# laboshinl/loam_velodyne

Measured on AMD Instinct MI355X. Metric: sweeps/sec (64-ring, 1M-pt map): feature extraction + odometry + scan-to-map registration, higher is better.
Workload: dtype f32

## Files before the change

include/loamx.h:

```cpp
#ifndef LOAMX_H
#define LOAMX_H

#include <stddef.h>
#include <stdint.h>

#ifdef __cplusplus
extern "C" {
#endif

#define LOAMX_OK 0
#define LOAMX_SKIPPED 1
#define LOAMX_E_INVALID (-1)
#define LOAMX_E_CAPACITY (-2)
#define LOAMX_E_HIP (-3)
#define LOAMX_E_NOGPU (-4)
#define LOAMX_E_UNSUPPORTED (-5)
#define LOAMX_E_INTERNAL (-6)

typedef struct loamx_cloud {
  void* data;
  uint32_t count;
  uint32_t stride;
  uint32_t intensity_offset;
  uint32_t reserved;
} loamx_cloud;

const char* loamx_last_error(void);
int loamx_device_count(void);
#define LOAMX_ABI_VERSION 6
int loamx_abi_version(void);
const char* loamx_build_info(void);
void* loamx_host_alloc(size_t bytes);
void loamx_host_free(void* p);

typedef struct loamx_scanreg loamx_scanreg;

typedef struct loamx_scanreg_config {
  float scan_period;
  int n_feature_regions;
  int curvature_region;
  int max_corner_sharp;
  int max_surface_flat;
  float less_flat_filter_size;
  float surface_curvature_threshold;
  int device;
  int max_corner_less_sharp;
  int imu_history_size;
} loamx_scanreg_config;


void loamx_scanreg_default_config(loamx_scanreg_config* cfg);
loamx_scanreg* loamx_scanreg_create(const loamx_scanreg_config* cfg);
void loamx_scanreg_destroy(loamx_scanreg* h);
int loamx_scanreg_configure(loamx_scanreg* h, const loamx_scanreg_config* cfg);
int loamx_scanreg_process(loamx_scanreg* h, const loamx_cloud* cloud, const uint32_t* ring_size, uint32_t n_rings,
                          loamx_cloud* sharp, loamx_cloud* less_sharp, loamx_cloud* flat, loamx_cloud* less_flat);

typedef struct loamx_multiscan_mapper {
  float lower_bound_deg;
  float upper_bound_deg;
  uint32_t n_scan_rings;
} loamx_multiscan_mapper;
int loamx_multiscan_mapper_preset(const char* sensor , loamx_multiscan_mapper* out);
int loamx_scanreg_process_raw(loamx_scanreg* h, const loamx_multiscan_mapper* mapper, const void* raw_xyz, uint32_t count,
                              uint32_t stride, loamx_cloud* full, uint32_t* ring_size, loamx_cloud* sharp, loamx_cloud* less_sharp,
                              loamx_cloud* flat, loamx_cloud* less_flat);

enum { LOAMX_RING_FROM_BOUNDS = 0, LOAMX_RING_FROM_TABLE = 1, LOAMX_RING_FROM_FIELD = 2 };
enum { LOAMX_TIME_FROM_AZIMUTH = 0, LOAMX_TIME_FROM_FIELD = 1 };
enum { LOAMX_FIELD_U8 = 1, LOAMX_FIELD_U16 = 2, LOAMX_FIELD_U32 = 3, LOAMX_FIELD_F32 = 4, LOAMX_FIELD_F64 = 5 };
typedef struct loamx_sensor_model {
  uint32_t n_scan_rings;
  uint32_t ring_source, time_source;
  float lower_bound_deg, upper_bound_deg;
  const float* ring_angles_deg;
  float max_angle_error_deg;
  uint32_t ring_offset, ring_type;
  uint32_t time_offset, time_type;
  double time_scale;
} loamx_sensor_model;
int loamx_sensor_model_from_mapper(const loamx_multiscan_mapper* m, loamx_sensor_model* out);
int loamx_sensor_model_check(const loamx_sensor_model* m, uint32_t stride);
int loamx_scanreg_process_sensor(loamx_scanreg* h, const loamx_sensor_model* m, const void* records, uint32_t count, uint32_t stride,
                                 loamx_cloud* full, uint32_t* ring_size, loamx_cloud* sharp, loamx_cloud* less_sharp,
                                 loamx_cloud* flat, loamx_cloud* less_flat);

int loamx_scanreg_update_imu(loamx_scanreg* h, double stamp_sec, float roll, float pitch, float yaw, const float acc_xyz[3]);
int loamx_scanreg_set_time(loamx_scanreg* h, double scan_time_sec);
int loamx_scanreg_get_imu_trans(loamx_scanreg* h, float imu_trans[12]);

typedef struct loamx_odom loamx_odom;

typedef struct loamx_odom_config {
  float scan_period;
  int max_iterations;
  float delta_t_abort;
  float delta_r_abort;
  int device;
} loamx_odom_config;

void loamx_odom_default_config(loamx_odom_config* cfg);
loamx_odom* loamx_odom_create(const loamx_odom_config* cfg);
void loamx_odom_destroy(loamx_odom* h);
int loamx_odom_update_imu(loamx_odom* h, const float imu_trans[12]);
int loamx_odom_process(loamx_odom* h, const loamx_cloud* sharp, const loamx_cloud* less_sharp, const loamx_cloud* flat,
                       const loamx_cloud* less_flat);
int loamx_odom_get_transform(loamx_odom* h, float transform[6]);
int loamx_odom_get_transform_sum(loamx_odom* h, float transform_sum[6]);
int loamx_odom_set_transform(loamx_odom* h, const float transform[6]);
int loamx_odom_set_transform_sum(loamx_odom* h, const float transform_sum[6]);
int loamx_odom_get_last_clouds(loamx_odom* h, loamx_cloud* last_corner, loamx_cloud* last_surf);
int loamx_odom_transform_to_end(loamx_odom* h, loamx_cloud* cloud);
int loamx_odom_get_stats(loamx_odom* h, int stats[4]);

int loamx_scanreg_process_linked(loamx_scanreg* h, const loamx_cloud* cloud, const uint32_t* ring_size, uint32_t n_rings);
int loamx_odom_process_linked(loamx_odom* h, loamx_scanreg* sr);
int loamx_odom_link_wait(loamx_odom* h);

typedef struct loamx_map loamx_map;

typedef struct loamx_map_config {
  float scan_period;
  int max_iterations;
  float delta_t_abort;
  float delta_r_abort;
  float corner_filter_size;
  float surf_filter_size;
  float map_filter_size;
  int device;
} loamx_map_config;

void loamx_map_default_config(loamx_map_config* cfg);
loamx_map* loamx_map_create(const loamx_map_config* cfg);
void loamx_map_destroy(loamx_map* h);
int loamx_map_update_odometry(loamx_map* h, const float transform_sum[6]);
int loamx_map_process(loamx_map* h, const loamx_cloud* corner_last, const loamx_cloud* surf_last, loamx_cloud* full_res);
int loamx_map_process_linked(loamx_map* h, loamx_odom* od, loamx_cloud* full_res_registered);
int loamx_map_get_speculation(loamx_map* h, uint64_t counts[2]);
int loamx_map_insert(loamx_map* h, const loamx_cloud* corner_last, const loamx_cloud* surf_last, const float pose6[6]);
int loamx_map_get_transform(loamx_map* h, int which, float transform[6]);
int loamx_map_set_transform(loamx_map* h, int which, const float transform[6]);
int loamx_map_update_imu(loamx_map* h, double stamp_sec, float roll, float pitch);
int loamx_map_set_time(loamx_map* h, double laser_odometry_time_sec);
int loamx_map_has_fresh_map(loamx_map* h);
int loamx_map_get_surround(loamx_map* h, loamx_cloud* out);
int loamx_map_load_cubes(loamx_map* h, const loamx_cloud* corner, const loamx_cloud* surf);
int loamx_map_get_cubes(loamx_map* h, int which, loamx_cloud* out);
int loamx_map_save_snapshot(loamx_map* h, const char* path);
int loamx_map_load_snapshot(loamx_map* h, const char* path);
int loamx_map_set_timing(loamx_map* h, int on);
int loamx_map_get_timing(loamx_map* h, float ms[4], uint64_t counts[4]);
int loamx_map_get_stats(loamx_map* h, int stats[8]);

typedef struct loamx_tm loamx_tm;
loamx_tm* loamx_tm_create(void);
void loamx_tm_destroy(loamx_tm* h);
int loamx_tm_update_odometry(loamx_tm* h, const float transform_sum[6]);
int loamx_tm_update_mapping_transform(loamx_tm* h, const float aft_mapped[6], const float bef_mapped[6]);
int loamx_tm_associate_to_map(loamx_tm* h);
int loamx_tm_get_mapped(loamx_tm* h, float transform_mapped[6]);
int loamx_wire_pose_to_quat(const float rot_xyz[3], double quat_xyzw[4]);
int loamx_wire_quat_to_pose(const double quat_xyzw[4], float rot_xyz[3]);

typedef struct loamx_batch loamx_batch;

loamx_batch* loamx_batch_create(const loamx_map_config* cfg, uint32_t max_sweeps);
void loamx_batch_destroy(loamx_batch* h);
int loamx_batch_set_frozen(loamx_batch* h, const loamx_cloud* corner_map, const loamx_cloud* surf_map);
int loamx_batch_set_frozen_device(loamx_batch* h, const void* d_corner_xyzi, uint32_t n_corner, const void* d_surf_xyzi,
                                  uint32_t n_surf);
int loamx_batch_stage_frozen_device(loamx_batch* h, const void* d_corner_xyzi, uint32_t n_corner, const void* d_surf_xyzi,
                                    uint32_t n_surf, void* wait_event );
int loamx_batch_stage_frozen(loamx_batch* h, const loamx_cloud* corner_map, const loamx_cloud* surf_map);
int loamx_batch_swap_frozen(loamx_batch* h);
int loamx_batch_upload(loamx_batch* h, uint32_t n_sweeps, const loamx_cloud* corner_last, const loamx_cloud* surf_last,
                       const loamx_cloud* full_res, const float* guess6);
int loamx_batch_run(loamx_batch* h);
int loamx_batch_run_async(loamx_batch* h);
int loamx_batch_sync(loamx_batch* h);
int loamx_batch_download(loamx_batch* h, float* poses6, int* stats4);
int loamx_batch_download_full_res(loamx_batch* h, uint32_t sweep, loamx_cloud* out);
int loamx_batch_set_timing(loamx_batch* h, int on);
int loamx_batch_get_timing(loamx_batch* h, float ms[4], uint64_t counts[4]);
void* loamx_batch_stream(loamx_batch* h);
int loamx_batch_knn_probe(loamx_batch* h, int which, const float* queries_xyz, uint32_t n, uint32_t* idx5, float* d2_5);
int loamx_batch_qr6_probe(loamx_batch* h, const float* ata, const float* atb, uint32_t n, float* x_coop, float* x_scalar);
int loamx_batch_xrec_stress(loamx_batch* h, uint32_t pairs, uint32_t rounds, uint64_t out4[4]);
int loamx_batch_download_ds(loamx_batch* h, uint32_t sweep, loamx_cloud* corner_ds, loamx_cloud* surf_ds);

int loamx_voxel_probe(const float* pts_xyzi, uint32_t n, const uint32_t* seg_off, const uint32_t* seg_ids, const uint8_t* valid, uint32_t nseg,
                      float leaf_even, float leaf_odd, float* out_xyzi, uint32_t* out_off);
#define LOAMX_SCAN_COUNT_ON_DEVICE 1u
#define LOAMX_SCAN_IN_PLACE 2u
#define LOAMX_SCAN_ZERO_IN 4u
int loamx_scan_probe(uint32_t* in, uint32_t n, uint32_t max_n, uint32_t flags, uint32_t* out, uint32_t* total, uint32_t* out2);
#define LOAMX_INDEX_SINGLE 1u
#define LOAMX_INDEX_PACK_RING 2u
#define LOAMX_INDEX_FOLD_BOUNDS 4u
typedef struct loamx_index_desc {
  float ox, oy, oz, inv_h;
  int32_t nx, ny, nz;
  uint32_t ncell;
  uint32_t cell_base;
  uint32_t pt_base;
} loamx_index_desc;
int loamx_index_probe(const float* pts_xyzw, uint32_t n, const uint32_t* off, uint32_t K, float cell_edge, uint32_t flags, loamx_index_desc* desc,
                      uint32_t* table, uint32_t table_cap, uint32_t* table_len, float* sorted_xyzw);
#define LOAMX_VOXBUCKET_SRC_POINTERS 1u
typedef struct loamx_voxbucket_seg {
  uint32_t bucket0, nbuckets, pos_bits, pad;
} loamx_voxbucket_seg;
typedef struct loamx_voxbucket_status {
  uint32_t gave_up;
  uint32_t why;
  uint32_t buckets;
  uint32_t pad;
} loamx_voxbucket_status;
int loamx_voxbucket_probe(const float* pts_xyzi, uint32_t n, const uint32_t* seg_off, uint32_t nseg, const float* poses12, float leaf_even,
                          float leaf_odd, uint32_t flags, float* stack_xyzi, float* out_xyzi, uint32_t* out_off,
                          loamx_voxbucket_status* status, loamx_voxbucket_seg* segs, uint64_t* lo, uint32_t* cnt, uint32_t bucket_cap);
#define LOAMX_REPROJECT_BATCH 0u
#define LOAMX_REPROJECT_FUSED 1u
#define LOAMX_REPROJECT_SINGLE 2u
#define LOAMX_REPROJECT_COPY 3u
#define LOAMX_REPROJECT_GATHER 4u
#define LOAMX_REPROJECT_TO_START 5u
#define LOAMX_REPROJECT_NO_RING_TABLE 8u
#define LOAMX_REPROJECT_NO_BOUNDS 16u
typedef struct loamx_reproject_params {
  float T[6];
  float sT[3], cT[3];
  float shift[3];
  float s_start[3], c_start[3];
  float s_end[3], c_end[3];
  float scan_period;
  int32_t enabled;
} loamx_reproject_params;
int loamx_reproject_probe(const float* pts_xyzw, uint32_t n, const uint32_t* off, uint32_t K, const loamx_reproject_params* params, uint32_t ns,
                          uint32_t epoch, uint32_t n_corner_all, uint32_t flags, float* out_xyzw, uint32_t* ring_first, uint32_t* bounds);

typedef struct loamx_pipeline loamx_pipeline;

loamx_pipeline* loamx_pipeline_create(const loamx_scanreg_config* fcfg, const loamx_odom_config* ocfg,
                                      const loamx_map_config* mcfg, uint32_t n_streams);
void loamx_pipeline_destroy(loamx_pipeline* h);
int loamx_pipeline_set_frozen(loamx_pipeline* h, const loamx_cloud* corner_map, const loamx_cloud* surf_map);
int loamx_pipeline_set_frozen_device(loamx_pipeline* h, const void* d_corner_xyzi, uint32_t n_corner, const void* d_surf_xyzi,
                                     uint32_t n_surf);
int loamx_pipeline_stage_frozen_device(loamx_pipeline* h, const void* d_corner_xyzi, uint32_t n_corner, const void* d_surf_xyzi,
                                       uint32_t n_surf, void* wait_event);
int loamx_pipeline_stage_frozen(loamx_pipeline* h, const loamx_cloud* corner_map, const loamx_cloud* surf_map);
int loamx_pipeline_swap_frozen(loamx_pipeline* h);
int loamx_pipeline_set_state(loamx_pipeline* h, uint32_t stream, const float* transform, const float* transform_sum,
                             const float* bef_mapped, const float* aft_mapped);
int loamx_pipeline_upload(loamx_pipeline* h, uint32_t n_steps, const loamx_cloud* clouds, const uint32_t* const* ring_size,
                          const uint32_t* n_rings);
int loamx_pipeline_stage_step(loamx_pipeline* h, uint32_t step, const loamx_cloud* clouds, const uint32_t* const* ring_size,
                              const uint32_t* n_rings);
int loamx_pipeline_stage_step_raw(loamx_pipeline* h, uint32_t step, const void* const* raw_xyz, const uint32_t* counts, uint32_t stride,
                                  const loamx_multiscan_mapper* mapper, const double* scan_time_sec);
int loamx_pipeline_stage_step_sensor(loamx_pipeline* h, uint32_t step, const void* const* records, const uint32_t* counts,
                                     uint32_t stride, const loamx_sensor_model* m, const double* scan_time_sec);
int loamx_pipeline_update_imu(loamx_pipeline* h, uint32_t stream, double stamp_sec, float roll, float pitch, float yaw, const float acc_xyz[3]);
int loamx_pipeline_enable_async_downloads(loamx_pipeline* h);
int loamx_pipeline_download_step_async(loamx_pipeline* h, loamx_cloud* out, uint32_t n_out);
int loamx_pipeline_wait_downloads(loamx_pipeline* h);
int loamx_pipeline_download_counts(loamx_pipeline* h, uint64_t counts[2]);
int loamx_pipeline_step(loamx_pipeline* h, uint32_t step);
int loamx_pipeline_get(loamx_pipeline* h, uint32_t stream, float* transform, float* transform_sum, float* aft_mapped,
                       int* stats8);
int loamx_pipeline_download_full_res(loamx_pipeline* h, uint32_t slot, loamx_cloud* out);
int loamx_pipeline_download_last_clouds(loamx_pipeline* h, uint32_t stream, loamx_cloud* last_corner, loamx_cloud* last_surf);
int loamx_pipeline_set_lookahead(loamx_pipeline* h, int on);
int loamx_pipeline_lookahead_depth(loamx_pipeline* h);
int loamx_pipeline_drain_lookahead(loamx_pipeline* h, int* last_odometry_step);
int loamx_pipeline_set_timing(loamx_pipeline* h, int on);
int loamx_pipeline_get_timing(loamx_pipeline* h, float stage_ms[4], float reg_ms[4], uint64_t counts[4]);
int loamx_pipeline_get_odom_launch_timing(loamx_pipeline* h, double ms4[4], uint64_t counts7[7]);
void* loamx_pipeline_stream(loamx_pipeline* h);

typedef struct loamx_dist loamx_dist;
#define LOAMX_DIST_ID_BYTES 128
int loamx_dist_get_unique_id(unsigned char id[LOAMX_DIST_ID_BYTES]);
loamx_dist* loamx_dist_create(const unsigned char id[LOAMX_DIST_ID_BYTES], int rank, int world_size, int device);
void loamx_dist_destroy(loamx_dist* h);
int loamx_dist_rank(const loamx_dist* h);
int loamx_dist_world_size(const loamx_dist* h);
int loamx_dist_shard(const loamx_dist* h, uint32_t batch, uint32_t* begin, uint32_t* end);
int loamx_dist_broadcast_map(loamx_dist* h, void* d_corner_xyzi, uint32_t n_corner, void* d_surf_xyzi, uint32_t n_surf, int root,
                             void* wait_event, void** done_event);
int loamx_dist_allgather_results(loamx_dist* h, const float* poses6, const int* iters_flags2, uint32_t n_local, float* poses6_all,
                                 int* iters_flags2_all, uint32_t* counts_all);
int loamx_dist_allgather_results_cap(loamx_dist* h, const float* poses6, const int* iters_flags2, uint32_t n_local, float* poses6_all,
                                     int* iters_flags2_all, uint32_t capacity_records, uint32_t* counts_all);
int loamx_dist_allgather_counts(loamx_dist* h, uint32_t n_local, uint32_t* counts_all);
int loamx_dist_comm_count(loamx_dist* h);
#define LOAMX_DIST_RECORD_FLOATS 8
int loamx_dist_shard_of(int rank, int world_size, uint32_t batch, uint32_t* begin, uint32_t* end);
int loamx_dist_pack_results(const float* poses6, const int* iters_flags2, uint32_t n_local, uint32_t n_pad, float* send8);
int loamx_dist_unpack_results(const float* recv8, const uint32_t* counts, int world_size, uint32_t n_pad, float* poses6_all,
                              int* iters_flags2_all);
int loamx_dist_pack_clouds(uint32_t n_streams, const loamx_cloud* corner, const loamx_cloud* surf, const float* poses6, uint32_t* words,
                           uint64_t capacity_words, uint64_t* n_words);
int loamx_dist_unpack_clouds_header(const uint32_t* words, uint64_t n_words, uint32_t* n_streams, uint32_t* n_corner, uint32_t* n_surf,
                                    uint32_t capacity_streams);
int loamx_dist_unpack_clouds_stream(const uint32_t* words, uint64_t n_words, uint32_t stream, float pose6[6], loamx_cloud* corner,
                                    loamx_cloud* surf);
int loamx_dist_gatherv(loamx_dist* h, const uint32_t* send_words, uint32_t n_words, int root, uint32_t* recv_words, uint64_t capacity_words,
                       uint32_t* counts_all);
int loamx_dist_barrier(loamx_dist* h);
void* loamx_dist_stream(loamx_dist* h);

typedef struct loamx_densemap loamx_densemap;
typedef struct loamx_densemap_config {
  float leaf;
  float min_range;
  float max_range;
  uint64_t max_voxels;
  uint32_t initial_slots;
  int device;
} loamx_densemap_config;

void loamx_densemap_default_config(loamx_densemap_config* cfg);
loamx_densemap* loamx_densemap_create(const loamx_densemap_config* cfg);
void loamx_densemap_destroy(loamx_densemap* h);
int loamx_densemap_reset(loamx_densemap* h);
int loamx_densemap_add(loamx_densemap* h, const loamx_cloud* points, const float origin[3]);
int loamx_densemap_add_from_map(loamx_densemap* h, loamx_map* m);
int loamx_densemap_add_from_pipeline(loamx_densemap* h, loamx_pipeline* p, uint32_t slot);
int loamx_densemap_get_stats(loamx_densemap* h, uint64_t stats[6]);
int loamx_densemap_download(loamx_densemap* h, loamx_cloud* out, int axes );
int loamx_densemap_save_pcd(loamx_densemap* h, const char* path, int axes);
int loamx_write_pcd(const char* path, const loamx_cloud* c, int axes);

typedef struct loamx_densemap_carve_config {
  float max_range;
  uint32_t ray_stride;
  uint32_t end_margin;
  uint32_t max_steps;
} loamx_densemap_carve_config;
typedef struct loamx_densemap_static_rule {
  uint32_t min_misses;
  uint32_t num, den;
} loamx_densemap_static_rule;
void loamx_densemap_carve_default_config(loamx_densemap_carve_config* cfg);
void loamx_densemap_static_rule_default(loamx_densemap_static_rule* rule);
int loamx_densemap_rule_is_dynamic(const loamx_densemap_static_rule* rule, uint64_t n, uint32_t miss);
int loamx_densemap_enable_carving(loamx_densemap* h, const loamx_densemap_carve_config* cfg );
int loamx_densemap_get_carve_stats(loamx_densemap* h, uint64_t stats[6]);
int loamx_densemap_download_misses(loamx_densemap* h, uint32_t* out, uint64_t capacity, uint64_t* n);
int loamx_densemap_download_static(loamx_densemap* h, loamx_cloud* out, int axes, const loamx_densemap_static_rule* rule);
int loamx_densemap_save_pcd_static(loamx_densemap* h, const char* path, int axes, const loamx_densemap_static_rule* rule);
int loamx_densemap_prune(loamx_densemap* h, const loamx_densemap_static_rule* rule, uint64_t* removed);

typedef struct loamx_surfel {
  float x, y, z, intensity, normal_x, normal_y, normal_z, curvature;
} loamx_surfel;
typedef struct loamx_densemap_surfel_config {
  uint32_t min_points;
  float min_planar_ratio;
} loamx_densemap_surfel_config;
void loamx_densemap_surfel_default_config(loamx_densemap_surfel_config* cfg);
int loamx_densemap_surfel_of(float leaf, const int32_t idx[3], const uint64_t vals[4], const uint64_t mom[9],
                             const loamx_densemap_surfel_config* cfg, int axes, loamx_surfel* out);
int loamx_densemap_enable_moments(loamx_densemap* h);
int loamx_densemap_download_moments(loamx_densemap* h, uint64_t* out, uint64_t capacity, uint64_t* n);
int loamx_densemap_download_surfels(loamx_densemap* h, loamx_surfel* out, uint64_t capacity, uint64_t* n, int axes,
                                    const loamx_densemap_surfel_config* cfg, const loamx_densemap_static_rule* rule);
int loamx_densemap_save_pcd_surfels(loamx_densemap* h, const char* path, int axes, const loamx_densemap_surfel_config* cfg,
                                    const loamx_densemap_static_rule* rule);

int loamx_densemap_freeze(loamx_densemap* h, const loamx_densemap_surfel_config* cfg, const loamx_densemap_static_rule* rule,
                          uint64_t* n_surfels);
int loamx_densemap_frozen_size(loamx_densemap* h, uint64_t* n_surfels);
int loamx_densemap_align_step(loamx_densemap* h, const loamx_cloud* points, const float rtc[15], uint32_t neighbourhood,
                              float max_residual, int64_t sums[28], uint64_t counts[5]);
typedef struct loamx_densemap_align_config {
  uint32_t max_iterations;
  uint32_t neighbourhood;
  float max_residual;
  uint32_t min_matched;
  float eps_rot, eps_trans;
  float degenerate_ratio;
} loamx_densemap_align_config;
typedef struct loamx_densemap_align_result {
  double pose[12];
  uint32_t iterations, degenerate_dims;
  int status;
  double rms;
  uint64_t counts[5];
} loamx_densemap_align_result;
void loamx_densemap_align_default_config(loamx_densemap_align_config* cfg);
int loamx_densemap_align_solve(const int64_t sums[28], float degenerate_ratio, double x[6], uint32_t* dropped);
int loamx_densemap_align(loamx_densemap* h, const loamx_cloud* points, const double pose_in[12], const float centre[3] ,
                         const loamx_densemap_align_config* cfg , loamx_densemap_align_result* out);
int loamx_densemap_align_from_map(loamx_densemap* h, loamx_map* m, const double pose_in[12] ,
                                  const loamx_densemap_align_config* cfg, loamx_densemap_align_result* out);
int loamx_densemap_align_from_pipeline(loamx_densemap* h, loamx_pipeline* p, uint32_t slot, const double pose_in[12],
                                       const loamx_densemap_align_config* cfg, loamx_densemap_align_result* out);

#define LOAMX_ALIGN_MAX_POSES 4096
int loamx_densemap_align_step_many(loamx_densemap* h, const loamx_cloud* points, const float* rtc , uint32_t n_poses,
                                   uint32_t neighbourhood, float max_residual, int64_t* sums , uint64_t* counts );
int loamx_densemap_align_many(loamx_densemap* h, const loamx_cloud* points, const double* poses_in , uint32_t n_poses,
                              const float centre[3] , const loamx_densemap_align_config* cfg,
                              loamx_densemap_align_result* out , uint32_t* best );
int loamx_densemap_align_many_from_map(loamx_densemap* h, loamx_map* m, const double* poses_in, uint32_t n_poses,
                                       const loamx_densemap_align_config* cfg, loamx_densemap_align_result* out, uint32_t* best);
int loamx_densemap_align_many_from_pipeline(loamx_densemap* h, loamx_pipeline* p, uint32_t slot, const double* poses_in, uint32_t n_poses,
                                            const loamx_densemap_align_config* cfg, loamx_densemap_align_result* out, uint32_t* best);
int loamx_densemap_align_best(const loamx_densemap_align_result* results, uint32_t n, uint32_t* best);
int loamx_densemap_get_align_stats(loamx_densemap* h, uint64_t stats[3]);

#define LOAMX_PYRAMID_MAX_LEVELS 6
typedef struct loamx_densemap_pyramid_config {
  uint32_t levels;
  float max_curvature;
} loamx_densemap_pyramid_config;
void loamx_densemap_pyramid_default_config(loamx_densemap_pyramid_config* cfg);
int loamx_densemap_coarsen(loamx_densemap* h, uint32_t level, const loamx_densemap_static_rule* rule ,
                           uint64_t* keys, uint64_t* vals , uint64_t* mom , uint64_t capacity,
                           uint64_t* n);
int loamx_densemap_freeze_pyramid(loamx_densemap* h, const loamx_densemap_surfel_config* cfg, const loamx_densemap_static_rule* rule,
                                  const loamx_densemap_pyramid_config* pyramid , uint64_t* n_surfels );
int loamx_densemap_frozen_levels(loamx_densemap* h, uint32_t* levels);
int loamx_densemap_align_select_level(loamx_densemap* h, uint32_t level);
int loamx_densemap_align_pyramid(loamx_densemap* h, const loamx_cloud* points, const double pose_in[12], const float centre[3] ,
                                 const loamx_densemap_align_config* cfg, uint32_t first_level,
                                 loamx_densemap_align_result* out );
int loamx_densemap_align_pyramid_from_map(loamx_densemap* h, loamx_map* m, const double pose_in[12] ,
                                          const loamx_densemap_align_config* cfg, uint32_t first_level, loamx_densemap_align_result* out);
int loamx_densemap_align_pyramid_from_pipeline(loamx_densemap* h, loamx_pipeline* p, uint32_t slot, const double pose_in[12],
                                               const loamx_densemap_align_config* cfg, uint32_t first_level,
                                               loamx_densemap_align_result* out);

struct loamx_densemap_file_info {
  uint32_t version, flags;
  float leaf;
  uint64_t voxels;
  uint64_t offered, dropped_range, dropped_key;
  uint64_t carve_stats[6];
  loamx_densemap_carve_config carve;
};
int loamx_densemap_save(loamx_densemap* h, const char* path);
int loamx_densemap_load(loamx_densemap* h, const char* path);
int loamx_densemap_merge(loamx_densemap* dst, loamx_densemap* src);
int loamx_densemap_merge_file(loamx_densemap* dst, const char* path);
int loamx_densemap_file_info(const char* path, struct loamx_densemap_file_info* info, int deep);

#define LOAMX_RAY_NOT_TRACED 0
#define LOAMX_RAY_MISS 1
#define LOAMX_RAY_HIT 2
#define LOAMX_RAY_HIT_END 3
typedef struct loamx_ray_hit {
  uint64_t key;
  float x, y, z;
  float range;
  uint32_t n;
  uint32_t miss;
  uint32_t steps;
  uint32_t status;
} loamx_ray_hit;
typedef struct loamx_densemap_raycast_config {
  uint32_t max_steps;
  uint32_t skip_steps;
  uint32_t min_points;
} loamx_densemap_raycast_config;
void loamx_densemap_raycast_default_config(loamx_densemap_raycast_config* cfg);
int loamx_densemap_raycast(loamx_densemap* h, const loamx_cloud* ends, const float origin[3],
                           const loamx_densemap_raycast_config* cfg ,
                           const loamx_densemap_static_rule* rule ,
                           loamx_ray_hit* out , uint64_t capacity, uint64_t counts[5]);
int loamx_densemap_raycast_from_map(loamx_densemap* h, loamx_map* m, const loamx_densemap_raycast_config* cfg,
                                    const loamx_densemap_static_rule* rule, loamx_ray_hit* out, uint64_t capacity, uint64_t counts[5]);
int loamx_densemap_raycast_from_pipeline(loamx_densemap* h, loamx_pipeline* p, uint32_t slot,
                                         const loamx_densemap_raycast_config* cfg, const loamx_densemap_static_rule* rule,
                                         loamx_ray_hit* out, uint64_t capacity, uint64_t counts[5]);

typedef struct loamx_densemap_history_config {
  uint64_t max_bytes;
  uint64_t initial_points;
} loamx_densemap_history_config;
void loamx_densemap_history_default_config(loamx_densemap_history_config* cfg);
int loamx_densemap_enable_history(loamx_densemap* h, const loamx_densemap_history_config* cfg );
int loamx_densemap_history_size(loamx_densemap* h, uint64_t* calls, uint64_t* points);
int loamx_densemap_history_download(loamx_densemap* h, uint64_t call, loamx_cloud* out , float origin[3]);
int loamx_densemap_correct(const double correction[12], const float* xyz_in, float* xyz_out, uint64_t n);
int loamx_densemap_rebuild(loamx_densemap* h, const double* corrections ,
                           uint64_t n_calls);
int loamx_densemap_get_rebuild_stats(loamx_densemap* h, uint64_t stats[4]);

#define LOAMX_GRID_UNKNOWN 0
#define LOAMX_GRID_FREE 1
#define LOAMX_GRID_OBSTACLE 2
#define LOAMX_GRID_STEP 3
typedef struct loamx_densemap_grid_config {
  uint32_t cell_leaves;
  int32_t  x0, z0;
  uint32_t nx, nz;
  uint32_t min_points;
  int32_t  y_min, y_max;
  uint32_t band_lo, band_hi;
  uint32_t min_obstacle_voxels;
  uint32_t max_step;
  uint32_t clear_max;
} loamx_densemap_grid_config;
typedef struct loamx_grid_cell {
  int32_t  ground;
  float    elevation;
  uint32_t obstacles;
  int32_t  overhead;
  uint32_t clear2;
  uint32_t cls;
} loamx_grid_cell;
void loamx_densemap_grid_default_config(loamx_densemap_grid_config* cfg);
int loamx_densemap_grid_check(const loamx_densemap_grid_config* cfg);
int loamx_densemap_grid_window(float leaf, float centre_x, float centre_z, float half_extent, loamx_densemap_grid_config* cfg);
int loamx_densemap_grid(loamx_densemap* h, const loamx_densemap_grid_config* cfg ,
                        const loamx_densemap_static_rule* rule ,
                        loamx_grid_cell* out );
int loamx_grid_occupancy(const loamx_grid_cell* cells, uint64_t n, int8_t* out);
int loamx_write_grid_pgm(const char* stem, const loamx_grid_cell* cells, const loamx_densemap_grid_config* cfg, float leaf);

#define LOAMX_ROUTE_UNREACHABLE 0xffffffffu
#define LOAMX_ROUTE_GOAL 8u
#define LOAMX_ROUTE_NONE 9u
typedef struct loamx_grid_route_config {
  uint32_t connectivity;
  uint32_t min_clear2;
  uint32_t soft_clear2;
  uint32_t soft_weight;
  uint32_t unknown_weight;
} loamx_grid_route_config;
typedef struct loamx_route_cell {
  uint32_t cost;
  uint32_t next;
} loamx_route_cell;
void loamx_grid_route_default_config(loamx_grid_route_config* cfg);
int loamx_grid_route_check(const loamx_grid_route_config* cfg);
int loamx_grid_route_weight(const loamx_grid_cell* cell, const loamx_grid_route_config* cfg);
int loamx_densemap_route(loamx_densemap* h, const loamx_densemap_grid_config* grid_cfg ,
                         const loamx_densemap_static_rule* rule ,
                         const loamx_grid_route_config* cfg , const uint32_t* goals_xz, uint32_t n_goals,
                         loamx_grid_cell* out_cells , loamx_route_cell* out_field ,
                         uint64_t stats[6] );
int loamx_densemap_route_cells(loamx_densemap* h, const loamx_grid_cell* cells, uint32_t nx, uint32_t nz,
                               const loamx_grid_route_config* cfg , const uint32_t* goals_xz, uint32_t n_goals,
                               loamx_route_cell* out_field , uint64_t stats[6] );
int loamx_densemap_route_trace(loamx_densemap* h, const uint32_t* starts_xz, uint32_t n_starts ,
                               uint32_t* out_xz , uint32_t capacity, uint32_t* lengths );
int loamx_grid_route_trace(const loamx_route_cell* field, uint32_t nx, uint32_t nz, uint32_t start_x, uint32_t start_z,
                           uint32_t* out_xz , uint32_t capacity, uint32_t* length);
int loamx_grid_route_points(const loamx_densemap_grid_config* grid_cfg, float leaf, const loamx_grid_cell* cells ,
                            const uint32_t* route_xz, uint32_t n, float* out_xyz );
int loamx_densemap_grid_cell_of(const loamx_densemap_grid_config* grid_cfg, float leaf, float x, float z, uint32_t* rx, uint32_t* rz,
                                int* inside);

#define LOAMX_FRONTIER_NONE 0xFFFFFFFFu
typedef struct loamx_grid_frontier_config {
  uint32_t connectivity;
  uint32_t min_unknown;
  uint32_t min_clear2;
  uint32_t min_cells;
} loamx_grid_frontier_config;
typedef struct loamx_frontier {
  uint32_t min_cell;
  uint32_t cells;
  uint32_t lo[2], hi[2];
  uint64_t sum_rx, sum_rz;
  uint64_t unknown_links;
  uint32_t reachable;
// ... 143 lines not shown
```

loam_velodyne_amd/csrc/hostlink.hpp:

```cpp
#pragma once
#include "common.h"
#include <hsa/hsa.h>
#include <hsa/hsa_ext_amd.h>

namespace loamx {

template <int SLOTS> class HostLinkT {
 public:
  ~HostLinkT() {
    for (int s = 0; s < SLOTS; s++) {
      if (!made_[s]) continue;
      try { wait(s); } catch (...) {}
      (void)hsa_signal_destroy(sig_[s]);
    }
  }
  bool can_copy(void* host_dst, const void* dev_src, size_t bytes) {
    if (!init_()) return false;
    hsa_agent_t g, c;
    return owner_(dev_src, bytes, HSA_DEVICE_TYPE_GPU, &g) && owner_(host_dst, bytes, HSA_DEVICE_TYPE_CPU, &c);
  }
  void begin(int slot, uint32_t n) {
    LX_REQUIRE(init_(), "ROCr is not available");
    wait(slot);
    if (!made_[slot]) {
      LX_REQUIRE(hsa_signal_create(0, 0, nullptr, &sig_[slot]) == HSA_STATUS_SUCCESS, "hsa_signal_create failed");
      made_[slot] = true;
    }
    hsa_signal_store_relaxed(sig_[slot], (hsa_signal_value_t)n);
    pending_[slot] = n > 0;
    unissued_[slot] = n;
  }
  void abandon(int slot) {
    if (!pending_[slot]) return;
    if (unissued_[slot]) hsa_signal_subtract_relaxed(sig_[slot], (hsa_signal_value_t)unissued_[slot]);
    unissued_[slot] = 0;
    try { wait(slot); } catch (...) { pending_[slot] = false; }
  }
  void copy_d2h(int slot, void* host_dst, const void* dev_src, size_t bytes) {
    hsa_agent_t g, c;
    LX_REQUIRE(owner_(dev_src, bytes, HSA_DEVICE_TYPE_GPU, &g) && owner_(host_dst, bytes, HSA_DEVICE_TYPE_CPU, &c), "not ROCr-allocated memory");
    hsa_status_t st = HSA_STATUS_ERROR;
    const uint32_t eng = engine_(c, g);
    if (eng) {
      st = hsa_amd_memory_async_copy_on_engine(host_dst, c, dev_src, g, bytes, 0, nullptr, sig_[slot], (hsa_amd_sdma_engine_id_t)eng, false);
      if (st != HSA_STATUS_SUCCESS) engine_mask_ = 0;
    }
    if (st != HSA_STATUS_SUCCESS) st = hsa_amd_memory_async_copy(host_dst, c, dev_src, g, bytes, 0, nullptr, sig_[slot]);
    if (st != HSA_STATUS_SUCCESS) {
      abandon(slot);
      throw Error(LOAMX_E_HIP, "hsa_amd_memory_async_copy failed (" + std::to_string((int)st) + ")");
    }
    if (unissued_[slot]) unissued_[slot]--;
  }
  bool can_copy_h2d(void* dev_dst, const void* host_src, size_t bytes) {
    if (!init_()) return false;
    hsa_agent_t g, c;
    return owner_(dev_dst, bytes, HSA_DEVICE_TYPE_GPU, &g) && owner_(host_src, bytes, HSA_DEVICE_TYPE_CPU, &c);
  }
  bool host_ok(const void* host, size_t bytes) {
    hsa_agent_t c;
    return init_() && owner_(host, bytes, HSA_DEVICE_TYPE_CPU, &c);
  }
  void copy_h2d(int slot, void* dev_dst, const void* host_src, size_t bytes) {
    hsa_agent_t g, c;
    LX_REQUIRE(owner_(dev_dst, bytes, HSA_DEVICE_TYPE_GPU, &g) && owner_(host_src, bytes, HSA_DEVICE_TYPE_CPU, &c), "not ROCr-allocated memory");
    const hsa_status_t st = hsa_amd_memory_async_copy(dev_dst, g, host_src, c, bytes, 0, nullptr, sig_[slot]);
    if (st != HSA_STATUS_SUCCESS) {
      abandon(slot);
      throw Error(LOAMX_E_HIP, "hsa_amd_memory_async_copy (host -> device) failed (" + std::to_string((int)st) + ")");
    }
    if (unissued_[slot]) unissued_[slot]--;
  }
  uint32_t engine() const { return engine_mask_ == ~0u ? 0u : engine_mask_; }
  bool pending(int slot) const { return pending_[slot]; }
  void wait(int slot) {
    if (!pending_[slot]) return;
    hsa_signal_value_t v;
    while ((v = hsa_signal_wait_scacquire(sig_[slot], HSA_SIGNAL_CONDITION_LT, 1, UINT64_MAX, HSA_WAIT_STATE_BLOCKED)) > 0) {}
    pending_[slot] = false;
    if (v < 0) throw Error(LOAMX_E_HIP, "a device -> host DMA reported an error");
  }

 private:
  static bool init_() {
    static const bool ok = hsa_init() == HSA_STATUS_SUCCESS;
    return ok;
  }
  static bool owner_(const void* p, size_t bytes, hsa_device_type_t want, hsa_agent_t* agent) {
    hsa_amd_pointer_info_t info;
    info.size = sizeof(info);
    if (hsa_amd_pointer_info(p, &info, nullptr, nullptr, nullptr) != HSA_STATUS_SUCCESS) return false;
    if (info.type != HSA_EXT_POINTER_TYPE_HSA) return false;
    const char* base = (const char*)(want == HSA_DEVICE_TYPE_CPU && info.hostBaseAddress ? info.hostBaseAddress : info.agentBaseAddress);
    if (!base || (const char*)p < base || (const char*)p + bytes > base + info.sizeInBytes) return false;
    hsa_device_type_t type;
    if (hsa_agent_get_info(info.agentOwner, HSA_AGENT_INFO_DEVICE, &type) != HSA_STATUS_SUCCESS || type != want) return false;
    *agent = info.agentOwner;
    return true;
  }
  uint32_t engine_(hsa_agent_t cpu, hsa_agent_t gpu) {
    if (engine_mask_ == ~0u) {
      if (const char* e = diag_env("LOAMX_D2H_ENGINE")) engine_mask_ = (uint32_t)strtoul(e, nullptr, 0);
      else {
        uint32_t rec = 0;
        if (hsa_amd_memory_get_preferred_copy_engine(cpu, gpu, &rec) != HSA_STATUS_SUCCESS) rec = 0;
        rec &= ~(uint32_t)HSA_AMD_SDMA_ENGINE_0;
        engine_mask_ = rec ? (rec & (~rec + 1u)) : (uint32_t)HSA_AMD_SDMA_ENGINE_1;
      }
    }
    return engine_mask_;
  }
  uint32_t engine_mask_ = ~0u;
  hsa_signal_t sig_[SLOTS] = {};
  bool made_[SLOTS] = {}, pending_[SLOTS] = {};
  uint32_t unissued_[SLOTS] = {};
};
using HostLinkDma = HostLinkT<2>;
using HostLinkUp = HostLinkT<8>;

}
```

loam_velodyne_amd/csrc/pipeline.hip:

```cpp
#include "pinned_copy.hpp"
#include "features.hpp"
#include "odometry.hpp"
#include "registration.hpp"
#include "hostlink.hpp"
#include "densemap.hpp"
#include "odom_lookahead.hpp"
#include <atomic>
#include <deque>
#include <chrono>
#include <mutex>
#include <memory>

namespace loamx {

struct OdomPub {
  HTwist transform, transform_sum;
  OdomStats stats = {0, 0, 0, 0};
  int rc = LOAMX_SKIPPED;
  const float4* last_corner = nullptr; uint32_t n_last_corner = 0;
  const float4* last_surf = nullptr; uint32_t n_last_surf = 0;
  ToEndParams to_end;
};

struct PipeStreamState {
  HTwist bef, aft, tobe, incre;
  OdomPub cur;
  SweepStats map_stats = {0, 0, 0, 0, 0, 0, 0, 0};
  bool mapped = false;
};

class Pipeline {
 public:
  Pipeline(const loamx_scanreg_config& fc, const loamx_odom_config& oc, const loamx_map_config& mc, uint32_t n_streams)
      : reg(mc.device, n_streams), fcfg(fc), n_streams_(n_streams), st(n_streams), imu(n_streams), map_imu(n_streams), map_imu_seq(n_streams, 0) {
    OdomParams op;
    op.scan_period = oc.scan_period;
    op.max_iterations = diag_env("LOAMX_ODOM_MAXIT") ? atoi(diag_env("LOAMX_ODOM_MAXIT")) : oc.max_iterations;
    if (op.max_iterations < 1 || op.max_iterations > 255) throw Error(LOAMX_E_INVALID, "odometry max_iterations must be in [1, 255]");
    op.delta_t_abort = oc.delta_t_abort;
    op.delta_r_abort = oc.delta_r_abort;
    {
      int g = (int)std::min<uint32_t>(n_streams, 2);
      if (const char* e = diag_env("LOAMX_ODOM_GROUPS")) g = atoi(e);
      n_groups = (uint32_t)std::max(1, std::min(g, (int)std::min<uint32_t>(n_streams, MAX_GROUPS)));
    }
    for (uint32_t g = 0; g < n_groups; g++) {
      chains.emplace_back(new OdomChain());
      OdomChain& c = *chains.back();
      c.s0 = (uint32_t)((uint64_t)g * n_streams / n_groups);
      c.s1 = (uint32_t)((uint64_t)(g + 1) * n_streams / n_groups);
      c.ob.reset(new OdometryBatch(mc.device, c.s1 - c.s0, nullptr));
    }
    for (auto& o : ores) o.resize(n_streams);
    for (auto& tr : imu) tr.history_size = std::max(200, fc.imu_history_size);
    reg.params.max_iterations = mc.max_iterations;
    reg.early_exit = true;
    reg.double_buffer_full = true;
    reg.params.delta_t_abort = mc.delta_t_abort;
    reg.params.delta_r_abort = mc.delta_r_abort;
    reg.params.corner_leaf = mc.corner_filter_size;
    reg.params.surf_leaf = mc.surf_filter_size;
    for (auto& c : chains) { c->ob->params = op; c->ob->set_keep(OR - 2); }
    device = mc.device;
    if (getenv("LOAMX_NO_LOOKAHEAD")) prefetch = false;
    const double spin_us = diag_env("LOAMX_SPIN_US") ? atof(diag_env("LOAMX_SPIN_US")) : 400.0;
    la.reset(new LookAhead(
        n_groups, [this](uint32_t g, int k) { run_chain_step(*chains[g], (uint32_t)k); }, [this] { (void)hipSetDevice(device); },
        std::chrono::duration_cast<std::chrono::steady_clock::duration>(std::chrono::duration<double, std::micro>(spin_us))));
  }
  Registrar reg;
  static constexpr int OR = 16;
  struct LazyTimer {
    hipEvent_t a = nullptr, b = nullptr;
    bool pending = false;
    float ms = 0.f;
    void start(hipStream_t s) {
      if (!a) { LX_HIP(hipEventCreate(&a)); LX_HIP(hipEventCreate(&b)); }
      pending = false;
      LX_HIP(hipEventRecord(a, s));
    }
    void stop(hipStream_t s) { LX_HIP(hipEventRecord(b, s)); pending = true; }
    bool resolve() {
      if (!pending || hipEventQuery(b) != hipSuccess) return false;
      LX_HIP(hipEventElapsedTime(&ms, a, b));
      pending = false;
      return true;
    }
    void destroy() { if (a) { (void)hipEventDestroy(a); (void)hipEventDestroy(b); a = b = nullptr; } }
  };
  struct OdomChain {
    uint32_t s0 = 0, s1 = 0;
    std::unique_ptr<OdometryBatch> ob;
    hipEvent_t ev_tail[OR] = {};
    LazyTimer tm[OR];
    std::atomic<float> ms{0.f};
    double tr[4] = {0, 0, 0, 0};
    std::atomic<float> last_us{0.f};
  };
  static constexpr uint32_t MAX_GROUPS = 16;
  uint32_t n_groups = 1;
  std::vector<std::unique_ptr<OdomChain>> chains;
  OdomChain& chain_of(uint32_t s) { uint32_t g = 0; while (g + 1 < n_groups && s >= chains[g]->s1) g++; return *chains[g]; }
  OdometryBatch& OB(uint32_t s) { return *chain_of(s).ob; }
  uint32_t LS(uint32_t s) { return s - chain_of(s).s0; }
  loamx_scanreg_config fcfg;
  uint32_t n_streams_;
  int device;
  std::vector<PipeStreamState> st;
  std::vector<std::unique_ptr<FeatureExtractor>> fx;
  static constexpr uint32_t RING = 8;
  bool streaming = false;
  std::atomic<uint32_t> staged_hi{0};
  hipStream_t cstream = nullptr, dstream = nullptr;
  hipEvent_t ev_stage[RING] = {};
  hipEvent_t ev_reg_done = nullptr, ev_d2h[2] = {nullptr, nullptr};
  bool d2h_pending[2] = {false, false};
  uint64_t downloads_direct = 0, downloads_hip = 0;
  HostLinkDma hostlink;
  HostLinkUp uplink;
  uint32_t up_runs[RING] = {};
  std::atomic<long> last_step{-1};
  std::vector<uint32_t> last_full_off;
  std::vector<uint32_t> last_who;
  struct RawSlot {
    bool raw = false, finalized = true;
    std::vector<uint32_t> count, off;
    DevBuf<char> d_bytes;
    DevBuf<float4> d_raw4, d_binned;
    DevBuf<uint32_t> d_ring_fld;
    DevBuf<double> d_time_fld;
    DevBuf<uint32_t> d_ring_cnt;
    PinBuf<uint32_t> h_ring_cnt;
    DevBuf<ImuLast> d_last;
    PinBuf<ImuLast> h_last;
    DevBuf<double> d_imu_d;
    DevBuf<float> d_imu_f;
    PinBuf<double> h_imu_d;
    PinBuf<float> h_imu_f;
    std::vector<uint32_t> imu_H;
    std::vector<float> imu_trans;
    std::vector<double> scan_time;
    std::vector<uint64_t> map_imu_upto;
    hipEvent_t ev_ingest = nullptr;
    uint32_t n_rings = 0;
  };
  RawSlot rawslot[RING];
  std::vector<ImuTracker> imu;
  struct MapImu { double stamp; float roll, pitch; uint64_t seq; };
  std::vector<std::deque<MapImu>> map_imu;
  std::vector<uint64_t> map_imu_seq;
  std::mutex map_imu_mu;
  void map_imu_push(uint32_t s, double stamp, float roll, float pitch) {
    std::lock_guard<std::mutex> lk(map_imu_mu);
    if (map_imu[s].size() >= 200) map_imu[s].pop_front();
    map_imu[s].push_back(MapImu{stamp, roll, pitch, map_imu_seq[s]++});
  }
  bool map_imu_blend(uint32_t s, uint64_t seq_limit, double odo_time, float scan_period, float* p6) {
    std::lock_guard<std::mutex> lk(map_imu_mu);
    const std::deque<MapImu>& Hq = map_imu[s];
    size_t n = 0;
    while (n < Hq.size() && Hq[n].seq < seq_limit) n++;
    if (!n) return false;
    size_t i = 0;
    while (i < n - 1 && (odo_time - Hq[i].stamp) + scan_period > 0) i++;
    float roll, pitch;
    if (i == 0 || (odo_time - Hq[i].stamp) + scan_period > 0) {
      roll = Hq[i].roll; pitch = Hq[i].pitch;
    } else {
      const float ratio = (float)(((Hq[i].stamp - odo_time) - scan_period) / (Hq[i].stamp - Hq[i - 1].stamp));
      const float inv = 1 - ratio;
      roll = Hq[i].roll * inv + Hq[i - 1].roll * ratio;
      pitch = Hq[i].pitch * inv + Hq[i - 1].pitch * ratio;
    }
    p6[0] = (float)(0.998 * p6[0] + 0.002 * pitch);
    p6[2] = (float)(0.998 * p6[2] + 0.002 * roll);
    return true;
  }
  RawBinner binner;
  FeatureExtractor& FX(uint32_t t) { return *fx[streaming ? t % RING : t]; }
  char& LA(uint32_t t) { return launched[streaming ? t % RING : t]; }
  uint32_t n_staged() const { return streaming ? staged_hi.load(std::memory_order_acquire) : (uint32_t)fx.size(); }
  hipStream_t fstream = nullptr;
  bool prefetch = true;
  std::vector<char> launched;
  PinBuf<uint32_t> h_off3[OR];
  hipEvent_t evF[OR][2] = {};
  LazyTimer tmM[2];
  float feat_ms[OR] = {};
  int f_hi = -1;
  int ahead_depth = std::max(1, std::min(diag_env("LOAMX_ODOM_AHEAD") ? atoi(diag_env("LOAMX_ODOM_AHEAD")) : 6, OR - 2));
  int depth() const { return !prefetch ? 0 : (streaming ? std::min(ahead_depth, (int)RING - 2) : ahead_depth); }
  float last_ms[4] = {0, 0, 0, 0};
  std::atomic<bool> timing{false};

  std::vector<OdomPub> ores[OR];
  std::unique_ptr<LookAhead> la;
  void run_chain_step(OdomChain& c, uint32_t k) {
    const auto tc0 = std::chrono::steady_clock::now();
    c.tr[0] = tr_us(); run_odometry(c, k); c.tr[3] = tr_us();
    c.last_us.store((float)std::chrono::duration<double, std::micro>(std::chrono::steady_clock::now() - tc0).count(), std::memory_order_relaxed);
  }
  int drain_lookahead() { return prefetch ? la->drain() : la->done_min(); }
  void park_odometry(int restart) {
    if (restart >= 0) pre_t = -1;
    la->park(restart);
  }

  ~Pipeline() {
    la.reset();
    for (auto& c : chains) {
      for (auto& e : c->ev_tail) if (e) (void)hipEventDestroy(e);
      for (auto& tm : c->tm) tm.destroy();
    }
    fx.clear();
    for (auto& a : evF) for (auto& e : a) if (e) (void)hipEventDestroy(e);
    for (auto& tm : tmM) tm.destroy();
    for (auto& e : ev_stage) if (e) (void)hipEventDestroy(e);
    for (auto& r : rawslot) if (r.ev_ingest) (void)hipEventDestroy(r.ev_ingest);
    for (auto& e : ev_d2h) if (e) (void)hipEventDestroy(e);
    if (ev_reg_done) (void)hipEventDestroy(ev_reg_done);
    if (cstream) { (void)hipStreamSynchronize(cstream); (void)hipStreamDestroy(cstream); }
    if (dstream) { (void)hipStreamSynchronize(dstream); (void)hipStreamDestroy(dstream); }
    if (fstream) (void)hipStreamDestroy(fstream);
  }

  void launch_features(uint32_t t) {
    TraceRange trace_range("loamx:features");
    finalize_raw(t);
    FeatureExtractor& F = FX(t);
    const uint32_t ns = n_streams_, nring = F.total_rings();
    if (streaming) {
      LX_HIP(hipStreamWaitEvent(fstream, ev_stage[t % RING], 0));
      if (up_runs[t % RING]) { uplink.wait((int)(t % RING)); up_runs[t % RING] = 0; }
    }
    PinBuf<uint32_t>& hb = h_off3[t % OR];
    hb.reserve(3 * (ns + 1) + nring + 2);
    for (auto& e : evF[t % OR]) if (!e) LX_HIP(hipEventCreate(&e));
    LX_HIP(hipEventRecord(evF[t % OR][0], fstream));
    F.run_async();
    LX_REQUIRE(F.n_offsets() == 3 * (ns + 1) + nring + 1, "internal: offset table layout");
    store_to_pinned_u32(hb.p, F.d_offsets(), F.n_offsets(), fstream);
    LX_HIP(hipEventRecord(evF[t % OR][1], fstream));
    LA(t) = 1;
  }

  std::unique_ptr<FeatureExtractor> new_extractor_() {
    auto f = std::make_unique<FeatureExtractor>(device, fstream);
    f->params = feat_params_from(fcfg);
    return f;
  }
  void feature_stream_() {
    if (!fstream) fstream = create_stream(env_priority("LOAMX_PRIO_FEAT", -1), diag_env("LOAMX_FEAT_CU_STRIDE") ? atoi(diag_env("LOAMX_FEAT_CU_STRIDE")) : 0, 1);
    LX_HIP(hipStreamSynchronize(fstream));
    fx.clear();
  }
  void restart_input_(uint32_t n_slots, bool ring) {
    streaming = ring;
    staged_hi = 0;
    last_step = -1;
    launched.assign(n_slots, 0);
    la->reset();
    f_hi = -1;
  }

  void upload(uint32_t n_steps, const loamx_cloud* clouds, const uint32_t* const* ring_size, const uint32_t* n_rings) {
    LX_REQUIRE(n_steps >= 1 && clouds && ring_size && n_rings, "invalid argument");
    LX_HIP(hipSetDevice(device));
    feature_stream_();
    restart_input_(n_steps, false);
    for (uint32_t t = 0; t < n_steps; t++) {
      auto f = new_extractor_();
      f->upload(n_streams_, clouds + (size_t)t * n_streams_, ring_size + (size_t)t * n_streams_, n_rings + (size_t)t * n_streams_);
      fx.push_back(std::move(f));
    }
  }

  void begin_staging_(uint32_t t, const char* entry) {
    LX_HIP(hipSetDevice(device));
    if (!streaming) {
      LX_REQUIRE(t == 0, "streaming input starts at step 0");
      feature_stream_();
      for (uint32_t k = 0; k < RING; k++) fx.push_back(new_extractor_());
      if (!cstream) cstream = create_stream(0);
      for (auto& e : ev_stage) if (!e) LX_HIP(hipEventCreateWithFlags(&e, hipEventDisableTiming));
      restart_input_(RING, true);
    }
    LX_REQUIRE(t == staged_hi.load(), "steps must be staged in order");
    LX_REQUIRE(t < RING || last_step.load() + (long)RING >= (long)t, std::string(entry) + "(t) needs step(t - 8) to have run: only eight steps can be in flight");
  }
  void publish_staged_(uint32_t t) {
    LA(t) = 0;
    staged_hi.store(t + 1, std::memory_order_release);
  }

  void stage_step(uint32_t t, const loamx_cloud* clouds, const uint32_t* const* ring_size, const uint32_t* n_rings) {
    LX_REQUIRE(clouds && ring_size && n_rings, "invalid argument");
    begin_staging_(t, "stage_step");
    TraceRange trace_range("loamx:pipeline:stage_step");
    if (t > 0) finalize_raw(t - 1);
    rawslot[t % RING].raw = false;
    rawslot[t % RING].finalized = true;
    static const bool direct = !(diag_env("LOAMX_H2D_DIRECT") && atoi(diag_env("LOAMX_H2D_DIRECT")) == 0);
    const int slot = (int)(t % RING);
    up_runs[slot] = 0;
    uint32_t n_blocks = 0;
    bool all_direct = direct;
    if (direct) {
      for (uint32_t s = 0; s < n_streams_ && all_direct;) {
        all_direct = clouds[s].stride == 16 && clouds[s].intensity_offset == 12;
        uint32_t e = s + 1;
        size_t cnt = clouds[s].count;
        while (all_direct && e < n_streams_ && (const char*)clouds[e].data == (const char*)clouds[s].data + sizeof(float4) * cnt) cnt += clouds[e++].count;
        if (cnt) { n_blocks++; all_direct = all_direct && uplink.host_ok(clouds[s].data, sizeof(float4) * cnt); }
        s = e;
      }
    }
    if (all_direct && n_blocks) {
      uplink.begin(slot, n_blocks);
      uint32_t issued = 0;
      try {
        fx[slot]->upload_async(n_streams_, clouds, ring_size, n_rings, cstream, ev_stage[slot], [&](void* dst, const void* src, size_t bytes) {
          if (!uplink.can_copy_h2d(dst, src, bytes)) throw Error(LOAMX_E_HIP, "internal: a staging block is not ROCr's memory after all");
          uplink.copy_h2d(slot, dst, src, bytes);
          issued++;
          return true;
        });
      } catch (...) {
        uplink.abandon(slot);
        throw;
      }
      up_runs[slot] = issued;
    } else {
      fx[slot]->upload_async(n_streams_, clouds, ring_size, n_rings, cstream, ev_stage[slot]);
    }
    publish_staged_(t);
  }

  void stage_step_raw(uint32_t t, const void* const* raw_xyz, const uint32_t* counts, uint32_t stride, const loamx_multiscan_mapper& mapper,
                      const double* scan_time) {
    LX_REQUIRE(raw_xyz && counts, "invalid argument");
    mapper_check(mapper.lower_bound_deg, mapper.upper_bound_deg, mapper.n_scan_rings, stride);
    stage_records_(t, raw_xyz, counts, stride, mapper_params(mapper.lower_bound_deg, mapper.upper_bound_deg, mapper.n_scan_rings), scan_time);
  }
  void stage_step_sensor(uint32_t t, const void* const* records, const uint32_t* counts, uint32_t stride, const loamx_sensor_model& model,
                         const double* scan_time) {
    LX_REQUIRE(records && counts, "invalid argument");
    sensor_model_check(model, stride);
    stage_records_(t, records, counts, stride, sensor_params(model), scan_time);
  }
  void stage_records_(uint32_t t, const void* const* raw_xyz, const uint32_t* counts, uint32_t stride, const SensorParams& model,
                      const double* scan_time) {
    begin_staging_(t, "stage_step_raw");
    TraceRange trace_range("loamx:pipeline:stage_step_raw");
    if (t > 0) finalize_raw(t - 1);
    const uint32_t ns = n_streams_, nr = model.M.n_rings;
    RawSlot& R = rawslot[t % RING];
    R.raw = true;
    R.finalized = false;
    R.n_rings = nr;
    R.count.assign(counts, counts + ns);
    R.off.assign(ns + 1, 0);
    for (uint32_t s = 0; s < ns; s++) {
      LX_REQUIRE(raw_xyz[s] || counts[s] == 0, "NULL raw cloud");
      R.off[s + 1] = R.off[s] + counts[s];
    }
    const uint32_t ntot = R.off[ns];
    R.d_bytes.reserve((size_t)ntot * stride + 16);
    R.d_raw4.reserve((size_t)ntot + 1);
    R.d_binned.reserve((size_t)ntot + 1);
    if (model.ring_src == RING_FIELD) R.d_ring_fld.reserve((size_t)ntot + 1);
    if (model.time_src == TIME_FIELD) R.d_time_fld.reserve((size_t)ntot + 1);
    R.d_ring_cnt.reserve((size_t)ns * nr + 1);
    R.h_ring_cnt.reserve((size_t)ns * nr + 1);
    R.d_last.reserve(ns);
    R.h_last.reserve(ns);
    R.imu_H.assign(ns, 0);
    R.imu_trans.assign((size_t)12 * ns, 0.f);
    if (scan_time) R.scan_time.assign(scan_time, scan_time + ns); else R.scan_time.clear();
    {
      std::lock_guard<std::mutex> lk(map_imu_mu);
      R.map_imu_upto = map_imu_seq;
    }
    if (!R.ev_ingest) LX_HIP(hipEventCreateWithFlags(&R.ev_ingest, hipEventDisableTiming));
    size_t Htot = 0;
    for (uint32_t s = 0; s < ns; s++) { R.imu_H[s] = imu[s].size(); Htot += R.imu_H[s]; }
    if (Htot) {
      R.h_imu_d.reserve(2 * Htot); R.h_imu_f.reserve(9 * Htot); R.d_imu_d.reserve(2 * Htot); R.d_imu_f.reserve(9 * Htot);
    }
    binner.init(cstream);
    LX_HIP(hipMemsetAsync(R.d_last.p, 0, sizeof(ImuLast) * ns, cstream));
    size_t hbase = 0;
    std::vector<ImuTable> tables(ns);
    for (uint32_t s = 0; s < ns; s++) {
      if (scan_time) imu[s].set_scan_time(scan_time[s]);
      const uint32_t H = R.imu_H[s];
      if (H) {
        imu[s].fill_table(R.h_imu_d.p + 2 * hbase, R.h_imu_f.p + 9 * hbase, tables[s]);
        tables[s].dt = R.d_imu_d.p + 2 * hbase;
        tables[s].dstamp = R.d_imu_d.p + 2 * hbase + H;
        tables[s].state = R.d_imu_f.p + 9 * hbase;
        hbase += H;
      }
    }
    if (Htot) {
      LX_HIP(hipMemcpyAsync(R.d_imu_d.p, R.h_imu_d.p, sizeof(double) * 2 * Htot, hipMemcpyHostToDevice, cstream));
      LX_HIP(hipMemcpyAsync(R.d_imu_f.p, R.h_imu_f.p, sizeof(float) * 9 * Htot, hipMemcpyHostToDevice, cstream));
    }
    for (uint32_t s = 0; s < ns; s++) {
      const uint32_t n = counts[s];
      if (n) LX_HIP(hipMemcpyAsync(R.d_bytes.p + (size_t)R.off[s] * stride, raw_xyz[s], (size_t)n * stride, hipMemcpyHostToDevice, cstream));
      SensorParams sp = model;
      sp.ring_fld = model.ring_src == RING_FIELD ? R.d_ring_fld.p + R.off[s] : nullptr;
      sp.time_fld = model.time_src == TIME_FIELD ? R.d_time_fld.p + R.off[s] : nullptr;
      unpack_records(R.d_bytes.p + (size_t)R.off[s] * stride, stride, n, sp, R.d_raw4.p + R.off[s], cstream);
      binner.run(R.d_raw4.p + R.off[s], n, sp, fcfg.scan_period, R.d_binned.p + R.off[s], R.d_ring_cnt.p + (size_t)s * nr,
                 R.imu_H[s] ? &tables[s] : nullptr, R.imu_H[s] ? R.d_last.p + s : nullptr);
    }
    LX_HIP(hipMemcpyAsync(R.h_ring_cnt.p, R.d_ring_cnt.p, sizeof(uint32_t) * ns * nr, hipMemcpyDeviceToHost, cstream));
    LX_HIP(hipMemcpyAsync(R.h_last.p, R.d_last.p, sizeof(ImuLast) * ns, hipMemcpyDeviceToHost, cstream));
    LX_HIP(hipEventRecord(R.ev_ingest, cstream));
    publish_staged_(t);
  }

  std::mutex raw_mu;
  void finalize_raw(uint32_t t) {
    if (!streaming) return;
    std::lock_guard<std::mutex> lk(raw_mu);
    RawSlot& R = rawslot[t % RING];
    if (!R.raw || R.finalized) return;
    LX_HIP(hipEventSynchronize(R.ev_ingest));
    const uint32_t ns = n_streams_, nr = R.n_rings;
    std::vector<const uint32_t*> rs(ns);
    std::vector<uint32_t> nrv(ns, nr);
    for (uint32_t s = 0; s < ns; s++) {
      if (R.imu_H[s] && R.h_last.p[s].valid) imu[s].apply_last(R.h_last.p[s]);
      imu[s].begin_sweep();
      memcpy(&R.imu_trans[12 * (size_t)s], imu[s].imu_trans(), sizeof(float) * 12);
      rs[s] = R.h_ring_cnt.p + (size_t)s * nr;
    }
    fx[t % RING]->upload_device(ns, R.d_binned.p, R.off.data(), rs.data(), nrv.data(), cstream, ev_stage[t % RING]);
    R.finalized = true;
  }

  void download_step_async(loamx_cloud* out, uint32_t n_out) {
    LX_REQUIRE(out, "NULL argument");
    LX_REQUIRE(reg.double_buffer_full, "call loamx_pipeline_enable_async_downloads() before the first step");
    LX_HIP(hipSetDevice(device));
    const uint32_t nw = last_full_off.empty() ? 0u : (uint32_t)last_full_off.size() - 1;
    LX_REQUIRE(n_out >= nw, "fewer output descriptors than registered streams");
    const int par = (int)((run_count + 1) & 1);
    int rc_cap = LOAMX_OK;
    for (uint32_t k = 0; k < nw; k++) {
      check_cloud(&out[k], false);
      LX_REQUIRE(out[k].stride == 16 && out[k].intensity_offset == 12, "asynchronous downloads need packed float4 records (stride 16, intensity at 12)");
    }
    struct Run { char* dst; const char* src; size_t bytes; };
    std::vector<Run> runs;
    for (uint32_t k = 0; k < nw;) {
      uint32_t e = k;
      size_t cnt = 0;
      char* base = (char*)out[k].data;
      do {
        const uint32_t n = last_full_off[e + 1] - last_full_off[e];
        const uint32_t m = std::min(n, out[e].count);
        if (n > out[e].count) rc_cap = LOAMX_E_CAPACITY;
        out[e].count = n;
        cnt += m;
        e++;
        if (m != n) break;
      } while (e < nw && (char*)out[e].data == base + sizeof(float4) * cnt);
      if (cnt) runs.push_back(Run{base, (const char*)(reg.d_full_res() + last_full_off[k]), sizeof(float4) * cnt});
      k = e;
    }
    static const bool via_hip = diag_env("LOAMX_D2H_HIP") != nullptr;
    bool direct = !via_hip && !runs.empty();
    for (const Run& r : runs) direct = direct && hostlink.can_copy(r.dst, r.src, r.bytes);
    wait_download(par);
    if (direct) {
      if (ev_reg_done) LX_HIP(hipEventSynchronize(ev_reg_done));
      try {
        hostlink.begin(par, (uint32_t)runs.size());
        for (const Run& r : runs) hostlink.copy_d2h(par, r.dst, r.src, r.bytes);
        downloads_direct++;
      } catch (const Error&) {
        direct = false;
      }
    }
    if (!direct && !runs.empty()) {
      if (!dstream) dstream = create_stream(0);
      if (!ev_d2h[par]) LX_HIP(hipEventCreateWithFlags(&ev_d2h[par], hipEventDisableTiming));
      LX_HIP(hipStreamWaitEvent(dstream, ev_reg_done, 0));
      for (const Run& r : runs) LX_HIP(hipMemcpyAsync(r.dst, r.src, r.bytes, hipMemcpyDeviceToHost, dstream));
      LX_HIP(hipEventRecord(ev_d2h[par], dstream));
      d2h_pending[par] = true;
      downloads_hip++;
    }
    if (rc_cap != LOAMX_OK) throw Error(LOAMX_E_CAPACITY, "an output cloud is smaller than the registered cloud (count fields hold the needed sizes)");
  }
  void wait_download(int par) {
    hostlink.wait(par);
    if (d2h_pending[par]) { LX_HIP(hipEventSynchronize(ev_d2h[par])); d2h_pending[par] = false; }
  }
  void wait_downloads() {
    for (int par = 0; par < 2; par++) wait_download(par);
  }
  uint64_t run_count = 0;

  void run_odometry(OdomChain& c, uint32_t t) {
    const uint32_t ns = n_streams_, ng = c.s1 - c.s0;
    FeatureExtractor& F = FX(t);
    LX_REQUIRE(LA(t), "internal: odometry of a step whose features were not launched");
    OdometryBatch& odom = *c.ob;
    uint32_t* hb = h_off3[t % OR].p;
    uint32_t* ho[3] = {hb, hb + (ns + 1), hb + 2 * (ns + 1)};
    uint32_t* hlf = hb + 3 * (ns + 1);
    wait_event(evF[t % OR][1]);
    F.check_finite_input();
    c.tr[1] = tr_us();
    const bool timed = timing.load(std::memory_order_relaxed);
    if (timed && c.s0 == 0) LX_HIP(hipEventElapsedTime(&feat_ms[t % OR], evF[t % OR][0], evF[t % OR][1]));
    std::vector<OdomInput> in(ng);
    std::vector<int> rc(ng, 0);
    for (uint32_t s = c.s0; s < c.s1; s++) {
      const uint32_t la = hlf[F.ring_base(s)], lb = hlf[F.ring_base(s + 1)];
      in[s - c.s0] = OdomInput{F.d_feat(0) + ho[0][s], ho[0][s + 1] - ho[0][s], F.d_feat(1) + ho[1][s], ho[1][s + 1] - ho[1][s],
                               F.d_feat(2) + ho[2][s], ho[2][s + 1] - ho[2][s], F.d_less_flat() + la, lb - la};
    }
    const int slot = (int)(t % OR);
    if (timed) c.tm[slot].start(odom.stream());
    if (streaming && rawslot[t % RING].raw)
      for (uint32_t s = c.s0; s < c.s1; s++) odom.update_imu(s - c.s0, &rawslot[t % RING].imu_trans[12 * (size_t)s]);
    odom.process(in.data(), rc.data(), true);
    c.tr[2] = tr_us();
    if (!c.ev_tail[slot]) LX_HIP(hipEventCreateWithFlags(&c.ev_tail[slot], hipEventDisableTiming));
    LX_HIP(hipEventRecord(c.ev_tail[slot], odom.stream()));
    if (timed) c.tm[slot].stop(odom.stream());
    for (auto& tm : c.tm)
      if (tm.resolve()) c.ms.store(tm.ms, std::memory_order_relaxed);
    for (uint32_t s = c.s0; s < c.s1; s++) {
      const uint32_t l = s - c.s0;
      OdomStream& O = odom.stream_state(l);
      OdomPub& N = ores[slot][s];
      N.transform = O.transform;
      N.transform_sum = O.transform_sum;
      N.stats = O.stats;
      N.rc = rc[l];
      N.last_corner = odom.d_last_corner(l); N.n_last_corner = O.n_last_corner;
      N.last_surf = odom.d_last_surf(l); N.n_last_surf = O.n_last_surf;
      N.to_end = odom.to_end_params(l, true);
    }
  }
  int pre_t = -1;
  void prestage_gather(int tn, int last_staged, hipStream_t s_) {
    static const bool off = !(diag_env("LOAMX_PRESTAGE") && atoi(diag_env("LOAMX_PRESTAGE")) != 0);
    if (off || !prefetch || pre_t == tn || tn > last_staged || tn < 1) return;
    const uint32_t ns = n_streams_;
    if (la->done_min() < tn) return;
    FeatureExtractor& F = FX((uint32_t)tn);
    std::vector<const float4*> fsrc;
    std::vector<uint32_t> nfr;
    std::vector<ToEndParams> tep;
    for (uint32_t s = 0; s < ns; s++) {
      const OdomPub& N = ores[tn % OR][s];
      if (N.rc != LOAMX_OK) continue;
      fsrc.push_back(F.d_cloud() + F.point_base(s));
      nfr.push_back(F.point_base(s + 1) - F.point_base(s));
      tep.push_back(N.to_end);
    }
    const uint32_t nw = (uint32_t)fsrc.size();
    if (!nw) return;
    const int par = (int)(run_count & 1);
    hostlink.wait(par);
    if (d2h_pending[par]) { LX_HIP(hipStreamWaitEvent(s_, ev_d2h[par], 0)); d2h_pending[par] = false; }
    float4* dst = reg.stage_full_next(nw, nfr.data());
    if (!dst) return;
    std::vector<uint32_t> foff(nw + 1, 0);
    for (uint32_t k = 0; k < nw; k++) foff[k + 1] = foff[k] + nfr[k];
    chains[0]->ob->to_end_gather(dst, foff.data(), fsrc.data(), tep.data(), nw, s_);
    pre_t = tn;
  }

  bool trace = getenv("LOAMX_PIPE_TRACE") != nullptr;
  std::chrono::steady_clock::time_point tr0, tr_exit = std::chrono::steady_clock::now();
  double tr_us() const { return std::chrono::duration<double, std::micro>(std::chrono::steady_clock::now() - tr0).count(); }

  struct Step {
    uint32_t t = 0;
    int ti = 0, last_staged = -1;
    LookaheadWindow w;
    bool late_pending = false;
    hipStream_t s_ = nullptr;
    std::vector<uint32_t> who;
    std::vector<const float4*> cl, sl, fsrc;
    std::vector<uint32_t> ncl, nsl, nfr;
    std::vector<float> guess;
    std::vector<ToEndParams> to_end;
    uint32_t nw = 0;
    float f_ms = 0.f;
    double gap_us = 0, tr[5] = {0, 0, 0, 0, 0};
  };
  void launch_features_upto(int k) {
    while (f_hi < k) { ++f_hi; if (!LA((uint32_t)f_hi)) launch_features((uint32_t)f_hi); }
  }

  void join_odometry_(Step& S) {
    const uint32_t t = S.t;
    const int ti = S.ti;
    if (la->jumped(ti)) {
      park_odometry(ti);
      f_hi = ti - 1;
    }
    LX_REQUIRE(ti + (OR - 2) >= la->done_max(), "this step's odometry results have been overwritten: steps run in order");
    if (ti > la->done_min()) {
      launch_features_upto(S.w.feat_join);
      if (prefetch) {
        la->allow(S.w.odom_join);
        la->wait(ti);
      } else {
        if (la->limit() >= 0) park_odometry(-1);
        for (uint32_t g = 0; g < n_groups; g++)
          if (ti > la->done(g)) { run_odometry(*chains[g], t); la->ran_inline(g, ti); }
      }
    }
    LA(t) = 0;
    for (uint32_t s = 0; s < n_streams_; s++) st[s].cur = ores[t % OR][s];
    S.f_ms = feat_ms[t % OR];
    for (auto& c : chains) LX_HIP(hipStreamWaitEvent(S.s_, c->ev_tail[t % OR], 0));
  }
  void release_lookahead_(Step& S) {
    launch_features_upto(S.w.feat_reg);
    la->allow(S.w.odom_reg);
    S.late_pending = S.w.late;
  }
  void release_late_(Step& S) {
    if (!S.late_pending) return;
    S.late_pending = false;
    launch_features_upto(S.w.feat_late);
    la->allow(S.w.odom_late);
  }
  void gather_inputs_(Step& S) {
    S.tr[0] = tr_us();
    if (timing) tmM[S.t & 1].start(S.s_);
    const uint32_t ns = n_streams_;
    FeatureExtractor& F = FX(S.t);
    S.cl.resize(ns); S.sl.resize(ns); S.fsrc.resize(ns);
    S.ncl.resize(ns); S.nsl.resize(ns); S.nfr.resize(ns);
    for (uint32_t s = 0; s < ns; s++) {
      PipeStreamState& P = st[s];
      if (P.cur.rc != LOAMX_OK) continue;
      transform_associate_to_map(P.cur.transform_sum, P.bef, P.aft, P.incre, P.tobe);
      float g[6];
      P.tobe.get(g);
      S.guess.insert(S.guess.end(), g, g + 6);
      const uint32_t k = (uint32_t)S.who.size();
      S.cl[k] = P.cur.last_corner; S.ncl[k] = P.cur.n_last_corner;
      S.sl[k] = P.cur.last_surf; S.nsl[k] = P.cur.n_last_surf;
      S.fsrc[k] = F.d_cloud() + F.point_base(s);
      S.nfr[k] = F.point_base(s + 1) - F.point_base(s);
      S.to_end.push_back(P.cur.to_end);
      S.who.push_back(s);
    }
    S.nw = (uint32_t)S.who.size();
  }
  void stage_full_res_(Step& S) {
    if (!S.nw) { last_full_off.clear(); last_who.clear(); return; }
    const uint32_t nw = S.nw;
    std::vector<uint32_t> foff(nw + 1, 0);
    for (uint32_t k = 0; k < nw; k++) foff[k + 1] = foff[k] + S.nfr[k];
    const bool adopted = pre_t == S.ti && reg.adopt_full_next(nw, S.nfr.data());
    pre_t = -1;
    if (!adopted) {
      if (reg.double_buffer_full) {
        const int par = (int)(run_count & 1);
        const double tw0 = trace ? tr_us() : 0.0;
        hostlink.wait(par);
        if (trace) S.tr[4] = tr_us() - tw0;
        if (d2h_pending[par]) { LX_HIP(hipStreamWaitEvent(S.s_, ev_d2h[par], 0)); d2h_pending[par] = false; }
      }
      float4* full_dst = reg.stage_full(nw, S.nfr.data());
      chains[0]->ob->to_end_gather(full_dst, foff.data(), S.fsrc.data(), S.to_end.data(), nw, S.s_);
    }
    last_full_off = foff;
    last_who = S.who;
    run_count++;
  }
  void enqueue_registration_(Step& S) {
    if (!S.nw) return;
    const uint32_t nw = S.nw;
    const RawSlot& R = rawslot[S.t % RING];
    reg.upload_device(nw, S.cl.data(), S.ncl.data(), S.sl.data(), S.nsl.data(), nullptr, nullptr, S.guess.data());
    bool blend = false;
    static const bool no_blend = diag_env("LOAMX_NO_MAP_IMU_BLEND") != nullptr;
    if (!no_blend && streaming && R.raw && !R.scan_time.empty())
      for (uint32_t k = 0; k < nw; k++) blend = blend || R.map_imu_upto[S.who[k]] > 0;
    reg.defer_full = blend;
    reg.on_first_wait = [&]() { release_late_(S); prestage_gather(S.ti + 1, S.last_staged, S.s_); };
    reg.run_async();
    reg.on_first_wait = nullptr;
    if (blend) {
      std::vector<float> p6(6 * (size_t)nw);
      reg.download(p6.data(), nullptr);
      if (reg.submap_sufficient())
        for (uint32_t k = 0; k < nw; k++)
          (void)map_imu_blend(S.who[k], R.map_imu_upto[S.who[k]], R.scan_time[S.who[k]], fcfg.scan_period, &p6[6 * (size_t)k]);
      reg.finish_with_poses(p6.data());
      reg.defer_full = false;
    }
    if (reg.double_buffer_full) {
      if (!ev_reg_done) LX_HIP(hipEventCreateWithFlags(&ev_reg_done, hipEventDisableTiming));
      LX_HIP(hipEventRecord(ev_reg_done, S.s_));
    }
  }
  void release_behind_registration_(Step& S) {
    release_late_(S);
    if (S.nw) prestage_gather(S.ti + 1, S.last_staged, S.s_);
    if (timing) tmM[S.t & 1].stop(S.s_);
    S.tr[1] = tr_us();
  }
  int collect_(Step& S) {
    int ret = LOAMX_SKIPPED;
    if (S.nw) {
      std::vector<float> poses(6 * (size_t)S.nw);
      std::vector<SweepStats> ss(S.nw);
      reg.download(poses.data(), nullptr);
      reg.download_stats(ss.data());
      for (uint32_t k = 0; k < S.nw; k++) {
        PipeStreamState& P = st[S.who[k]];
        P.map_stats = ss[k];
        P.mapped = true;
        if (reg.submap_sufficient()) {
          P.tobe.set(&poses[6 * (size_t)k]);
          P.bef = P.cur.transform_sum;
          P.aft = P.tobe;
        }
      }
      ret = LOAMX_OK;
    }
    S.tr[2] = tr_us();
    return ret;
  }
  void finish_step_(Step& S) {
    const uint32_t t = S.t;
    S.tr[3] = tr_us();
    last_step = (long)t;
    tr_exit = std::chrono::steady_clock::now();
    if (trace) {
      fprintf(stderr, "[pipe t=%u] caller gap %.0f | M-start %.0f  M-enqueued %.0f  M-downloaded %.0f  O-joined %.0f  (download-wait %.0f) |", t, S.gap_us, S.tr[0], S.tr[1], S.tr[2], S.tr[3], S.tr[4]);
      for (uint32_t g = 0; g < n_groups; g++) {
        const OdomChain& c = *chains[g];
        fprintf(stderr, " O[%u-%u): %.0f %.0f %.0f %.0f done %d pass %.0f us |", c.s0, c.s1, c.tr[0], c.tr[1], c.tr[2], c.tr[3], la->done(g), (double)c.last_us.load());
      }
      fprintf(stderr, " f_hi %d o_limit %d staged %u", f_hi, la->limit(), n_staged());
      fprintf(stderr, "\n");
    }
    if (timing) {
      for (auto& x : tmM) x.resolve();
      last_ms[0] = S.f_ms;
      {
        float m = 0.f;
        for (auto& c : chains) m = std::max(m, c->ms.load(std::memory_order_relaxed));
        last_ms[1] = m;
      }
      last_ms[2] = tmM[t & 1].pending ? tmM[(t + 1) & 1].ms : tmM[t & 1].ms;
      last_ms[3] = last_ms[2];
    }
  }

  int step(uint32_t t) {
    TraceRange trace_range("loamx:pipeline:step");
    LX_REQUIRE(t < n_staged(), "step index beyond the staged sweeps");
    LX_REQUIRE(!streaming || t + RING >= staged_hi.load(), "this step's slot has been re-staged already");
    Step S;
    const auto t_entry = std::chrono::steady_clock::now();
    S.gap_us = std::chrono::duration<double, std::micro>(t_entry - tr_exit).count();
    tr0 = t_entry;
    LX_HIP(hipSetDevice(device));
    S.t = t;
    S.ti = (int)t;
    S.s_ = reg.stream();
    S.last_staged = (int)n_staged() - 1;
    S.w = lookahead_window(S.ti, depth(), S.last_staged, prefetch);
    join_odometry_(S);
    release_lookahead_(S);
    gather_inputs_(S);
    stage_full_res_(S);
    enqueue_registration_(S);
    release_behind_registration_(S);
    const int ret = collect_(S);
    finish_step_(S);
    return ret;
  }
};

}

using namespace loamx;

struct loamx_pipeline {
  Pipeline p;
  loamx_pipeline(const loamx_scanreg_config& f, const loamx_odom_config& o, const loamx_map_config& m, uint32_t n) : p(f, o, m, n) {}
};

extern "C" {

loamx_pipeline* loamx_pipeline_create(const loamx_scanreg_config* fcfg, const loamx_odom_config* ocfg, const loamx_map_config* mcfg,
                                      uint32_t n_streams) {
  loamx_pipeline* h = nullptr;
  guard([&]() {
    loamx_scanreg_config f;
    loamx_odom_config o;
    loamx_map_config m;
    if (fcfg) f = *fcfg; else loamx_scanreg_default_config(&f);
    if (ocfg) o = *ocfg; else loamx_odom_default_config(&o);
    if (mcfg) m = *mcfg; else loamx_map_default_config(&m);
    LX_REQUIRE(n_streams >= 1 && n_streams <= 1024, "n_streams must be in [1, 1024]");
    LX_REQUIRE(f.device == m.device && o.device == m.device, "all three configurations must name the same device");
    LX_REQUIRE(f.max_corner_less_sharp == 0 || f.max_corner_less_sharp >= f.max_corner_sharp, "max_corner_less_sharp must be >= max_corner_sharp");
    h = new loamx_pipeline(f, o, m, n_streams);
    return LOAMX_OK;
  });
  return h;
}
void loamx_pipeline_destroy(loamx_pipeline* h) { delete h; }

int loamx_pipeline_set_frozen(loamx_pipeline* h, const loamx_cloud* corner_map, const loamx_cloud* surf_map) {
  return guard([&]() { LX_REQUIRE(h, "NULL handle"); h->p.reg.set_submap_host(corner_map, surf_map); return LOAMX_OK; });
}
int loamx_pipeline_set_frozen_device(loamx_pipeline* h, const void* d_corner, uint32_t nc, const void* d_surf, uint32_t ns) {
  return guard([&]() {
    LX_REQUIRE(h && (d_corner || !nc) && (d_surf || !ns), "NULL argument");
    h->p.reg.set_submap_device((const float4*)d_corner, nc, (const float4*)d_surf, ns);
    return LOAMX_OK;
  });
}
int loamx_pipeline_stage_frozen_device(loamx_pipeline* h, const void* d_corner, uint32_t nc, const void* d_surf, uint32_t ns, void* wait_event) {
  return guard([&]() {
    LX_REQUIRE(h && (d_corner || !nc) && (d_surf || !ns), "NULL argument");
    h->p.reg.stage_submap_device((const float4*)d_corner, nc, (const float4*)d_surf, ns, (hipEvent_t)wait_event);
    return LOAMX_OK;
  });
}
int loamx_pipeline_stage_frozen(loamx_pipeline* h, const loamx_cloud* corner_map, const loamx_cloud* surf_map) {
  return guard([&]() {
    LX_REQUIRE(h, "NULL handle");
    h->p.reg.stage_submap_host(corner_map, surf_map);
    return LOAMX_OK;
  });
}
int loamx_pipeline_swap_frozen(loamx_pipeline* h) {
  return guard([&]() {
    LX_REQUIRE(h, "NULL handle");
    if (!h->p.reg.submap_staged()) return (int)LOAMX_SKIPPED;
    h->p.reg.swap_submap();
    return (int)LOAMX_OK;
  });
}
int loamx_pipeline_set_state(loamx_pipeline* h, uint32_t stream, const float* transform, const float* transform_sum, const float* bef,
                             const float* aft) {
  return guard([&]() {
    LX_REQUIRE(h && stream < h->p.n_streams_, "invalid stream");
    h->p.park_odometry(-1);
    if (transform) h->p.OB(stream).stream_state(h->p.LS(stream)).transform.set(transform);
    if (transform_sum) h->p.OB(stream).stream_state(h->p.LS(stream)).transform_sum.set(transform_sum);
    if (bef) h->p.st[stream].bef.set(bef);
    if (aft) h->p.st[stream].aft.set(aft);
    return LOAMX_OK;
  });
}
int loamx_pipeline_upload(loamx_pipeline* h, uint32_t n_steps, const loamx_cloud* clouds, const uint32_t* const* ring_size,
                          const uint32_t* n_rings) {
  return guard([&]() { LX_REQUIRE(h, "NULL handle"); h->p.upload(n_steps, clouds, ring_size, n_rings); return LOAMX_OK; });
}
int loamx_pipeline_stage_step(loamx_pipeline* h, uint32_t step, const loamx_cloud* clouds, const uint32_t* const* ring_size, const uint32_t* n_rings) {
  return guard([&]() { LX_REQUIRE(h, "NULL handle"); h->p.stage_step(step, clouds, ring_size, n_rings); return LOAMX_OK; });
}
int loamx_pipeline_stage_step_raw(loamx_pipeline* h, uint32_t step, const void* const* raw_xyz, const uint32_t* counts, uint32_t stride,
                                  const loamx_multiscan_mapper* mapper, const double* scan_time_sec) {
  return guard([&]() {
    LX_REQUIRE(h && mapper, "NULL argument");
    h->p.stage_step_raw(step, raw_xyz, counts, stride, *mapper, scan_time_sec);
    return LOAMX_OK;
  });
}
int loamx_pipeline_stage_step_sensor(loamx_pipeline* h, uint32_t step, const void* const* records, const uint32_t* counts, uint32_t stride,
                                     const loamx_sensor_model* m, const double* scan_time_sec) {
  return guard([&]() {
    LX_REQUIRE(h && m, "NULL argument");
    h->p.stage_step_sensor(step, records, counts, stride, *m, scan_time_sec);
    return LOAMX_OK;
  });
}
int loamx_pipeline_update_imu(loamx_pipeline* h, uint32_t stream, double stamp_sec, float roll, float pitch, float yaw, const float acc_xyz[3]) {
  return guard([&]() {
    LX_REQUIRE(h && acc_xyz && stream < h->p.n_streams_, "invalid argument");
    h->p.imu[stream].update(stamp_sec, roll, pitch, yaw, acc_xyz);
    h->p.map_imu_push(stream, stamp_sec, roll, pitch);
    return LOAMX_OK;
  });
}
int loamx_pipeline_enable_async_downloads(loamx_pipeline* h) {
  return guard([&]() { LX_REQUIRE(h, "NULL handle"); h->p.reg.double_buffer_full = true; return LOAMX_OK; });
}
int loamx_pipeline_download_step_async(loamx_pipeline* h, loamx_cloud* out, uint32_t n_out) {
  return guard([&]() { LX_REQUIRE(h, "NULL handle"); h->p.download_step_async(out, n_out); return LOAMX_OK; });
}
int loamx_pipeline_download_counts(loamx_pipeline* h, uint64_t counts[2]) {
  return guard([&]() {
    LX_REQUIRE(h && counts, "NULL argument");
    counts[0] = h->p.downloads_direct;
    counts[1] = h->p.downloads_hip;
    return LOAMX_OK;
  });
}
int loamx_pipeline_wait_downloads(loamx_pipeline* h) {
  return guard([&]() { LX_REQUIRE(h, "NULL handle"); h->p.wait_downloads(); return LOAMX_OK; });
}
int loamx_pipeline_step(loamx_pipeline* h, uint32_t step) {
  return guard([&]() { LX_REQUIRE(h, "NULL handle"); return h->p.step(step); });
}
int loamx_pipeline_get(loamx_pipeline* h, uint32_t stream, float* transform, float* transform_sum, float* aft, int* stats8) {
  return guard([&]() {
    LX_REQUIRE(h && stream < h->p.n_streams_, "invalid stream");
    PipeStreamState& P = h->p.st[stream];
    const OdomPub& O = P.cur;
    if (transform) O.transform.get(transform);
    if (transform_sum) O.transform_sum.get(transform_sum);
    if (aft) P.aft.get(aft);
    if (stats8) {
      stats8[0] = O.stats.iterations; stats8[1] = O.stats.sel; stats8[2] = P.map_stats.iterations; stats8[3] = P.map_stats.sel;
      stats8[4] = P.map_stats.corner_q; stats8[5] = P.map_stats.surf_q; stats8[6] = P.map_stats.degenerate; stats8[7] = P.mapped ? 1 : 0;
    }
    return LOAMX_OK;
  });
}
int loamx_pipeline_download_full_res(loamx_pipeline* h, uint32_t slot, loamx_cloud* out) {
  return guard([&]() { LX_REQUIRE(h && out, "NULL argument"); return h->p.reg.download_full_res(slot, out); });
}
int loamx_pipeline_download_last_clouds(loamx_pipeline* h, uint32_t stream, loamx_cloud* last_corner, loamx_cloud* last_surf) {
  return guard([&]() {
    LX_REQUIRE(h && last_corner && last_surf, "NULL argument");
    LX_REQUIRE(stream < h->p.n_streams_, "stream index out of range");
    LX_REQUIRE(h->p.last_step.load() >= 0, "no step has run");
    check_cloud(last_corner, false);
    check_cloud(last_surf, false);
    LX_HIP(hipSetDevice(h->p.device));
    const OdomPub& N = h->p.st[stream].cur;
    std::vector<float4> tmp(std::max(N.n_last_corner, N.n_last_surf));
    if (N.n_last_corner) LX_HIP(hipMemcpy(tmp.data(), N.last_corner, sizeof(float4) * N.n_last_corner, hipMemcpyDeviceToHost));
    const int rc = unpack_cloud(tmp.data(), N.n_last_corner, last_corner);
    if (N.n_last_surf) LX_HIP(hipMemcpy(tmp.data(), N.last_surf, sizeof(float4) * N.n_last_surf, hipMemcpyDeviceToHost));
    const int rs = unpack_cloud(tmp.data(), N.n_last_surf, last_surf);
    return rc != LOAMX_OK ? rc : rs;
  });
}
int loamx_pipeline_set_lookahead(loamx_pipeline* h, int on) {
  return guard([&]() {
    LX_REQUIRE(h, "NULL handle");
    if (!on && h->p.prefetch) h->p.park_odometry(-1);
    h->p.prefetch = on != 0;
    return LOAMX_OK;
  });
}
int loamx_pipeline_drain_lookahead(loamx_pipeline* h, int* last_odometry_step) {
  return guard([&]() {
    LX_REQUIRE(h, "NULL handle");
    const int done = h->p.drain_lookahead();
    if (last_odometry_step) *last_odometry_step = done;
    return LOAMX_OK;
  });
}
int loamx_pipeline_set_timing(loamx_pipeline* h, int on) {
  return guard([&]() {
    LX_REQUIRE(h, "NULL handle");
    h->p.timing = on != 0;
    h->p.reg.set_timing(on != 0, on != 2);
    for (auto& c : h->p.chains) c->ob->set_launch_timing(on != 0 && on != 2);
    return LOAMX_OK;
  });
}
int loamx_pipeline_get_odom_launch_timing(loamx_pipeline* h, double ms4[4], uint64_t counts7[7]) {
  return guard([&]() {
    LX_REQUIRE(h && ms4 && counts7, "NULL argument");
    for (int k = 0; k < 4; k++) ms4[k] = 0.0;
    for (int k = 0; k < 7; k++) counts7[k] = 0;
    for (auto& c : h->p.chains) {
      const OdometryBatch::LaunchTotals t = c->ob->launch_totals();
      ms4[0] += t.lm_ms; ms4[1] += t.lm_noop_ms; ms4[2] += t.corr_ms; ms4[3] += t.corr_noop_ms;
      counts7[0] += t.lm_launches; counts7[1] += t.lm_noop_launches; counts7[2] += t.lm_iterations; counts7[3] += t.corr_launches;
      counts7[4] += t.corr_noop_launches; counts7[5] += t.lm_bytes; counts7[6] += t.corr_features;
    }
    return LOAMX_OK;
  });
}
int loamx_pipeline_get_timing(loamx_pipeline* h, float stage_ms[4], float reg_ms[4], uint64_t counts[4]) {
  return guard([&]() {
    LX_REQUIRE(h && stage_ms && reg_ms && counts, "NULL argument");
    for (int k = 0; k < 4; k++) stage_ms[k] = h->p.last_ms[k];
    h->p.reg.get_timing(reg_ms, counts);
    return LOAMX_OK;
  });
}
int loamx_pipeline_lookahead_depth(loamx_pipeline* h) { return h ? h->p.depth() : 0; }
void* loamx_pipeline_stream(loamx_pipeline* h) { return h ? (void*)h->p.reg.stream() : nullptr; }

}

void loamx_pipeline_dense_source(loamx_pipeline* h, uint32_t slot, loamx::DenseSource& out) {
  LX_REQUIRE(h, "NULL pipeline");
  Pipeline& P = h->p;
  out = loamx::DenseSource{};
  out.stream = P.reg.stream();
  out.device = P.device;
  const uint32_t nw = P.last_full_off.empty() ? 0u : (uint32_t)P.last_full_off.size() - 1;
  if (!nw) return;
  LX_REQUIRE(slot < nw, "slot beyond the streams registered in the last step");
  out.pts = P.reg.d_full_res() + P.last_full_off[slot];
  out.n = P.last_full_off[slot + 1] - P.last_full_off[slot];
  const HTwist& aft = P.st[P.last_who[slot]].aft;
  out.origin[0] = aft.pos.x; out.origin[1] = aft.pos.y; out.origin[2] = aft.pos.z;
  out.has_cloud = true;
}
```

loam_velodyne_amd/csrc/registration.hip:

```cpp
#include "registration.hpp"
#include "pinned_copy.hpp"
#include <atomic>
#include <chrono>
#include "scan.hpp"
#include "voxel.hpp"

namespace loamx {

__global__ __launch_bounds__(256) void k_stack(const float4* __restrict__ in, const float4* const* __restrict__ src, uint32_t n,
                                               const uint32_t* __restrict__ seg_off, uint32_t nseg, const Pose* __restrict__ poses,
                                               float inv_corner, float inv_surf, float4* __restrict__ stack, int* __restrict__ ijk,
                                               int* __restrict__ seg_minmax) {
  const uint32_t i = blockIdx.x * blockDim.x + threadIdx.x;
  const bool active = i < n;
  uint32_t seg = 0;
  int ix = 0, iy = 0, iz = 0;
  if (active) {
    seg = vox_find_seg(seg_off, nseg, i);
    const Pose T = poses[seg >> 1];
    const float4 p = src ? src[seg][i - seg_off[seg]] : in[i];
    float x = p.x, y = p.y, z = p.z;
    to_map(T, x, y, z);
    to_be_mapped(T, x, y, z);
    stack[i] = make_float4(x, y, z, p.w);
// ... 228 lines not shown
      SweepStats st = sSt;
      st.iterations = iter + 1;
      st.sel = sel_rows;
      st.corner_q = (int)(ds_off[2 * s + 1] - ds_off[2 * s]);
      st.surf_q = (int)(ds_off[2 * s + 2] - ds_off[2 * s + 1]);
      stats[s] = st;
      if (host_stats) mirror_to_host(host_stats + s, host_poses + s, st, sP);
    }
    return;
  }
  SOLVE_TS(2);
  if (tid < 64) qr_solve6_coop(AtA, AtB, X);
  else if (tid == 64 && iter == 0) s_cert = certainly_not_degenerate(AtA, 100.f) ? 1 : 0;
  __syncthreads();
  SOLVE_TS(3);
  float* P = matP + 36 * s;
  if (tid == 0) {
    if (iter == 0) sSt.degenerate = s_cert ? 0 : (degeneracy_projector_full(AtA, 100.f, P, ws) ? 1 : 0);
    if (sSt.degenerate) {
      for (int r = 0; r < 6; r++) X2[r] = X[r];
      for (int r = 0; r < 6; r++) {
        float acc = 0.f;
        for (int c = 0; c < 6; c++) acc += P[r * 6 + c] * X2[c];
        X[r] = acc;
      }
    }
  }
  __syncthreads();
  SOLVE_TS(4);
  if (tid < 6) {
    const float ang = (tid < 2 ? sP.rx : (tid < 4 ? sP.ry : sP.rz)) + X[tid >> 1];
    trig[tid] = (float)((tid & 1) ? cos((double)ang) : sin((double)ang));
  }
  __syncthreads();
  SOLVE_TS(5);
  if (tid != 0) return;
  SweepStats st = sSt;
  st.iterations = iter + 1;
  st.sel = sel_rows;
  st.corner_q = (int)(ds_off[2 * s + 1] - ds_off[2 * s]);
  st.surf_q = (int)(ds_off[2 * s + 2] - ds_off[2 * s + 1]);
  Pose T = sP;
  T.rx = T.rx + X[0]; T.ry = T.ry + X[1]; T.rz = T.rz + X[2];
  T.srx = trig[0]; T.crx = trig[1]; T.sry = trig[2]; T.cry = trig[3]; T.srz = trig[4]; T.crz = trig[5];
  T.tx += X[3]; T.ty += X[4]; T.tz += X[5];
  poses[s] = T;
  const float d0 = (float)(X[0] * 180.0 / M_PI), d1 = (float)(X[1] * 180.0 / M_PI), d2 = (float)(X[2] * 180.0 / M_PI);
  const float deltaR = (float)sqrt((double)d0 * d0 + (double)d1 * d1 + (double)d2 * d2);
  const float t0 = X[3] * 100, t1 = X[4] * 100, t2 = X[5] * 100;
  const float deltaT = (float)sqrt((double)t0 * t0 + (double)t1 * t1 + (double)t2 * t2);
  if (deltaR < delta_r_abort && deltaT < delta_t_abort) st.done = 1;
  stats[s] = st;
  if (host_stats) mirror_to_host(host_stats + s, host_poses + s, st, T);
  SOLVE_TS(6);
}

#ifndef KNN_LPQ
#define KNN_LPQ 4
#endif
#ifndef KNN_MLP
#define KNN_MLP 4
#endif
template <int NR, int MLP, int LPQ>
__device__ __forceinline__ void knn_scan_group(const float4* __restrict__ pts, const uint32_t (&beg)[NR], const uint32_t (&len)[NR], float qx, float qy,
                                      float qz, int gl, unsigned long long (&bk)[6], uint32_t (&bp)[6]) {
  uint32_t E[NR], O[NR];
  uint32_t acc = 0;
#pragma unroll
  for (int k = 0; k < NR; k++) {
    O[k] = beg[k] - acc;
    acc += len[k];
    E[k] = acc;
  }
  const uint32_t total = acc;
  for (uint32_t c0 = (uint32_t)gl; c0 < total; c0 += MLP * LPQ) {
    uint32_t pos[MLP];
    float4 p[MLP];
#pragma unroll
    for (int u = 0; u < MLP; u++) {
      const uint32_t cc = c0 + u * LPQ;
      uint32_t o = O[NR - 1];
#pragma unroll
      for (int k = NR - 2; k >= 0; k--) o = cc < E[k] ? O[k] : o;
      pos[u] = cc < total ? cc + o : 0u;
    }
#pragma unroll
    for (int u = 0; u < MLP; u++) p[u] = pts[pos[u]];
#pragma unroll
    for (int u = 0; u < MLP; u++) {
      const float dx = qx - p[u].x, dy = qy - p[u].y, dz = qz - p[u].z;
      const float d2 = dx * dx + dy * dy + dz * dz;
      const bool ok = (c0 + u * LPQ) < total && d2 < KNN_COVER2;
      const unsigned long long key = ok ? ((unsigned long long)__float_as_uint(d2) << 32) | __float_as_uint(p[u].w) : KNN_NONE;
      knn_insert6(bk, bp, key, pos[u]);
    }
  }
}

__device__ __forceinline__ float knn_gap(float f, int c, int d) {
  const float v = d > 0 ? (float)(c + 1) - f : f - (float)c;
  const float w = v * 0.9999f - 1e-5f;
  return w > 0.f ? w : 0.f;
}

template <int LPQ, int QB>
__device__ __forceinline__ void knn5_group(const GridDesc& g, const float4* __restrict__ pts, const uint32_t* __restrict__ cell_start, float qx, float qy,
                                  float qz, int gl, uint32_t* tab, unsigned long long (&wk)[6], uint32_t (&win)[6]) {
#pragma unroll
  for (int j = 0; j < 6; j++) { wk[j] = KNN_NONE; win[j] = 0u; }
  const float fx = (qx - g.ox) * g.inv_h, fy = (qy - g.oy) * g.inv_h, fz = (qz - g.oz) * g.inv_h;
  const float flx = floorf(fx), fly = floorf(fy), flz = floorf(fz);
  if (!(flx >= -2.f && flx <= (float)(g.nx + 1) && fly >= -2.f && fly <= (float)(g.ny + 1) && flz >= -2.f && flz <= (float)(g.nz + 1))) return;
  const int cx = (int)flx, cy = (int)fly, cz = (int)flz;
  const int sx = (fx - flx) < 0.5f ? -1 : 1, sy = (fy - fly) < 0.5f ? -1 : 1, sz = (fz - flz) < 0.5f ? -1 : 1;
  {
    uint32_t v[(36 + LPQ - 1) / LPQ];
#pragma unroll
    for (int i = 0; i < (36 + LPQ - 1) / LPQ; i++) {
      const int e = gl + LPQ * i;
      const int r = e >> 2, k = e & 3, a = r / 3, b = r - 3 * a;
      const int z = cz + (a == 1 ? sz : (a == 2 ? -sz : 0)), y = cy + (b == 1 ? sy : (b == 2 ? -sy : 0));
      const bool in = e < 36 && z >= 0 && z < g.nz && y >= 0 && y < g.ny;
      v[i] = in ? cell_start[((uint32_t)z * g.ny + y) * g.nx + clampi(cx - 1 + k, 0, g.nx)] : 0u;
    }
#pragma unroll
    for (int i = 0; i < (36 + LPQ - 1) / LPQ; i++) {
      const int e = gl + LPQ * i;
      if (e < 36) tab[e * QB] = v[i];
    }
  }
  __builtin_amdgcn_wave_barrier();
  unsigned long long bk[6];
  uint32_t bp[6];
#pragma unroll
  for (int j = 0; j < 6; j++) { bk[j] = KNN_NONE; bp[j] = 0u; }
  const int kn = sx < 0 ? 0 : 1;
  {
    uint32_t beg[4], len[4];
#pragma unroll
    for (int i = 0; i < 4; i++) {
      const int r = i < 2 ? i : i + 1;
      const uint32_t lo = tab[(4 * r + kn) * QB], hi = tab[(4 * r + kn + 2) * QB];
      beg[i] = lo;
      len[i] = hi - lo;
    }
    knn_scan_group<4, KNN_MLP, LPQ>(pts, beg, len, qx, qy, qz, gl, bk, bp);
  }
  knn_pop6<LPQ>(bk, bp, gl, wk, win);
  {
    const float rad2 = wk[5] != KNN_NONE ? __uint_as_float((uint32_t)(wk[5] >> 32)) : KNN_COVER2;
    const float r2c = rad2 * g.inv_h * g.inv_h;
    const float gx_near = knn_gap(fx, cx, sx), gx_far = knn_gap(fx, cx, -sx);
    const float gxl = sx < 0 ? gx_near : gx_far, gxr = sx < 0 ? gx_far : gx_near;
    const float gy[3] = {0.f, knn_gap(fy, cy, sy), knn_gap(fy, cy, -sy)};
    const float gz[3] = {0.f, knn_gap(fz, cz, sz), knn_gap(fz, cz, -sz)};
    uint32_t beg[9], len[9];
#pragma unroll
    for (int a = 0; a < 3; a++)
#pragma unroll
      for (int b = 0; b < 3; b++) {
        const int r = 3 * a + b;
        const float gyz = gy[b] * gy[b] + gz[a] * gz[a];
        uint32_t lo = 0u, hi = 0u;
        if (a < 2 && b < 2) {
          if (gyz + gx_far * gx_far < r2c) { lo = tab[(4 * r + 2 - 2 * kn) * QB]; hi = tab[(4 * r + 3 - 2 * kn) * QB]; }
        } else if (gyz < r2c) {
          lo = tab[(4 * r + ((gyz + gxl * gxl < r2c) ? 0 : 1)) * QB];
          hi = tab[(4 * r + ((gyz + gxr * gxr < r2c) ? 3 : 2)) * QB];
        }
        beg[r] = lo;
        len[r] = hi - lo;
      }
#pragma unroll
    for (int k = 0; k < 6; k++) { bk[k] = gl == 0 ? wk[k] : KNN_NONE; bp[k] = win[k]; }
    knn_scan_group<9, KNN_MLP, LPQ>(pts, beg, len, qx, qy, qz, gl, bk, bp);
  }
  knn_pop6<LPQ>(bk, bp, gl, wk, win);
}

struct GnArgs {
  const float4* ds_pts;
  const uint32_t* ds_off;
  Pose* poses;
  SweepStats* stats;
  const GridDesc* cdesc;
  const float4* cpts;
  const uint32_t* cstart;
  const GridDesc* sdesc;
  const float4* spts;
  const uint32_t* sstart;
  double* partials;
  uint32_t* arrive;
  float* matP;
  SweepStats* host_stats;
  Pose* host_poses;
  uint32_t nblk;
  unsigned long long* dbg;
  int iter;
  float delta_t_abort, delta_r_abort;
  const uint32_t* skip_word;
  uint32_t skip_value;
};

constexpr int GN_TILE = LX_RES_THREADS / KNN_LPQ;
#ifdef LOAMX_PROF_GN
#define GN_TS(k) do { if (blockIdx.y == 0 && tid == 0 && A.iter == 0) A.dbg[(size_t)tile * 8 + (k)] = wall_clock64(); } while (0)
#else
#define GN_TS(k) do { } while (0)
#endif

#ifndef GN_WAVES
#define GN_WAVES 6
#endif
#define GN_KERNEL k_gn_iter
#define GN_JACOBI false
#include "gn_iter_kernel.inc"
#undef GN_KERNEL
#undef GN_JACOBI
#ifdef LOAMX_DIAG
#define GN_KERNEL k_gn_iter_jacobi
#define GN_JACOBI true
#include "gn_iter_kernel.inc"
#undef GN_KERNEL
#undef GN_JACOBI
#endif

__global__ __launch_bounds__(256) void k_knn_probe(const float4* __restrict__ queries, uint32_t n, const GridDesc* __restrict__ desc,
                                                   const float4* __restrict__ pts, const uint32_t* __restrict__ cell_start,
                                                   uint32_t* __restrict__ idx5, float* __restrict__ d2_5) {
  constexpr int QB = 256 / KNN_LPQ;
  __shared__ uint32_t tab[36 * QB];
  const int grp = threadIdx.x / KNN_LPQ, gl = threadIdx.x % KNN_LPQ;
  const uint32_t q = blockIdx.x * QB + grp;
  if (q >= n) return;
  const float4 p = queries[q];
  unsigned long long wk[6];
  uint32_t win[6];
  knn5_group<KNN_LPQ, QB>(*desc, pts, cell_start, p.x, p.y, p.z, gl, tab + grp, wk, win);
  if (gl != 0) return;
#pragma unroll
  for (int j = 0; j < 5; j++) {
    idx5[5 * (size_t)q + j] = wk[j] != KNN_NONE ? (uint32_t)(wk[j] & 0xffffffffull) : 0xffffffffu;
    d2_5[5 * (size_t)q + j] = wk[j] != KNN_NONE ? __uint_as_float((uint32_t)(wk[j] >> 32)) : FLT_MAX;
  }
}

__global__ __launch_bounds__(256) void k_transform_full(float4* __restrict__ full, uint32_t n, const uint32_t* __restrict__ full_off,
                                                        uint32_t ns, const Pose* __restrict__ poses, const SweepStats* __restrict__ stats,
                                                        uint32_t* __restrict__ full_done, int mode, uint32_t tag,
                                                        const uint32_t* __restrict__ skip_word, uint32_t skip_value) {
  uint32_t i = blockIdx.x * blockDim.x + threadIdx.x;
  if (i >= n) return;
  if (skip_word && *skip_word == skip_value) return;
  const uint32_t s = vox_find_seg(full_off, ns, i);
  if (mode == 1) {
    if (!stats[s].done) return;
    if (i == full_off[s]) full_done[s] = tag;
  } else if (mode == 2) {
    if (full_done[s] != 0u) return;
  }
  const Pose T = poses[s];
  float4 p = full[i];
  to_map(T, p.x, p.y, p.z);
  full[i] = p;
}

__global__ __launch_bounds__(256) void k_gather_segments(float4* __restrict__ dst, const uint32_t* __restrict__ off, uint32_t nseg,
                                                         const float4* const* __restrict__ src, uint32_t n) {
  const uint32_t i = blockIdx.x * blockDim.x + threadIdx.x;
  if (i >= n) return;
  const uint32_t k = vox_find_seg(off, nseg, i);
  dst[i] = src[k][i - off[k]];
}

struct ParamBlock1 { uint32_t w[18]; };
__global__ __launch_bounds__(256) void k_gather_one(float4* __restrict__ dst, const float4* __restrict__ src, uint32_t n, ParamBlock1 blk,
                                                    uint32_t* __restrict__ blk_dst) {
  if (blockIdx.x == 0 && threadIdx.x < 18) blk_dst[threadIdx.x] = blk.w[threadIdx.x];
  const uint32_t i = blockIdx.x * blockDim.x + threadIdx.x;
  if (i < n) dst[i] = src[i];
}

Registrar::Registrar(int device, uint32_t max_sweeps) : device_(device), max_sweeps_(max_sweeps) {
  select_device(device);
  st_ = create_stream(env_priority("LOAMX_PRIO_REG", +1), 0, 1);
  corner_index.init(st_);
  surf_index.init(st_);
  poses_.reserve(max_sweeps);
  stats_.reserve(max_sweeps);
  matP_.reserve((size_t)36 * max_sweeps);
  arrive_.reserve(max_sweeps);
  LX_HIP(hipMemsetAsync(arrive_.p, 0, sizeof(uint32_t) * max_sweeps, st_));
  guess_.reserve((size_t)6 * max_sweeps);
  ds_off_.reserve(2 * max_sweeps + 2);
  vox_.init(st_);
  vb_.init(st_);
  vb_disabled_ = getenv("LOAMX_VOX_LEGACY") != nullptr;
  jacobi_eig_ = diag_env("LOAMX_EIG_JACOBI") != nullptr;
  full_done_.reserve(max_sweeps);
  h_stats_.reserve(max_sweeps);
  h_poses_.reserve(max_sweeps);
  ev_.resize(2 + 2 * 64);
  for (auto& e : ev_) LX_HIP(hipEventCreate(&e));
}

Registrar::~Registrar() {
  for (auto& e : ev_) (void)hipEventDestroy(e);
  if (ev_build_) (void)hipEventDestroy(ev_build_);
  if (ev_swap_) (void)hipEventDestroy(ev_swap_);
  if (ev_look_) (void)hipEventDestroy(ev_look_);
  if (st_build_) { (void)hipStreamSynchronize(st_build_); (void)hipStreamDestroy(st_build_); }
  if (st_) (void)hipStreamDestroy(st_);
}

void Registrar::set_submap_host(const loamx_cloud* corner, const loamx_cloud* surf) {
  check_cloud(corner, false);
  check_cloud(surf, false);
  LX_HIP(hipSetDevice(device_));
  PinBuf<float4> hc, hs;
  hc.reserve(corner->count);
  hs.reserve(surf->count);
  pack_cloud(corner, hc.p);
  pack_cloud(surf, hs.p);
  own_corner_.reserve(corner->count);
  own_surf_.reserve(surf->count);
  LX_HIP(hipMemcpyAsync(own_corner_.p, hc.p, sizeof(float4) * corner->count, hipMemcpyHostToDevice, st_));
  LX_HIP(hipMemcpyAsync(own_surf_.p, hs.p, sizeof(float4) * surf->count, hipMemcpyHostToDevice, st_));
  corner_index.build(own_corner_.p, corner->count);
  surf_index.build(own_surf_.p, surf->count);
  LX_HIP(hipStreamSynchronize(st_));
}

void Registrar::set_submap_device(const float4* d_corner, uint32_t nc, const float4* d_surf, uint32_t ns, bool sync) {
  LX_HIP(hipSetDevice(device_));
  corner_index.build(d_corner, nc);
  surf_index.build(d_surf, ns);
  if (sync) LX_HIP(hipStreamSynchronize(st_));
}

void Registrar::set_submap_device_split(const float4* d_corner, uint32_t nc, hipStream_t corner_stream, const float4* d_surf, uint32_t ns, bool bounds_done) {
  LX_HIP(hipSetDevice(device_));
  corner_index.bind(corner_stream);
  corner_index.build(d_corner, nc, bounds_done);
  corner_index.bind(st_);
  surf_index.build(d_surf, ns, bounds_done);
}

void Registrar::stage_submap_device(const float4* d_corner, uint32_t nc, const float4* d_surf, uint32_t ns, hipEvent_t wait_for) {
  LX_HIP(hipSetDevice(device_));
  if (!st_build_) {
    st_build_ = create_stream(0);
    LX_HIP(hipEventCreateWithFlags(&ev_build_, hipEventDisableTiming));
    LX_HIP(hipEventCreateWithFlags(&ev_swap_, hipEventDisableTiming));
    corner_next_.init(st_build_);
    surf_next_.init(st_build_);
  }
  if (swapped_once_) LX_HIP(hipStreamWaitEvent(st_build_, ev_swap_, 0));
  if (wait_for) LX_HIP(hipStreamWaitEvent(st_build_, wait_for, 0));
  corner_next_.bind(st_build_);
  surf_next_.bind(st_build_);
  corner_next_.build(d_corner, nc);
  surf_next_.build(d_surf, ns);
  LX_HIP(hipEventRecord(ev_build_, st_build_));
  next_staged_ = true;
}

void Registrar::stage_submap_host(const loamx_cloud* corner, const loamx_cloud* surf) {
  check_cloud(corner, false);
  check_cloud(surf, false);
  LX_HIP(hipSetDevice(device_));
  if (st_build_) LX_HIP(hipStreamSynchronize(st_build_));
  h_next_corner_.reserve(corner->count + 1);
  h_next_surf_.reserve(surf->count + 1);
  pack_cloud(corner, h_next_corner_.p);
  pack_cloud(surf, h_next_surf_.p);
  next_corner_.reserve(corner->count + 1);
  next_surf_.reserve(surf->count + 1);
  if (!st_build_) stage_submap_device(nullptr, 0, nullptr, 0);
  LX_HIP(hipMemcpyAsync(next_corner_.p, h_next_corner_.p, sizeof(float4) * corner->count, hipMemcpyHostToDevice, st_build_));
  LX_HIP(hipMemcpyAsync(next_surf_.p, h_next_surf_.p, sizeof(float4) * surf->count, hipMemcpyHostToDevice, st_build_));
  stage_submap_device(next_corner_.p, corner->count, next_surf_.p, surf->count);
}

void Registrar::swap_submap() {
  LX_REQUIRE(next_staged_, "swap_submap() without a staged sub-map");
  LX_HIP(hipSetDevice(device_));
  LX_HIP(hipStreamWaitEvent(st_, ev_build_, 0));
  LX_HIP(hipEventRecord(ev_swap_, st_));
  corner_index.swap(corner_next_);
  surf_index.swap(surf_next_);
  corner_index.bind(st_);
  surf_index.bind(st_);
  next_staged_ = false;
  swapped_once_ = true;
}

template <class Count> static void prefix_offsets(std::vector<uint32_t>& off, uint32_t n, Count&& count) {
  off.assign(n + 1, 0);
  for (uint32_t s = 0; s < n; s++) off[s + 1] = off[s] + count(s);
}

template <class Count> void Registrar::plan_inputs_(uint32_t n_sweeps, bool staged, Count&& count) {
  LX_REQUIRE(n_sweeps >= 1 && n_sweeps <= max_sweeps_, "n_sweeps out of range for this handle");
  LX_HIP(hipSetDevice(device_));
  n_sweeps_ = n_sweeps;
  h_seg_off_.assign(2 * n_sweeps + 1, 0);
  if (!staged) h_full_off_.assign(n_sweeps + 1, 0);
  max_q_per_sweep_ = 0;
  for (uint32_t s = 0; s < n_sweeps; s++) {
    const uint32_t nc = count(s, 0), nf = count(s, 1);
    h_seg_off_[2 * s + 1] = h_seg_off_[2 * s] + nc;
    h_seg_off_[2 * s + 2] = h_seg_off_[2 * s + 1] + nf;
    max_q_per_sweep_ = std::max(max_q_per_sweep_, nc + nf);
    if (!staged) h_full_off_[s + 1] = h_full_off_[s] + count(s, 2);
  }
  n_in_ = h_seg_off_[2 * n_sweeps];
  if (!staged) n_full_ = h_full_off_[n_sweeps];
  in_.reserve(n_in_ + 1);
  stack_.reserve(n_in_ + 1);
  ds_pts_.reserve(n_in_ + 1);
  vox_.reserve(n_in_ + 1, 2 * n_sweeps);
  LX_REQUIRE(n_in_ < SCAN_MAX_N, "too many feature points in one batch");
  if (n_full_) full_.reserve(n_full_);
  nblk_ = max_q_per_sweep_ / GN_TILE + 2;
  partials_.reserve((size_t)n_sweeps * nblk_ * LX_NSUM);
}

size_t Registrar::write_param_block_(const float* guess6, const float4* const* corner_src, const float4* const* surf_src, const float4* const* full_src) {
  const uint32_t ns = n_sweeps_;
  const size_t nseg = 2 * (size_t)ns;
  const size_t o_off = sizeof(float) * 6 * ns, o_full = o_off + sizeof(uint32_t) * (nseg + 1);
  const size_t end_full = o_full + sizeof(uint32_t) * (ns + 1), o_src = (end_full + 15) & ~(size_t)15;
  const size_t bytes = corner_src ? o_src + sizeof(float4*) * (nseg + ns) : end_full;
  h_blob_.reserve(bytes + 16);
  blob_.reserve(bytes + 16);
  memcpy(h_blob_.p, guess6, sizeof(float) * 6 * ns);
  memcpy(h_blob_.p + o_off, h_seg_off_.data(), sizeof(uint32_t) * (nseg + 1));
  memcpy(h_blob_.p + o_full, h_full_off_.data(), sizeof(uint32_t) * (ns + 1));
  if (corner_src) {
    const float4** hsrc = (const float4**)(h_blob_.p + o_src);
    for (uint32_t s = 0; s < ns; s++) { hsrc[2 * s] = corner_src[s]; hsrc[2 * s + 1] = surf_src[s]; }
    for (uint32_t s = 0; s < ns; s++) hsrc[nseg + s] = full_src ? full_src[s] : nullptr;
  }
  d_guess_ = (const float*)blob_.p;
  d_seg_off_ = (const uint32_t*)(blob_.p + o_off);
  d_full_off_ = (const uint32_t*)(blob_.p + o_full);
  d_src_ = corner_src ? (const float4* const*)(blob_.p + o_src) : nullptr;
  return bytes;
}

void Registrar::upload(uint32_t n_sweeps, const loamx_cloud* corner_last, const loamx_cloud* surf_last, const loamx_cloud* full_res,
                       const float* guess6, bool wait) {
  LX_REQUIRE(corner_last && surf_last && guess6, "NULL input");
  plan_inputs_(n_sweeps, false, [&](uint32_t s, int k) {
    const loamx_cloud* c = k == 0 ? &corner_last[s] : k == 1 ? &surf_last[s] : full_res ? &full_res[s] : nullptr;
    if (!c) return 0u;
    check_cloud(c, false);
    return c->count;
  });
  h_in_.reserve(n_in_ + 1);
  for (uint32_t s = 0; s < n_sweeps; s++) {
    pack_cloud(&corner_last[s], h_in_.p + h_seg_off_[2 * s]);
    pack_cloud(&surf_last[s], h_in_.p + h_seg_off_[2 * s + 1]);
  }
  if (!packed_all_finite(h_in_.p, n_in_)) throw Error(LOAMX_E_INVALID, "a feature cloud holds non-finite coordinates");
  fetch_from_pinned(in_.p, h_in_.p, n_in_, st_);
  if (n_full_) {
    h_full_.reserve(n_full_);
    for (uint32_t s = 0; s < n_sweeps; s++) pack_cloud(&full_res[s], h_full_.p + h_full_off_[s]);
    fetch_from_pinned(full_.p, h_full_.p, n_full_, st_);
  }
  const size_t bytes = write_param_block_(guess6, nullptr, nullptr, nullptr);
  LX_HIP(hipMemcpyAsync(blob_.p, h_blob_.p, bytes, hipMemcpyHostToDevice, st_));
  if (wait) LX_HIP(hipStreamSynchronize(st_));
}

float4* Registrar::stage_full(uint32_t n_sweeps, const uint32_t* n_full) {
  LX_REQUIRE(n_sweeps >= 1 && n_sweeps <= max_sweeps_, "n_sweeps out of range for this handle");
  full_next_staged_ = false;
  prefix_offsets(h_full_off_, n_sweeps, [&](uint32_t s) { return n_full[s]; });
  n_full_ = h_full_off_[n_sweeps];
  if (double_buffer_full) {
    std::swap(full_.p, full_alt_.p);
    std::swap(full_.cap, full_alt_.cap);
  }
  full_.reserve((size_t)n_full_ + 1);
  full_staged_ = true;
  return full_.p;
}

float4* Registrar::stage_full_next(uint32_t n_sweeps, const uint32_t* n_full) {
  LX_REQUIRE(double_buffer_full, "internal: pre-staging needs the second full-resolution buffer");
  LX_REQUIRE(n_sweeps >= 1 && n_sweeps <= max_sweeps_, "n_sweeps out of range for this handle");
  prefix_offsets(next_full_off_, n_sweeps, [&](uint32_t s) { return n_full[s]; });
  if ((size_t)next_full_off_[n_sweeps] + 1 > full_alt_.cap) return nullptr;
  full_next_staged_ = true;
  return full_alt_.p;
}
bool Registrar::adopt_full_next(uint32_t n_sweeps, const uint32_t* n_full) {
  if (!full_next_staged_ || next_full_off_.size() != n_sweeps + 1) { full_next_staged_ = false; return false; }
  for (uint32_t s = 0; s < n_sweeps; s++)
    if (next_full_off_[s + 1] - next_full_off_[s] != n_full[s]) { full_next_staged_ = false; return false; }
  full_next_staged_ = false;
  h_full_off_ = next_full_off_;
  n_full_ = h_full_off_[n_sweeps];
  std::swap(full_.p, full_alt_.p);
  std::swap(full_.cap, full_alt_.cap);
  full_staged_ = true;
  return true;
}

void Registrar::upload_device(uint32_t n_sweeps, const float4* const* corner_last, const uint32_t* n_corner,
                              const float4* const* surf_last, const uint32_t* n_surf, const float4* const* full_res,
                              const uint32_t* n_full, const float* guess6) {
  const bool staged = full_staged_ && !full_res;
  full_staged_ = false;
  plan_inputs_(n_sweeps, staged, [&](uint32_t s, int k) { return k == 0 ? n_corner[s] : k == 1 ? n_surf[s] : full_res ? n_full[s] : 0u; });
  const size_t bytes = write_param_block_(guess6, corner_last, surf_last, full_res);
  if (n_sweeps == 1 && n_full_ && !staged && bytes == sizeof(ParamBlock1)) {
    ParamBlock1 pb1;
    memcpy(pb1.w, h_blob_.p, sizeof(pb1));
    hipLaunchKernelGGL(k_gather_one, dim3((n_full_ + 255) / 256), dim3(256), 0, st_, full_.p, full_res[0], n_full_, pb1, (uint32_t*)blob_.p);
  } else {
    LX_HIP(hipMemcpyAsync(blob_.p, h_blob_.p, bytes, hipMemcpyHostToDevice, st_));
    if (n_full_ && !staged)
      hipLaunchKernelGGL(k_gather_segments, dim3((n_full_ + 255) / 256), dim3(256), 0, st_, full_.p, d_full_off_, n_sweeps, d_src_ + 2 * (size_t)n_sweeps,
                         n_full_);
  }
}

static double host_us() {
  return std::chrono::duration<double, std::micro>(std::chrono::steady_clock::now().time_since_epoch()).count();
}
struct Registrar::RunTrace {
  bool on;
  double t0, front = 0, first_gn = 0, callback = 0;
  int looks = 0;
};
#ifdef LOAMX_PROF_GN
static DevBuf<unsigned long long> g_gn_dbg;
#endif

void Registrar::enqueue_full(int mode) {
  if (!n_full_) return;
  if (mode == 1 && ++full_tag_ == 0u) full_tag_ = 1u;
  const uint32_t* skip = run_.vb_unchecked ? vb_.d_fail_word() : nullptr;
  hipLaunchKernelGGL(k_transform_full, dim3((n_full_ + 255) / 256), dim3(256), 0, st_, full_.p, n_full_, d_full_off_, n_sweeps_, poses_.p,
                     stats_.p, full_done_.p, mode, full_tag_, skip, vb_.epoch());
}

void Registrar::enqueue_front(bool legacy) {
  const uint32_t ns = n_sweeps_, nseg = 2 * ns, n = n_in_;
  hipLaunchKernelGGL(k_pose_init, dim3((ns + 63) / 64), dim3(64), 0, st_, d_guess_, ns, poses_.p, stats_.p, vox_.seg_minmax(), arrive_.p,
                     full_done_.p);
  if (n == 0) {
    LX_HIP(hipMemsetAsync(ds_off_.p, 0, sizeof(uint32_t) * (nseg + 1), st_));
    return;
  }
  if (legacy) {
    const uint32_t nb = (n + 255) / 256;
    hipLaunchKernelGGL(k_stack, dim3(nb), dim3(256), 0, st_, in_.p, d_src_, n, d_seg_off_, nseg, poses_.p, 1.0f / params.corner_leaf,
                       1.0f / params.surf_leaf, stack_.p, vox_.ijk(), vox_.seg_minmax());
    vox_.sort_reduce(stack_.p, nullptr, n, d_seg_off_, nseg, ds_pts_.p, ds_off_.p);
  } else {
    vb_.run(in_.p, d_src_, n, d_seg_off_, h_seg_off_.data(), nseg, poses_.p, 1.0f / params.corner_leaf, 1.0f / params.surf_leaf, stack_.p,
            ds_pts_.p, ds_off_.p);
  }
}

bool Registrar::wait_for_mirrors() {
  const bool no_poll = diag_env("LOAMX_NO_MIRROR_POLL") != nullptr;
  if (no_poll) { LX_HIP(hipEventSynchronize(ev_look_)); return false; }
  const uint32_t ns = n_sweeps_;
  const volatile SweepStats* hs = h_stats_.p;
  for (unsigned spin = 0;; spin++) {
    bool all = true;
    for (uint32_t k = 0; k < ns && all; k++) all = hs[k].done != 0;
    if (all) {
      std::atomic_thread_fence(std::memory_order_acquire);
      for (uint32_t k = 0; k < ns && all; k++) {
        SweepStats st;
        Pose T;
        memcpy(&st, (const void*)&h_stats_.p[k], sizeof(st));
        memcpy(&T, (const void*)&h_poses_.p[k], sizeof(T));
        all = st.pad1 == mirror_check_word(st, T);
      }
      if (all) return true;
    }
    if ((spin & 15) == 15) {
      const hipError_t q = hipEventQuery(ev_look_);
      if (q == hipSuccess) return false;
      if (q != hipErrorNotReady) LX_HIP(q);
    }
    cpu_relax();
  }
}

RegOutcome Registrar::run_iterations(RunTrace& tr) {
  TraceRange trace_range("loamx:registration:gauss-newton");
  GnArgs a;
  a.ds_pts = ds_pts_.p; a.ds_off = ds_off_.p; a.poses = poses_.p; a.stats = stats_.p;
  a.cdesc = corner_index.desc(); a.cpts = corner_index.sorted(); a.cstart = corner_index.cell_start();
  a.sdesc = surf_index.desc(); a.spts = surf_index.sorted(); a.sstart = surf_index.cell_start();
  a.partials = partials_.p; a.arrive = arrive_.p; a.matP = matP_.p;
  a.host_stats = h_stats_.p; a.host_poses = h_poses_.p;
  a.nblk = nblk_; a.delta_t_abort = params.delta_t_abort; a.delta_r_abort = params.delta_r_abort;
  a.dbg = nullptr;
  a.skip_word = run_.vb_unchecked ? vb_.d_fail_word() : nullptr;
  a.skip_value = vb_.epoch();
#ifdef LOAMX_PROF_GN
  g_gn_dbg.reserve((size_t)nblk_ * 8 + 64);
  LX_HIP(hipMemsetAsync(g_gn_dbg.p, 0, sizeof(unsigned long long) * ((size_t)nblk_ * 8 + 64), st_));
  a.dbg = g_gn_dbg.p;
#endif
  struct Ops {
    Registrar& r;
    GnArgs& a;
    RunTrace& tr;
    const dim3 grid;
    void gn(int it) {
      const bool tm = r.timing_ && r.launch_timing_ && r.n_res_launch_ < 64;
      if (tm) LX_HIP(hipEventRecord(r.ev_[2 + 2 * r.n_res_launch_], r.st_));
      a.iter = it;
#ifdef LOAMX_DIAG
      if (r.jacobi_eig_) hipLaunchKernelGGL(k_gn_iter_jacobi, grid, dim3(LX_RES_THREADS), 0, r.st_, a);
      else
#endif
      hipLaunchKernelGGL(k_gn_iter, grid, dim3(LX_RES_THREADS), 0, r.st_, a);
      if (tm) {
        LX_HIP(hipEventRecord(r.ev_[3 + 2 * r.n_res_launch_], r.st_));
        r.n_res_launch_++;
      }
    }
    void full(int mode) { r.enqueue_full(mode); }
    void mark() {
      if (tr.on && tr.first_gn == 0) tr.first_gn = host_us();
      if (!r.ev_look_) LX_HIP(hipEventCreateWithFlags(&r.ev_look_, hipEventDisableTiming));
      LX_HIP(hipEventRecord(r.ev_look_, r.st_));
    }
    void first_wait() {
      if (r.on_first_wait) { r.on_first_wait(); r.on_first_wait = nullptr; }
    }
    RegLook look() {
      if (tr.on && tr.callback == 0) tr.callback = host_us();
      r.wait_for_mirrors();
      RegLook l{r.bucket_stage_gave_up_(), true, 0};
      for (uint32_t k = 0; k < r.n_sweeps_ && !l.gave_up; k++) {
        l.all_done = l.all_done && r.h_stats_.p[k].done;
        l.need = std::max(l.need, r.h_stats_.p[k].iterations);
      }
      return l;
    }
  } ops{*this, a, tr, dim3(8 * ((nblk_ + 7) / 8 + 1), n_sweeps_)};
  static const int ahead = diag_env("LOAMX_GN_AHEAD") ? std::max(0, atoi(diag_env("LOAMX_GN_AHEAD"))) : 1;
  const RegOutcome o = reg_schedule(ops, RegPlan{early_exit, params.max_iterations, pred_iters_, ahead, n_full_ != 0 && !defer_full});
  pred_iters_ = o.pred_iters_next;
  run_.mirrors_written = run_.results_final = o.all_done;
  tr.looks = o.looks;
#ifdef LOAMX_PROF_GN
  dump_gn_profile_();
#endif
  return o;
}

#ifdef LOAMX_PROF_GN
void Registrar::dump_gn_profile_() {
  std::vector<unsigned long long> h((size_t)nblk_ * 8);
  (void)hipStreamSynchronize(st_);
  (void)hipMemcpy(h.data(), g_gn_dbg.p, sizeof(unsigned long long) * h.size(), hipMemcpyDeviceToHost);
  unsigned long long t0 = ~0ull;
  for (uint32_t t = 0; t < nblk_; t++) if (h[8 * t]) t0 = std::min(t0, h[8 * t]);
  fprintf(stderr, "[gn iter 0, sweep 0: tile: start / search / rows / reduce us (+solve)]");
  for (uint32_t t = 0; t < nblk_; t++) {
    const unsigned long long* v = &h[8 * t];
    if (!v[0]) continue;
    if (t % 16 == 0 || v[5]) fprintf(stderr, " %u:%.0f/%.0f/%.0f/%.0f", t, (v[0] - t0) * 0.01, (v[1] - v[0]) * 0.01, (v[2] - v[1]) * 0.01, (v[3] - v[2]) * 0.01);
    if (v[5]) fprintf(stderr, "(+solve %.0f, ends at %.0f)", (v[5] - v[4]) * 0.01, (v[5] - t0) * 0.01);
  }
  fprintf(stderr, "\n");
  unsigned long long ts[16];
  (void)hipMemcpyFromSymbol(ts, HIP_SYMBOL(g_solve_ts), sizeof(ts));
  fprintf(stderr, "[solve_sweep, us since entry] partial sums %.1f  sums+AtA %.1f  qr %.1f  projector %.1f  trig %.1f  update+stores %.1f\n", (ts[1] - ts[0]) * 0.01,
          (ts[2] - ts[0]) * 0.01, (ts[3] - ts[0]) * 0.01, (ts[4] - ts[0]) * 0.01, (ts[5] - ts[0]) * 0.01, (ts[6] - ts[0]) * 0.01);
}
#endif

void Registrar::begin_attempt_(bool legacy) {
  if (timing_) LX_HIP(hipEventRecord(ev_[0], st_));
  n_res_launch_ = 0;
  if (early_exit) memset(h_stats_.p, 0, sizeof(SweepStats) * n_sweeps_);
  run_ = Run{};
  run_.vb_unchecked = !legacy && n_in_ > 0;
}

void Registrar::run_async(bool force_general) {
  LX_REQUIRE(n_sweeps_ > 0, "run() before upload()");
  TraceRange trace_range("loamx:registration");
  static const bool trace = getenv("LOAMX_REG_TRACE") != nullptr;
  RunTrace tr{trace, trace ? host_us() : 0.0};
  LX_HIP(hipSetDevice(device_));
  const bool can_bucket = !force_general && !vb_disabled_ && VoxBucket::fits(n_in_, 2 * n_sweeps_);
  RegOutcome o;
  for (int attempt = 0; attempt < 2; attempt++) {
    const bool legacy = attempt == 1 || !can_bucket;
    begin_attempt_(legacy);
    enqueue_front(legacy);
    if (trace) tr.front = host_us();
    o = RegOutcome{};
    if (submap_sufficient() && n_in_ > 0) {
      o = run_iterations(tr);
      if (trace && tr.first_gn == 0) tr.first_gn = host_us();
    }
    bool again = o.gave_up;
    if (!again && early_exit && run_.vb_unchecked) {
      LX_HIP(hipStreamSynchronize(st_));
      again = bucket_stage_gave_up_();
    }
    if (!again) break;
  }
  if (n_full_ && !defer_full && !o.full_enqueued) enqueue_full(0);
  if (timing_) { LX_HIP(hipEventRecord(ev_[1], st_)); timed_run_ = true; }
  LX_HIP(hipGetLastError());
  if (on_first_wait) on_first_wait();
  if (trace && tr.callback == 0) tr.callback = host_us();
  if (trace)
    fprintf(stderr, "[reg] voxel stage enqueued %.0f us, first iterations enqueued %.0f, callback done %.0f, run_async returns %.0f, looks %d\n",
            tr.front - tr.t0, tr.first_gn - tr.t0, tr.callback - tr.t0, host_us() - tr.t0, tr.looks);
}

bool Registrar::bucket_stage_gave_up_() {
  if (!run_.vb_unchecked) return false;
  run_.vb_unchecked = false;
  if (!vb_.failed()) return false;
  static const bool trace = getenv("LOAMX_VB_TRACE") != nullptr;
  if (trace) fprintf(stderr, "[voxbucket] gave up (reason mask 0x%x, %u points, %u sweeps): repeating through the general kernel\n", vb_.why(), n_in_, n_sweeps_);
  return true;
}

void Registrar::redo_if_bucket_path_failed() {
  if (!bucket_stage_gave_up_()) return;
  run_async(true);
  LX_HIP(hipStreamSynchronize(st_));
}

void Registrar::finish_with_poses(const float* poses6) {
  const uint32_t ns = n_sweeps_;
  h_guess_.reserve((size_t)6 * ns + 8);
  memcpy(h_guess_.p, poses6, sizeof(float) * 6 * ns);
  guess_.reserve((size_t)6 * ns + 8);
  LX_HIP(hipMemcpyAsync(guess_.p, h_guess_.p, sizeof(float) * 6 * ns, hipMemcpyHostToDevice, st_));
  hipLaunchKernelGGL(k_pose_set, dim3((ns + 63) / 64), dim3(64), 0, st_, guess_.p, ns, poses_.p);
  enqueue_full(0);
  const bool owed = run_.vb_unchecked;
  run_ = Run{};
  run_.vb_unchecked = owed;
  LX_HIP(hipGetLastError());
}

void Registrar::knn_probe(int which, const float* xyz, uint32_t n, uint32_t* idx5, float* d2_5) {
  LX_REQUIRE(which == 0 || which == 1, "which must be 0 (corner sub-map) or 1 (surf sub-map)");
  LX_REQUIRE(xyz && idx5 && d2_5, "NULL argument");
  SubMapIndex& ix = which == 0 ? corner_index : surf_index;
  LX_REQUIRE(ix.size() >= 1, "the sub-map is empty");
  LX_HIP(hipSetDevice(device_));
  if (!n) return;
  DevBuf<float4> dq;
  DevBuf<uint32_t> di;
  DevBuf<float> dd;
  dq.reserve(n); di.reserve((size_t)5 * n); dd.reserve((size_t)5 * n);
  std::vector<float4> hq(n);
  for (uint32_t i = 0; i < n; i++) hq[i] = make_float4(xyz[3 * i], xyz[3 * i + 1], xyz[3 * i + 2], 0.f);
  LX_HIP(hipMemcpyAsync(dq.p, hq.data(), sizeof(float4) * n, hipMemcpyHostToDevice, st_));
  hipLaunchKernelGGL(k_knn_probe, dim3((n + 256 / KNN_LPQ - 1) / (256 / KNN_LPQ)), dim3(256), 0, st_, dq.p, n, ix.desc(), ix.sorted(), ix.cell_start(), di.p, dd.p);
  LX_HIP(hipMemcpyAsync(idx5, di.p, sizeof(uint32_t) * 5 * n, hipMemcpyDeviceToHost, st_));
  LX_HIP(hipMemcpyAsync(d2_5, dd.p, sizeof(float) * 5 * n, hipMemcpyDeviceToHost, st_));
  LX_HIP(hipStreamSynchronize(st_));
}

__global__ __launch_bounds__(64) void k_qr6_probe(const float* __restrict__ ata, const float* __restrict__ atb, uint32_t n, float* __restrict__ x_coop,
                                                  float* __restrict__ x_scalar) {
  __shared__ float A[36], B[6], X[6];
  const uint32_t i = blockIdx.x;
  const int tid = (int)threadIdx.x;
  if (tid < 36) A[tid] = ata[36 * (size_t)i + tid];
  if (tid < 6) { B[tid] = atb[6 * (size_t)i + tid]; X[tid] = 0.f; }
  __syncthreads();
  qr_solve6_coop(A, B, X);
  __syncthreads();
  if (tid < 6) x_coop[6 * (size_t)i + tid] = X[tid];
  if (tid == 0) {
    float M[6][6], b[6], x[6];
    for (int r = 0; r < 6; r++) {
      b[r] = B[r];
      for (int c = 0; c < 6; c++) M[r][c] = A[r * 6 + c];
    }
    qr_solve<6, 6>(M, b, x);
    for (int r = 0; r < 6; r++) x_scalar[6 * (size_t)i + r] = x[r];
  }
}
void Registrar::qr6_probe(const float* ata, const float* atb, uint32_t n, float* x_coop, float* x_scalar) {
  LX_REQUIRE(ata && atb && x_coop && x_scalar, "NULL argument");
  LX_HIP(hipSetDevice(device_));
  if (!n) return;
  DevBuf<float> da, db, dx, dy;
  da.reserve((size_t)36 * n); db.reserve((size_t)6 * n); dx.reserve((size_t)6 * n); dy.reserve((size_t)6 * n);
  LX_HIP(hipMemcpyAsync(da.p, ata, sizeof(float) * 36 * n, hipMemcpyHostToDevice, st_));
  LX_HIP(hipMemcpyAsync(db.p, atb, sizeof(float) * 6 * n, hipMemcpyHostToDevice, st_));
  hipLaunchKernelGGL(k_qr6_probe, dim3(n), dim3(64), 0, st_, da.p, db.p, n, dx.p, dy.p);
  LX_HIP(hipMemcpyAsync(x_coop, dx.p, sizeof(float) * 6 * n, hipMemcpyDeviceToHost, st_));
  LX_HIP(hipMemcpyAsync(x_scalar, dy.p, sizeof(float) * 6 * n, hipMemcpyDeviceToHost, st_));
  LX_HIP(hipStreamSynchronize(st_));
}

__device__ __forceinline__ double xrec_probe_value(unsigned k) {
  return __hiloint2double((int)(k * 2654435761u ^ 0x5bd1e995u), (int)(~k * 40503u + 0x9e3779b9u));
}
__global__ __launch_bounds__(64) void k_xrec_stress(xrec_t* __restrict__ rec, unsigned rounds, unsigned long long* __restrict__ out) {
  const unsigned p = blockIdx.x >> 1, t = threadIdx.x;
  xrec_t* r = rec + (size_t)p * 64 + t;
  if ((blockIdx.x & 1u) == 0u) {
    for (unsigned k = 1; k <= rounds; k++) xrec_store(r, xrec_probe_value(k), k);
    asm volatile("s_waitcnt vmcnt(0)" ::: "memory");
    return;
  }
  unsigned long long acc = 0, torn = 0, bad = 0, late = 0;
  const unsigned long long t0 = wall_clock64();
  unsigned last = 0, polls = 0;
  while (last != rounds) {
    const xrec_t v = xrec_load(r);
    if (v.x == v.w) {
      if (v.x != 0u) {
        acc++;
        const double want = xrec_probe_value(v.x);
        if (__double2hiint(xrec_value(v)) != __double2hiint(want) || __double2loint(xrec_value(v)) != __double2loint(want)) bad++;
        last = v.x;
      }
    } else {
      torn++;
    }
    if ((++polls & 4095u) == 0u && wall_clock64() - t0 > 300000000ull) { late = 1; break; }
  }
  atomicAdd(&out[0], acc); atomicAdd(&out[1], torn); atomicAdd(&out[2], bad); atomicAdd(&out[3], late);
}
void Registrar::xrec_stress(uint32_t pairs, uint32_t rounds, unsigned long long out4[4]) {
  LX_REQUIRE(out4 && pairs >= 1 && pairs <= 512 && rounds >= 1, "invalid argument");
  LX_HIP(hipSetDevice(device_));
  DevBuf<xrec_t> rec;
  DevBuf<unsigned long long> out;
  rec.reserve((size_t)pairs * 64);
  out.reserve(4);
  LX_HIP(hipMemsetAsync(rec.p, 0, sizeof(xrec_t) * pairs * 64, st_));
  LX_HIP(hipMemsetAsync(out.p, 0, sizeof(unsigned long long) * 4, st_));
  hipLaunchKernelGGL(k_xrec_stress, dim3(2 * pairs), dim3(64), 0, st_, rec.p, rounds, out.p);
  LX_HIP(hipMemcpyAsync(out4, out.p, sizeof(unsigned long long) * 4, hipMemcpyDeviceToHost, st_));
  LX_HIP(hipStreamSynchronize(st_));
}

void Registrar::sync() { wait_stream(st_); }

void Registrar::fetch_results() {
  const bool seen_final = run_.results_final && !run_.vb_unchecked;
  if (!seen_final) LX_HIP(hipStreamSynchronize(st_));
  vox_.check();
  vb_.check();
  scan_check_errors();
  if (seen_final) return;
  redo_if_bucket_path_failed();
  if (!run_.mirrors_written) {
    LX_HIP(hipMemcpyAsync(h_poses_.p, poses_.p, sizeof(Pose) * n_sweeps_, hipMemcpyDeviceToHost, st_));
    LX_HIP(hipMemcpyAsync(h_stats_.p, stats_.p, sizeof(SweepStats) * n_sweeps_, hipMemcpyDeviceToHost, st_));
    LX_HIP(hipStreamSynchronize(st_));
    run_.mirrors_written = true;
  }
}

void Registrar::download_stats(SweepStats* out) {
  fetch_results();
  memcpy(out, h_stats_.p, sizeof(SweepStats) * n_sweeps_);
}

void Registrar::download(float* poses6, int* stats4) {
  LX_REQUIRE(n_sweeps_ > 0, "download() before run()");
  fetch_results();
  for (uint32_t s = 0; s < n_sweeps_; s++) {
    if (poses6) {
      const Pose& T = h_poses_.p[s];
      float* o = poses6 + 6 * s;
      o[0] = T.rx; o[1] = T.ry; o[2] = T.rz; o[3] = T.tx; o[4] = T.ty; o[5] = T.tz;
    }
    if (stats4) {
      const SweepStats& st = h_stats_.p[s];
      int* o = stats4 + 4 * s;
      o[0] = st.iterations; o[1] = st.sel; o[2] = st.corner_q; o[3] = st.surf_q;
    }
  }
}

void Registrar::download_full_res_async(uint32_t sweep, const loamx_cloud* into) {
  LX_REQUIRE(sweep < n_sweeps_, "sweep index out of range");
  const uint32_t a = h_full_off_[sweep], b = h_full_off_[sweep + 1];
  run_.full_dl_direct = nullptr;
  if (into && b > a && into->count >= b - a && packed_layout(into) && host_pinned(into->data, sizeof(float4) * (b - a))) {
    LX_HIP(hipMemcpyAsync(into->data, full_.p + a, sizeof(float4) * (b - a), hipMemcpyDeviceToHost, st_));
    run_.full_dl_direct = into->data;
  } else {
    h_full_dl_.reserve((size_t)(b - a) + 1);
    if (b > a) LX_HIP(hipMemcpyAsync(h_full_dl_.p, full_.p + a, sizeof(float4) * (b - a), hipMemcpyDeviceToHost, st_));
  }
  run_.full_dl_sweep = (int)sweep;
}

int Registrar::download_full_res(uint32_t sweep, loamx_cloud* out) {
  LX_REQUIRE(sweep < n_sweeps_, "sweep index out of range");
  check_cloud(out, false);
  fetch_results();
  const uint32_t a = h_full_off_[sweep], b = h_full_off_[sweep + 1];
  const bool landed = run_.full_dl_sweep == (int)sweep && run_.full_dl_direct && run_.full_dl_direct == out->data;
  if (run_.full_dl_sweep != (int)sweep || (run_.full_dl_direct && !landed)) {
    h_full_dl_.reserve((size_t)(b - a) + 1);
    if (b > a) LX_HIP(hipMemcpyAsync(h_full_dl_.p, full_.p + a, sizeof(float4) * (b - a), hipMemcpyDeviceToHost, st_));
  }
  run_.full_dl_sweep = -1;
  run_.full_dl_direct = nullptr;
  wait_stream(st_);
  if (landed) { out->count = b - a; return LOAMX_OK; }
  return unpack_cloud(h_full_dl_.p, b - a, out);
}

void Registrar::download_ds(uint32_t sweep, std::vector<float4>& corner_ds, std::vector<float4>& surf_ds) {
  LX_REQUIRE(sweep < n_sweeps_, "sweep index out of range");
  fetch_results();
  uint32_t off[3];
  LX_HIP(hipMemcpyAsync(off, ds_off_.p + 2 * sweep, sizeof(off), hipMemcpyDeviceToHost, st_));
  LX_HIP(hipStreamSynchronize(st_));
  corner_ds.resize(off[1] - off[0]);
  surf_ds.resize(off[2] - off[1]);
  if (!corner_ds.empty())
    LX_HIP(hipMemcpyAsync(corner_ds.data(), ds_pts_.p + off[0], sizeof(float4) * corner_ds.size(), hipMemcpyDeviceToHost, st_));
  if (!surf_ds.empty())
    LX_HIP(hipMemcpyAsync(surf_ds.data(), ds_pts_.p + off[1], sizeof(float4) * surf_ds.size(), hipMemcpyDeviceToHost, st_));
  LX_HIP(hipStreamSynchronize(st_));
}

void Registrar::download_ds_counts(uint32_t sweep, uint32_t counts[2]) {
  LX_REQUIRE(sweep < n_sweeps_ && counts, "sweep index out of range");
  fetch_results();
  uint32_t off[3];
  LX_HIP(hipMemcpyAsync(off, ds_off_.p + 2 * sweep, sizeof(off), hipMemcpyDeviceToHost, st_));
  LX_HIP(hipStreamSynchronize(st_));
  counts[0] = off[1] - off[0];
  counts[1] = off[2] - off[1];
}

void Registrar::get_timing(float ms[4], uint64_t counts[4]) {
  for (int k = 0; k < 4; k++) { ms[k] = 0.f; counts[k] = 0; }
  if (!timing_ || !timed_run_) return;
  LX_HIP(hipEventSynchronize(ev_[1]));
  LX_HIP(hipEventElapsedTime(&ms[0], ev_[0], ev_[1]));
  for (int k = 0; k < n_res_launch_; k++) {
    float t = 0.f;
    LX_HIP(hipEventElapsedTime(&t, ev_[2 + 2 * k], ev_[3 + 2 * k]));
    ms[1] += t;
  }
  counts[0] = n_res_launch_;
  std::vector<SweepStats> st(n_sweeps_);
  download_stats(st.data());
  for (auto& s : st) {
    counts[1] += (uint64_t)s.iterations * (uint64_t)(s.corner_q + s.surf_q);
    counts[2] += (uint64_t)(s.corner_q + s.surf_q);
  }
}

}
```

loam_velodyne_amd/csrc/registration.hpp:

```cpp
#pragma once
#include <functional>
#include "common.h"
#include "dev_math.hpp"
#include "reg_schedule.hpp"
#include "submap_index.hpp"
#include "voxel.hpp"
#include "voxbucket.hpp"

namespace loamx {

constexpr int LX_RES_THREADS = 256;
constexpr int LX_NSUM = 28;

struct SweepStats {
  int iterations, sel, corner_q, surf_q, degenerate, done, pad0, pad1;
};

__host__ __device__ inline int mirror_check_word(const SweepStats& st, const Pose& T) {
  const unsigned* w = reinterpret_cast<const unsigned*>(&T);
  unsigned x = 0x5bd1e995u ^ (unsigned)st.iterations ^ ((unsigned)st.sel << 8) ^ ((unsigned)st.degenerate << 30);
  for (int i = 0; i < (int)(sizeof(Pose) / 4); i++) x = (x << 5 | x >> 27) ^ w[i];
  return (int)x;
}

struct RegParams {
  int max_iterations = 10;
  float delta_t_abort = 0.05f, delta_r_abort = 0.05f;
  float corner_leaf = 0.2f, surf_leaf = 0.4f;
};

class Registrar {
 public:
  Registrar(int device, uint32_t max_sweeps);
  ~Registrar();
  RegParams params;
  SubMapIndex corner_index, surf_index;
  void stage_submap_device(const float4* d_corner, uint32_t nc, const float4* d_surf, uint32_t ns, hipEvent_t wait_for = nullptr);
  void stage_submap_host(const loamx_cloud* corner, const loamx_cloud* surf);
  bool submap_staged() const { return next_staged_; }
  void swap_submap();
  bool double_buffer_full = false;
  bool defer_full = false;
  void finish_with_poses(const float* poses6);
  std::function<void()> on_first_wait;
  bool early_exit = false;
  hipStream_t stream() const { return st_; }

  void set_submap_host(const loamx_cloud* corner, const loamx_cloud* surf);
  void set_submap_device(const float4* d_corner, uint32_t nc, const float4* d_surf, uint32_t ns, bool sync = true);

  void upload(uint32_t n_sweeps, const loamx_cloud* corner_last, const loamx_cloud* surf_last, const loamx_cloud* full_res,
              const float* guess6, bool wait = true);
  void upload_device(uint32_t n_sweeps, const float4* const* corner_last, const uint32_t* n_corner, const float4* const* surf_last,
                     const uint32_t* n_surf, const float4* const* full_res, const uint32_t* n_full, const float* guess6);
  float4* stage_full(uint32_t n_sweeps, const uint32_t* n_full);
  float4* stage_full_next(uint32_t n_sweeps, const uint32_t* n_full);
  bool adopt_full_next(uint32_t n_sweeps, const uint32_t* n_full);
  void run_async(bool force_general = false);
  void sync();
  void download(float* poses6, int* stats4);
  void download_stats(SweepStats* out);
  int download_full_res(uint32_t sweep, loamx_cloud* out);
  void download_full_res_async(uint32_t sweep, const loamx_cloud* into = nullptr);
  void set_submap_device_split(const float4* d_corner, uint32_t nc, hipStream_t corner_stream, const float4* d_surf, uint32_t ns, bool bounds_done = false);
  void download_ds(uint32_t sweep, std::vector<float4>& corner_ds, std::vector<float4>& surf_ds);
  void download_ds_counts(uint32_t sweep, uint32_t counts[2]);
  const float4* d_ds_points() const { return ds_pts_.p; }
  const uint32_t* d_ds_offsets() const { return ds_off_.p; }
  const Pose* d_poses() const { return poses_.p; }
  const float4* d_full_res() const { return full_.p; }
  uint32_t full_offset(uint32_t s) const { return h_full_off_[s]; }

  void knn_probe(int which, const float* xyz, uint32_t n, uint32_t* idx5, float* d2_5);
  void qr6_probe(const float* ata, const float* atb, uint32_t n, float* x_coop, float* x_scalar);
  void xrec_stress(uint32_t pairs, uint32_t rounds, unsigned long long out4[4]);
  void set_timing(bool on, bool per_launch = true) { timing_ = on; launch_timing_ = per_launch; }
  void get_timing(float ms[4], uint64_t counts[4]);
  uint32_t n_sweeps() const { return n_sweeps_; }
  bool submap_sufficient() const { return corner_index.size() > 10 && surf_index.size() > 100; }

 private:
  int device_;
  uint32_t max_sweeps_, n_sweeps_ = 0;
  hipStream_t st_ = nullptr;
  bool timing_ = false, timed_run_ = false, launch_timing_ = true;

  DevBuf<float4> own_corner_, own_surf_;

  PinBuf<float4> h_in_, h_full_;
  std::vector<uint32_t> h_seg_off_, h_full_off_;
  PinBuf<float> h_guess_;
  DevBuf<float4> in_, stack_, ds_pts_, full_, full_alt_;
  DevBuf<uint32_t> ds_off_;
  DevBuf<float> guess_;
  bool full_staged_ = false, full_next_staged_ = false;
  std::vector<uint32_t> next_full_off_;
  hipEvent_t ev_look_ = nullptr;
  PinBuf<float4> h_full_dl_;
  struct Run {
    bool vb_unchecked = false;
    bool mirrors_written = false;
    bool results_final = false;
    int full_dl_sweep = -1;
    void* full_dl_direct = nullptr;
  } run_;
  VoxelPipeline vox_;
  VoxBucket vb_;
  bool vb_disabled_ = false;
  bool jacobi_eig_ = false;
  void enqueue_front(bool legacy);
  void enqueue_full(int mode);
  void redo_if_bucket_path_failed();
  uint32_t n_in_ = 0, n_full_ = 0, max_q_per_sweep_ = 0;
  struct RunTrace;
  template <class Count> void plan_inputs_(uint32_t n_sweeps, bool staged, Count&& count);
  size_t write_param_block_(const float* guess6, const float4* const* corner_src, const float4* const* surf_src, const float4* const* full_src);
  void begin_attempt_(bool legacy);
  RegOutcome run_iterations(RunTrace& tr);
  bool bucket_stage_gave_up_();
  void dump_gn_profile_();
  bool wait_for_mirrors();
  void fetch_results();
  int pred_iters_ = 4;

  DevBuf<Pose> poses_;
  DevBuf<SweepStats> stats_;
  DevBuf<float> matP_;
  DevBuf<double> partials_;
  const float* d_guess_ = nullptr;
  const uint32_t* d_seg_off_ = nullptr;
  const uint32_t* d_full_off_ = nullptr;
  const float4* const* d_src_ = nullptr;
  DevBuf<char> blob_;
  PinBuf<char> h_blob_;
  SubMapIndex corner_next_, surf_next_;
  DevBuf<float4> next_corner_, next_surf_;
  PinBuf<float4> h_next_corner_, h_next_surf_;
  hipStream_t st_build_ = nullptr;
  hipEvent_t ev_build_ = nullptr, ev_swap_ = nullptr;
  bool next_staged_ = false, swapped_once_ = false;
  DevBuf<uint32_t> arrive_;
  DevBuf<uint32_t> full_done_;
  uint32_t full_tag_ = 0;
  uint32_t nblk_ = 0;

  std::vector<hipEvent_t> ev_;
  int n_res_launch_ = 0;
  PinBuf<SweepStats> h_stats_;
  PinBuf<Pose> h_poses_;
};

}
```

loam_velodyne_amd/loamx.py:

```python
from __future__ import annotations

import ctypes as C
import os
import numpy as np

_HERE = os.path.dirname(os.path.abspath(__file__))
LIB_PATH = os.environ.get("LOAMX_LIB") or os.path.join(_HERE, "libloamx.so")

OK, SKIPPED, E_INVALID, E_CAPACITY, E_HIP, E_NOGPU, E_UNSUPPORTED, E_INTERNAL = 0, 1, -1, -2, -3, -4, -5, -6


class Cloud(C.Structure):
    _fields_ = [("data", C.c_void_p), ("count", C.c_uint32), ("stride", C.c_uint32),
                ("intensity_offset", C.c_uint32), ("reserved", C.c_uint32)]


class ScanRegConfig(C.Structure):
    _fields_ = [("scan_period", C.c_float), ("n_feature_regions", C.c_int), ("curvature_region", C.c_int),
                ("max_corner_sharp", C.c_int), ("max_surface_flat", C.c_int), ("less_flat_filter_size", C.c_float),
                ("surface_curvature_threshold", C.c_float), ("device", C.c_int), ("max_corner_less_sharp", C.c_int),
                ("imu_history_size", C.c_int)]


class OdomConfig(C.Structure):
# ... 549 lines not shown
    def process(self, feats):
        arrs = [as_points(feats[n]) for n in ("sharp", "less_sharp", "flat", "less_flat")]
        cl = [cloud_of(a) for a in arrs]
        rc = _check(lib().loamx_odom_process(self.h, C.byref(cl[0]), C.byref(cl[1]), C.byref(cl[2]), C.byref(cl[3])))
        self._sizes = (len(arrs[1]), len(arrs[3]))
        return rc

    def process_linked(self, scanreg):
        rc = _check(lib().loamx_odom_process_linked(self.h, scanreg.h))
        self._sizes = (scanreg._linked_n, scanreg._linked_n)
        return rc

    def link_wait(self):
        return _check(lib().loamx_odom_link_wait(self.h))

    def _t(self, fn):
        t = np.zeros(6, np.float32)
        _check(fn(self.h, t.ctypes.data_as(C.c_void_p)))
        return t

    @property
    def transform(self):
        return self._t(lib().loamx_odom_get_transform)

    @property
    def transform_sum(self):
        return self._t(lib().loamx_odom_get_transform_sum)

    def set_transform(self, t6):
        t = np.ascontiguousarray(t6, np.float32)
        _check(lib().loamx_odom_set_transform(self.h, t.ctypes.data_as(C.c_void_p)))

    def set_transform_sum(self, t6):
        t = np.ascontiguousarray(t6, np.float32)
        _check(lib().loamx_odom_set_transform_sum(self.h, t.ctypes.data_as(C.c_void_p)))

    def last_clouds(self):
        c = np.zeros((max(self._sizes[0], 1), 4), np.float32)
        s = np.zeros((max(self._sizes[1], 1), 4), np.float32)
        cc, sc = cloud_of(c), cloud_of(s)
        _check(lib().loamx_odom_get_last_clouds(self.h, C.byref(cc), C.byref(sc)))
        return c[:cc.count].copy(), s[:sc.count].copy()

    def transform_to_end(self, cloud):
        a = as_points(cloud).copy()
        c = cloud_of(a)
        _check(lib().loamx_odom_transform_to_end(self.h, C.byref(c)))
        return a

    def stats(self):
        s = (C.c_int * 4)()
        _check(lib().loamx_odom_get_stats(self.h, s))
        return dict(iterations=s[0], sel=s[1], frame=s[2], degenerate=s[3])


class LaserMapping:

    def __init__(self, **cfg):
        self._c = _cfg(MapConfig, "loamx_map_default_config", **cfg)
        self.h = C.c_void_p(lib().loamx_map_create(C.byref(self._c)))
        if not self.h:
            raise LoamxError(E_INVALID, lib().loamx_last_error().decode())

    def close(self):
        if getattr(self, "h", None):
            lib().loamx_map_destroy(self.h)
            self.h = None

    __del__ = close

    def update_odometry(self, t6):
        t = np.ascontiguousarray(t6, np.float32)
        _check(lib().loamx_map_update_odometry(self.h, t.ctypes.data_as(C.c_void_p)))

    def update_imu(self, stamp, roll, pitch):
        _check(lib().loamx_map_update_imu(self.h, C.c_double(stamp), C.c_float(roll), C.c_float(pitch)))

    def set_time(self, t):
        _check(lib().loamx_map_set_time(self.h, C.c_double(t)))

    def process(self, corner_last, surf_last, full_res=None, inplace=False):
        c, s = as_points(corner_last), as_points(surf_last)
        cc, sc = cloud_of(c), cloud_of(s)
        if full_res is not None:
            f = as_points(full_res) if inplace else as_points(full_res).copy()
            fc = cloud_of(f)
            rc = _check(lib().loamx_map_process(self.h, C.byref(cc), C.byref(sc), C.byref(fc)))
            return rc, f
        rc = _check(lib().loamx_map_process(self.h, C.byref(cc), C.byref(sc), None))
        return rc, None

    def process_linked(self, odometry, full_out=None):
        if full_out is None:
            return _check(lib().loamx_map_process_linked(self.h, odometry.h, None)), None
        fc = cloud_of(full_out)
        rc = _check(lib().loamx_map_process_linked(self.h, odometry.h, C.byref(fc)))
        return rc, full_out[:fc.count]

    def speculation(self):
        c = (C.c_uint64 * 2)()
        _check(lib().loamx_map_get_speculation(self.h, c))
        return int(c[0]), int(c[1])

    def insert(self, corner_last, surf_last, pose6):
        c, s = as_points(corner_last), as_points(surf_last)
        cc, sc = cloud_of(c), cloud_of(s)
        p = np.ascontiguousarray(pose6, np.float32)
        assert p.shape == (6,)
        return _check(lib().loamx_map_insert(self.h, C.byref(cc), C.byref(sc), p.ctypes.data_as(C.c_void_p)))

    def transform(self, which="aft"):
        t = np.zeros(6, np.float32)
        _check(lib().loamx_map_get_transform(self.h, ("aft", "bef", "tobe", "sum").index(which), t.ctypes.data_as(C.c_void_p)))
        return t

    def set_transform(self, which, t6):
        t = np.ascontiguousarray(t6, np.float32)
        _check(lib().loamx_map_set_transform(self.h, ("aft", "bef", "tobe", "sum").index(which), t.ctypes.data_as(C.c_void_p)))

    def set_timing(self, on: bool):
        _check(lib().loamx_map_set_timing(self.h, 1 if on else 0))

    def timing(self):
        ms = (C.c_float * 4)()
        cnt = (C.c_uint64 * 4)()
        _check(lib().loamx_map_get_timing(self.h, ms, cnt))
        return dict(run_ms=ms[0], residual_ms=ms[1], residual_launches=int(cnt[0]), query_iterations=int(cnt[1]), queries=int(cnt[2]))

    def has_fresh_map(self):
        return bool(lib().loamx_map_has_fresh_map(self.h))

    def _get(self, fn, *args, cap=1 << 16):
        while True:
            out = np.zeros((cap, 4), np.float32)
            c = cloud_of(out)
            rc = fn(self.h, *args, C.byref(c))
            if rc == E_CAPACITY:
                cap = int(c.count) + 16
                continue
            _check(rc)
            return out[:c.count].copy()

    def save_snapshot(self, path: str):
        _check(lib().loamx_map_save_snapshot(self.h, path.encode()))

    def load_snapshot(self, path: str):
        _check(lib().loamx_map_load_snapshot(self.h, path.encode()))

    def surround(self):
        return self._get(lib().loamx_map_get_surround)

    def cubes(self, which):
        return self._get(lib().loamx_map_get_cubes, 0 if which == "corner" else 1)

    def load_cubes(self, corner, surf):
        c, s = as_points(corner), as_points(surf)
        cc, sc = cloud_of(c), cloud_of(s)
        _check(lib().loamx_map_load_cubes(self.h, C.byref(cc), C.byref(sc)))

    def stats(self):
        s = (C.c_int * 8)()
        _check(lib().loamx_map_get_stats(self.h, s))
        keys = ("iterations", "sel", "corner_ds", "surf_ds", "corner_from_map", "surf_from_map", "degenerate", "optimized")
        return dict(zip(keys, (int(v) for v in s)))


class Pipeline:

    def __init__(self, n_streams: int, scanreg=None, odom=None, mapping=None):
        self._f = _cfg(ScanRegConfig, "loamx_scanreg_default_config", **(scanreg or {}))
        self._o = _cfg(OdomConfig, "loamx_odom_default_config", **(odom or {}))
        self._m = _cfg(MapConfig, "loamx_map_default_config", **(mapping or {}))
        L = lib()
        L.loamx_pipeline_create.restype = C.c_void_p
        L.loamx_pipeline_stream.restype = C.c_void_p
        self.h = C.c_void_p(L.loamx_pipeline_create(C.byref(self._f), C.byref(self._o), C.byref(self._m), n_streams))
        if not self.h:
            raise LoamxError(E_INVALID, L.loamx_last_error().decode())
        self.n_streams = n_streams
        self._sizes = None

    def close(self):
        if getattr(self, "h", None):
            lib().loamx_pipeline_destroy(self.h)
            self.h = None

    __del__ = close

    def set_frozen(self, corner_map, surf_map):
        c, s = as_points(corner_map), as_points(surf_map)
        cc, sc = cloud_of(c), cloud_of(s)
        _check(lib().loamx_pipeline_set_frozen(self.h, C.byref(cc), C.byref(sc)))

    def set_frozen_device(self, d_corner_ptr, n_corner, d_surf_ptr, n_surf):
        _check(lib().loamx_pipeline_set_frozen_device(self.h, C.c_void_p(d_corner_ptr), n_corner, C.c_void_p(d_surf_ptr), n_surf))

    def stage_frozen_device(self, d_corner_ptr, n_corner, d_surf_ptr, n_surf, wait_event: int = 0):
        _check(lib().loamx_pipeline_stage_frozen_device(self.h, C.c_void_p(d_corner_ptr), n_corner, C.c_void_p(d_surf_ptr), n_surf,
                                                        C.c_void_p(wait_event or None)))

    def stage_frozen(self, corner_map, surf_map):
        cm, sm = as_points(corner_map), as_points(surf_map)
        cc, sc = cloud_of(cm), cloud_of(sm)
        _check(lib().loamx_pipeline_stage_frozen(self.h, C.byref(cc), C.byref(sc)))

    def swap_frozen(self) -> bool:
        return _check(lib().loamx_pipeline_swap_frozen(self.h)) == OK

    def set_state(self, stream, transform=None, transform_sum=None, bef=None, aft=None):
        def p(a):
            if a is None:
                return None
            a = np.ascontiguousarray(a, np.float32)
            keep.append(a)
            return a.ctypes.data_as(C.c_void_p)
        keep = []
        _check(lib().loamx_pipeline_set_state(self.h, stream, p(transform), p(transform_sum), p(bef), p(aft)))

    def upload(self, sweeps):
        n_steps = len(sweeps)
        ns = self.n_streams
        pts, rings = [], []
        for t in range(n_steps):
            assert len(sweeps[t]) == ns
            for s in range(ns):
                pts.append(as_points(sweeps[t][s][0]))
                rings.append(np.ascontiguousarray(sweeps[t][s][1], np.uint32))
        CA = (Cloud * len(pts))(*[cloud_of(a) for a in pts])
        RP = (C.c_void_p * len(pts))(*[r.ctypes.data for r in rings])
        NR = (C.c_uint32 * len(pts))(*[len(r) for r in rings])
        _check(lib().loamx_pipeline_upload(self.h, n_steps, CA, RP, NR))
        self._sizes = [len(a) for a in pts]

    def stage_step(self, t: int, sweeps_t):
        ns = self.n_streams
        assert len(sweeps_t) == ns
        pts = [as_points(sweeps_t[s][0]) for s in range(ns)]
        rings = [np.ascontiguousarray(sweeps_t[s][1], np.uint32) for s in range(ns)]
        CA = (Cloud * ns)(*[cloud_of(a) for a in pts])
        RP = (C.c_void_p * ns)(*[r.ctypes.data for r in rings])
        NR = (C.c_uint32 * ns)(*[len(r) for r in rings])
        _check(lib().loamx_pipeline_stage_step(self.h, t, CA, RP, NR))
        if not hasattr(self, "_staged"):
            self._staged = {}
        self._staged[t % 8] = (pts, rings, CA, RP, NR)

    def stage_step_raw(self, t: int, raws, sensor="VLP-16", mapper=None, scan_times=None):
        ns = self.n_streams
        assert len(raws) == ns
        arrs = [np.ascontiguousarray(r, np.float32).reshape(-1, 3) for r in raws]
        m = MultiScanMapper()
        if mapper is None:
            _check(lib().loamx_multiscan_mapper_preset(sensor.encode(), C.byref(m)))
        else:
            m.lower_bound_deg, m.upper_bound_deg, m.n_scan_rings = float(mapper[0]), float(mapper[1]), int(mapper[2])
        PP = (C.c_void_p * ns)(*[a.ctypes.data if len(a) else None for a in arrs])
        CN = (C.c_uint32 * ns)(*[len(a) for a in arrs])
        st = (C.c_double * ns)(*[float(x) for x in scan_times]) if scan_times is not None else None
        _check(lib().loamx_pipeline_stage_step_raw(self.h, t, PP, CN, 12, C.byref(m), st))
        if not hasattr(self, "_staged"):
            self._staged = {}
        self._staged[t % 8] = (arrs, PP, CN, st)

    def stage_step_sensor(self, t: int, records_list, model: SensorModel, scan_times=None):
        ns = self.n_streams
        assert len(records_list) == ns
        recs = [as_records(r) for r in records_list]
        strides = {r[2] for r in recs if r[1]}
        assert len(strides) <= 1, "every stream's records must have the same stride"
        stride = strides.pop() if strides else recs[0][2]
        PP = (C.c_void_p * ns)(*[r[0].ctypes.data if r[1] else None for r in recs])
        CN = (C.c_uint32 * ns)(*[r[1] for r in recs])
        st = (C.c_double * ns)(*[float(x) for x in scan_times]) if scan_times is not None else None
        _check(lib().loamx_pipeline_stage_step_sensor(self.h, t, PP, CN, stride, C.byref(model), st))
        if not hasattr(self, "_staged"):
            self._staged = {}
        self._staged[t % 8] = (recs, PP, CN, st, model)

    def update_imu(self, stream: int, stamp, roll, pitch, yaw, acc):
        a = np.ascontiguousarray(acc, np.float32)
        _check(lib().loamx_pipeline_update_imu(self.h, stream, C.c_double(stamp), C.c_float(roll), C.c_float(pitch), C.c_float(yaw),
                                               a.ctypes.data_as(C.c_void_p)))

    def enable_async_downloads(self):
        _check(lib().loamx_pipeline_enable_async_downloads(self.h))

    def download_step_async(self, outs):
        CA = (Cloud * len(outs))(*[cloud_of(a) for a in outs])
        _check(lib().loamx_pipeline_download_step_async(self.h, CA, len(outs)))
        self._dl_keep = (outs, CA)
        return [int(CA[k].count) for k in range(len(outs))]

    def wait_downloads(self):
        _check(lib().loamx_pipeline_wait_downloads(self.h))

    def download_counts(self):
        c = (C.c_uint64 * 2)()
        _check(lib().loamx_pipeline_download_counts(self.h, c))
        return int(c[0]), int(c[1])

    def step(self, t: int):
        return _check(lib().loamx_pipeline_step(self.h, t))

    def get(self, stream: int):
        tr, ts, aft = (np.zeros(6, np.float32) for _ in range(3))
        st = (C.c_int * 8)()
        _check(lib().loamx_pipeline_get(self.h, stream, tr.ctypes.data_as(C.c_void_p), ts.ctypes.data_as(C.c_void_p),
                                        aft.ctypes.data_as(C.c_void_p), st))
        keys = ("odom_iterations", "odom_sel", "map_iterations", "map_sel", "corner_ds", "surf_ds", "degenerate", "mapped")
        return tr, ts, aft, dict(zip(keys, (int(v) for v in st)))

    def download_full_res(self, slot: int, n: int):
        out = np.zeros((n, 4), np.float32)
        c = cloud_of(out)
        _check(lib().loamx_pipeline_download_full_res(self.h, slot, C.byref(c)))
        return out[:c.count]

    def last_clouds(self, stream: int, capacity: int):
        c, s = np.zeros((max(capacity, 1), 4), np.float32), np.zeros((max(capacity, 1), 4), np.float32)
        cc, sc = cloud_of(c), cloud_of(s)
        _check(lib().loamx_pipeline_download_last_clouds(self.h, stream, C.byref(cc), C.byref(sc)))
        return c[:cc.count].copy(), s[:sc.count].copy()

    def set_lookahead(self, on: bool):
        _check(lib().loamx_pipeline_set_lookahead(self.h, 1 if on else 0))

    def lookahead_depth(self) -> int:
        return int(lib().loamx_pipeline_lookahead_depth(self.h))

    def drain_lookahead(self):
        last = C.c_int(-1)
        _check(lib().loamx_pipeline_drain_lookahead(self.h, C.byref(last)))
        return int(last.value)

    def set_timing(self, on, per_launch: bool = True):
        _check(lib().loamx_pipeline_set_timing(self.h, (1 if per_launch else 2) if on else 0))

    def timing(self):
        ms = (C.c_float * 4)()
        rms = (C.c_float * 4)()
        cnt = (C.c_uint64 * 4)()
        _check(lib().loamx_pipeline_get_timing(self.h, ms, rms, cnt))
        return dict(features_ms=ms[0], odometry_ms=ms[1], registration_ms=ms[2], step_ms=ms[3], reg_run_ms=rms[0],
                    residual_ms=rms[1], residual_launches=int(cnt[0]), query_iterations=int(cnt[1]), queries=int(cnt[2]))

    def odom_launch_timing(self):
        ms = (C.c_double * 4)()
        cnt = (C.c_uint64 * 7)()
        _check(lib().loamx_pipeline_get_odom_launch_timing(self.h, ms, cnt))
        return dict(lm_ms=ms[0], lm_noop_ms=ms[1], corr_ms=ms[2], corr_noop_ms=ms[3], lm_launches=int(cnt[0]), lm_noop_launches=int(cnt[1]),
                    lm_iterations=int(cnt[2]), corr_launches=int(cnt[3]), corr_noop_launches=int(cnt[4]), lm_bytes=int(cnt[5]),
                    corr_features=int(cnt[6]))

    @property
    def stream(self) -> int:
        return int(lib().loamx_pipeline_stream(self.h) or 0)


class DenseMapConfig(C.Structure):
    _fields_ = [("leaf", C.c_float), ("min_range", C.c_float), ("max_range", C.c_float), ("max_voxels", C.c_uint64),
                ("initial_slots", C.c_uint32), ("device", C.c_int)]


class DenseMapCarveConfig(C.Structure):
    _fields_ = [("max_range", C.c_float), ("ray_stride", C.c_uint32), ("end_margin", C.c_uint32), ("max_steps", C.c_uint32)]


class DenseMapFileInfo(C.Structure):
    _fields_ = [("version", C.c_uint32), ("flags", C.c_uint32), ("leaf", C.c_float), ("voxels", C.c_uint64), ("offered", C.c_uint64),
                ("dropped_range", C.c_uint64), ("dropped_key", C.c_uint64), ("carve_stats", C.c_uint64 * 6), ("carve", DenseMapCarveConfig)]


def densemap_file_info(path: str, deep: bool = False) -> dict:
    i = DenseMapFileInfo()
    _check(lib().loamx_densemap_file_info(os.fsencode(path), C.byref(i), 1 if deep else 0))
    carving = bool(i.flags & 1)
    return dict(version=int(i.version), flags=int(i.flags), carving=carving, moments=bool(i.flags & 2), leaf=float(i.leaf),
                voxels=int(i.voxels), offered=int(i.offered), dropped_range=int(i.dropped_range), dropped_key=int(i.dropped_key),
                carve_stats=[int(v) for v in i.carve_stats],
                carve=dict(max_range=float(i.carve.max_range), ray_stride=int(i.carve.ray_stride), end_margin=int(i.carve.end_margin),
                           max_steps=int(i.carve.max_steps)) if carving else None)


REGION_INSIDE, REGION_OUTSIDE = 0, 1


class DenseMapRegion(C.Structure):
    _fields_ = [("lo", C.c_int32 * 3), ("hi", C.c_int32 * 3), ("side", C.c_uint32), ("reserved", C.c_uint32)]

    def __init__(self, lo=None, hi=None, side=None):
        super().__init__()
        lib().loamx_densemap_region_default(C.byref(self))
        if lo is not None:
            self.lo[:] = [int(v) for v in lo]
        if hi is not None:
            self.hi[:] = [int(v) for v in hi]
        if side is not None:
            self.side = side

    def check(self):
        _check(lib().loamx_densemap_region_check(C.byref(self)))
        return self

    def outside(self) -> "DenseMapRegion":
        return DenseMapRegion(list(self.lo), list(self.hi), REGION_OUTSIDE if self.side == REGION_INSIDE else REGION_INSIDE)

    def as_dict(self) -> dict:
        return dict(lo=list(self.lo), hi=list(self.hi), side=int(self.side))


class DenseMapPageConfig(C.Structure):
    _fields_ = [("dir", C.c_char_p), ("tile_voxels", C.c_uint32), ("radius", C.c_uint32 * 3)]

    def __init__(self, dir=None, tile_voxels=64, radius=(1, 1, 1)):
        super().__init__()
        self.dir = os.fsencode(dir) if dir is not None else None
        self.tile_voxels = tile_voxels
        self.radius[:] = [int(v) for v in radius]


def _f3(v):
    a = np.ascontiguousarray(v, np.float32)
    assert a.shape == (3,)
    return a


def _i3(v):
    return (C.c_int32 * 3)(*[int(x) for x in v])


def densemap_region_about(leaf: float, centre, half) -> DenseMapRegion:
    r, c, h = DenseMapRegion(), _f3(centre), _f3(half)
    _check(lib().loamx_densemap_region_about(C.c_float(leaf), c.ctypes.data_as(C.c_void_p), h.ctypes.data_as(C.c_void_p), C.byref(r)))
    return r


def densemap_tile_of(idx, tile_voxels: int):
    t = (C.c_int32 * 3)()
    _check(lib().loamx_densemap_tile_of(_i3(idx), C.c_uint32(tile_voxels), t))
    return tuple(int(v) for v in t)


def densemap_tile_region(tile, tile_voxels: int) -> DenseMapRegion:
    r = DenseMapRegion()
    _check(lib().loamx_densemap_tile_region(_i3(tile), C.c_uint32(tile_voxels), C.byref(r)))
    return r


def densemap_tile_name(tile) -> str:
    buf = C.create_string_buffer(64)
    _check(lib().loamx_densemap_tile_name(_i3(tile), buf, C.c_uint64(64)))
    return buf.value.decode()


def densemap_file_merge(path_a: str, path_b: str, path_out: str):
    _check(lib().loamx_densemap_file_merge(os.fsencode(path_a), os.fsencode(path_b), os.fsencode(path_out)))


class StaticRule(C.Structure):
    _fields_ = [("min_misses", C.c_uint32), ("num", C.c_uint32), ("den", C.c_uint32)]

    def __init__(self, min_misses=None, num=None, den=None):
        super().__init__()
        lib().loamx_densemap_static_rule_default(C.byref(self))
        for k, v in (("min_misses", min_misses), ("num", num), ("den", den)):
            if v is not None:
                setattr(self, k, v)

    def is_dynamic(self, n: int, miss: int) -> bool:
        return bool(_check(lib().loamx_densemap_rule_is_dynamic(C.byref(self), C.c_uint64(n), C.c_uint32(miss))))


class SurfelConfig(C.Structure):
    _fields_ = [("min_points", C.c_uint32), ("min_planar_ratio", C.c_float)]

    def __init__(self, min_points=None, min_planar_ratio=None):
        super().__init__()
        lib().loamx_densemap_surfel_default_config(C.byref(self))
        for k, v in (("min_points", min_points), ("min_planar_ratio", min_planar_ratio)):
            if v is not None:
                setattr(self, k, v)


SURFEL_FIELDS = ("x", "y", "z", "intensity", "normal_x", "normal_y", "normal_z", "curvature")

_AXES = {"loam": 0, "sensor": 1}


def _axes(axes) -> int:
    assert axes in _AXES, f"axes must be one of {tuple(_AXES)}"
    return _AXES[axes]


def surfel_of(leaf, idx, vals, mom, axes="loam", min_points=None, min_planar_ratio=None) -> np.ndarray:
    i = (C.c_int32 * 3)(*[int(v) for v in idx])
    v = (C.c_uint64 * 4)(*[int(x) % (1 << 64) for x in vals])
    m = (C.c_uint64 * 9)(*[int(x) % (1 << 64) for x in mom])
    c = SurfelConfig(min_points, min_planar_ratio)
    out = np.zeros(8, np.float32)
    _check(lib().loamx_densemap_surfel_of(C.c_float(leaf), i, v, m, C.byref(c), _axes(axes), out.ctypes.data_as(C.c_void_p)))
    return out


class AlignConfig(C.Structure):
    _fields_ = [("max_iterations", C.c_uint32), ("neighbourhood", C.c_uint32), ("max_residual", C.c_float), ("min_matched", C.c_uint32),
                ("eps_rot", C.c_float), ("eps_trans", C.c_float), ("degenerate_ratio", C.c_float)]

    def __init__(self, **kw):
        super().__init__()
        lib().loamx_densemap_align_default_config(C.byref(self))
        for k, v in kw.items():
            assert hasattr(self, k), k
            if v is not None:
                setattr(self, k, v)


class AlignResult(C.Structure):
    _fields_ = [("pose", C.c_double * 12), ("iterations", C.c_uint32), ("degenerate_dims", C.c_uint32), ("status", C.c_int),
                ("rms", C.c_double), ("counts", C.c_uint64 * 5)]

    def as_dict(self) -> dict:
        return dict(pose=np.array(self.pose[:], np.float64).reshape(3, 4), iterations=int(self.iterations),
                    degenerate_dims=int(self.degenerate_dims), status=int(self.status), rms=float(self.rms),
                    counts=dict(zip(ALIGN_COUNTS, (int(v) for v in self.counts))))


ALIGN_COUNTS = ("far", "outside", "unmatched", "rejected", "matched")


def align_solve(sums, degenerate_ratio=1e-4):
    s = np.ascontiguousarray(sums, np.int64)
    assert s.shape == (28,)
    x = np.zeros(6, np.float64)
    dropped = C.c_uint32(0)
    _check(lib().loamx_densemap_align_solve(s.ctypes.data_as(C.c_void_p), C.c_float(degenerate_ratio), x.ctypes.data_as(C.c_void_p),
                                            C.byref(dropped)))
    return x, int(dropped.value)


ALIGN_MAX_POSES = 4096
PYRAMID_MAX_LEVELS = 6


class PyramidConfig(C.Structure):
    _fields_ = [("levels", C.c_uint32), ("max_curvature", C.c_float)]


def align_best(results):
    arr = results if isinstance(results, C.Array) else (AlignResult * max(len(results), 1))(*results)
    n = len(results)
    best = C.c_uint32(0)
    _check(lib().loamx_densemap_align_best(arr, C.c_uint32(n), C.byref(best)))
    return None if best.value == 0xFFFFFFFF else int(best.value)


def pose_grid(base, centre=None, yaws=(0,), offsets=((0, 0, 0),)) -> np.ndarray:
    P = np.asarray(base, np.float64).reshape(3, 4)
    c = np.zeros(3) if centre is None else np.asarray(centre, np.float64).reshape(3)
    ys = np.asarray(yaws, np.float64).reshape(-1)
    os_ = np.asarray(offsets, np.float64).reshape(-1, 3)
    anchor = P[:, :3] @ c + P[:, 3]
    out = np.zeros((len(ys) * len(os_), 3, 4), np.float64)
    for i, a in enumerate(ys):
        if a == 0.0:
            R = P[:, :3].copy()
        else:
            ca, sa = np.cos(a), np.sin(a)
            R = np.array([[ca, 0.0, sa], [0.0, 1.0, 0.0], [-sa, 0.0, ca]]) @ P[:, :3]
        for j, o in enumerate(os_):
            out[i * len(os_) + j, :, :3] = R
            out[i * len(os_) + j, :, 3] = P[:, 3] if a == 0.0 and not o.any() else (anchor + o) - R @ c
    return out


def _pose12(pose):
    p = np.ascontiguousarray(pose, np.float64)
    assert p.shape == (3, 4) or p.shape == (12,), "a pose is a row-major 3x4 matrix"
    return p.reshape(12)


class RayHit(C.Structure):
    _fields_ = [("key", C.c_uint64), ("x", C.c_float), ("y", C.c_float), ("z", C.c_float), ("range", C.c_float), ("n", C.c_uint32),
                ("miss", C.c_uint32), ("steps", C.c_uint32), ("status", C.c_uint32)]


class RaycastConfig(C.Structure):
    _fields_ = [("max_steps", C.c_uint32), ("skip_steps", C.c_uint32), ("min_points", C.c_uint32)]


RAY_NOT_TRACED, RAY_MISS, RAY_HIT, RAY_HIT_END = range(4)
RAY_COUNTS = ("not_traced", "miss", "hit", "hit_end", "cells")
RAY_DTYPE = np.dtype([(n, np.dtype(t)) for n, t in RayHit._fields_])


def range_image_ends(pose, elevations_deg, n_azimuth: int, max_range: float) -> np.ndarray:
    P = np.asarray(pose, np.float64).reshape(3, 4)
    el = np.deg2rad(np.asarray(elevations_deg, np.float64).reshape(-1))
    az = 2.0 * np.pi * np.arange(int(n_azimuth)) / int(n_azimuth)
    ce, se = np.cos(el)[:, None], np.sin(el)[:, None]
    d = np.stack([ce * np.sin(az)[None, :], se * np.ones_like(az)[None, :], ce * np.cos(az)[None, :]], axis=2).reshape(-1, 3)
    out = np.zeros((len(d), 4), np.float32)
    out[:, :3] = (d * float(max_range)) @ P[:, :3].T + P[:, 3]
    out[:, 3] = np.repeat(np.arange(len(el)), int(n_azimuth))
    return out


# ... 1056 lines not shown
```

Before: 16270.

## Enqueue next step's registration front speculatively with epoch-based adoption

Replaces the opt-in prestage gather with a default-on early front: after collecting step t, the pipeline gathers inputs for step t+1, stages full-res points, uploads registration inputs and enqueues the registration front stage, holding the previous results on the host. The next step adopts that front if no state-changing event bumped the epoch, and otherwise drops it and restores the held state. This aims to hide front-stage and host gather latency behind the host's collect and finish work. In exchange it adds host-side copies of the held results, a non-blocking buffer-free check, and discard paths that waste GPU work whenever speculation is invalidated.

```diff
diff --git a/include/loamx.h b/include/loamx.h
--- a/include/loamx.h
+++ b/include/loamx.h
@@ -267,6 +267,7 @@
 int loamx_pipeline_wait_downloads(loamx_pipeline* h);
 int loamx_pipeline_download_counts(loamx_pipeline* h, uint64_t counts[2]);
 int loamx_pipeline_step(loamx_pipeline* h, uint32_t step);
+int loamx_pipeline_early_front_counts(loamx_pipeline* h, uint64_t counts[4]);
 int loamx_pipeline_get(loamx_pipeline* h, uint32_t stream, float* transform, float* transform_sum, float* aft_mapped,
                        int* stats8);
 int loamx_pipeline_download_full_res(loamx_pipeline* h, uint32_t slot, loamx_cloud* out);
diff --git a/loam_velodyne_amd/csrc/early_front.hpp b/loam_velodyne_amd/csrc/early_front.hpp
--- /dev/null
+++ b/loam_velodyne_amd/csrc/early_front.hpp
@@ -0,0 +1,67 @@
+#pragma once
+#include <atomic>
+#include <cstdint>
+
+namespace loamx {
+
+struct EarlyFrontAsk {
+  bool lookahead_on = false;
+  bool switched_off = false;
+  int next_step = 0;
+  int last_staged = -1;
+  int odom_done_min = -1;
+  bool buffer_free = false;
+  uint32_t n_registered = 0;
+};
+enum class EarlyFrontWhy { goes_out = 0, switched_off, lookahead_off, not_staged, odometry_behind, buffer_busy, nothing_to_register };
+
+inline EarlyFrontWhy early_front_why(const EarlyFrontAsk& a) {
+  if (a.switched_off) return EarlyFrontWhy::switched_off;
+  if (!a.lookahead_on) return EarlyFrontWhy::lookahead_off;
+  if (a.next_step > a.last_staged) return EarlyFrontWhy::not_staged;
+  if (a.odom_done_min < a.next_step) return EarlyFrontWhy::odometry_behind;
+  if (!a.buffer_free) return EarlyFrontWhy::buffer_busy;
+  if (!a.n_registered) return EarlyFrontWhy::nothing_to_register;
+  return EarlyFrontWhy::goes_out;
+}
+inline bool early_front_goes_out(const EarlyFrontAsk& a) { return early_front_why(a) == EarlyFrontWhy::goes_out; }
+
+inline bool early_front_adopted(int front_step, uint64_t front_epoch, int step, uint64_t epoch) {
+  return front_step == step && front_epoch == epoch;
+}
+
+enum class EarlyFrontEvent { set_state, upload, stage_step, set_lookahead, chain_parked, update_imu, swap_frozen, stage_frozen, set_timing, get, download };
+inline bool early_front_bumps_epoch(EarlyFrontEvent e, bool same_slot, bool stream_in_front) {
+  switch (e) {
+    case EarlyFrontEvent::set_state: case EarlyFrontEvent::upload: case EarlyFrontEvent::set_lookahead: case EarlyFrontEvent::chain_parked: return true;
+    case EarlyFrontEvent::stage_step: return same_slot;
+    case EarlyFrontEvent::update_imu: return stream_in_front;
+    default: return false;
+  }
+}
+
+struct EarlyFrontState {
+  std::atomic<uint64_t> epoch{0};
+  bool pending = false;
+  int step = -1;
+  uint64_t front_epoch = 0;
+  uint64_t counts[4] = {0, 0, 0, 0};
+  void note(EarlyFrontEvent e, bool same_slot = true, bool stream_in_front = true) {
+    if (early_front_bumps_epoch(e, same_slot, stream_in_front)) epoch.fetch_add(1, std::memory_order_acq_rel);
+  }
+  bool ask(const EarlyFrontAsk& a) {
+    if (early_front_goes_out(a)) return true;
+    counts[3]++;
+    return false;
+  }
+  void sent(int for_step, uint64_t under_epoch) { pending = true; step = for_step; front_epoch = under_epoch; counts[0]++; }
+  bool take(int t) {
+    if (!pending) return false;
+    pending = false;
+    const bool ok = early_front_adopted(step, front_epoch, t, epoch.load(std::memory_order_acquire));
+    counts[ok ? 1 : 2]++;
+    return ok;
+  }
+};
+
+}
diff --git a/loam_velodyne_amd/csrc/hostlink.hpp b/loam_velodyne_amd/csrc/hostlink.hpp
--- a/loam_velodyne_amd/csrc/hostlink.hpp
+++ b/loam_velodyne_amd/csrc/hostlink.hpp
@@ -73,6 +73,12 @@
   }
   uint32_t engine() const { return engine_mask_ == ~0u ? 0u : engine_mask_; }
   bool pending(int slot) const { return pending_[slot]; }
+  bool landed(int slot) {
+    if (!pending_[slot]) return true;
+    if (hsa_signal_load_scacquire(sig_[slot]) > 0) return false;
+    wait(slot);
+    return true;
+  }
   void wait(int slot) {
     if (!pending_[slot]) return;
     hsa_signal_value_t v;
diff --git a/loam_velodyne_amd/csrc/pipeline.hip b/loam_velodyne_amd/csrc/pipeline.hip
--- a/loam_velodyne_amd/csrc/pipeline.hip
+++ b/loam_velodyne_amd/csrc/pipeline.hip
@@ -5,6 +5,7 @@
 #include "hostlink.hpp"
 #include "densemap.hpp"
 #include "odom_lookahead.hpp"
+#include "early_front.hpp"
 #include <atomic>
 #include <deque>
 #include <chrono>
@@ -32,7 +33,9 @@
 class Pipeline {
  public:
   Pipeline(const loamx_scanreg_config& fc, const loamx_odom_config& oc, const loamx_map_config& mc, uint32_t n_streams)
-      : reg(mc.device, n_streams), fcfg(fc), n_streams_(n_streams), st(n_streams), imu(n_streams), map_imu(n_streams), map_imu_seq(n_streams, 0) {
+      : reg(mc.device, n_streams), fcfg(fc), n_streams_(n_streams), st(n_streams), imu(n_streams), map_imu(n_streams), map_imu_seq(n_streams, 0),
+        in_front(new std::atomic<char>[n_streams]) {
+    for (uint32_t s = 0; s < n_streams; s++) in_front[s].store(0);
     OdomParams op;
     op.scan_period = oc.scan_period;
     op.max_iterations = diag_env("LOAMX_ODOM_MAXIT") ? atoi(diag_env("LOAMX_ODOM_MAXIT")) : oc.max_iterations;
@@ -202,12 +205,13 @@
   }
   int drain_lookahead() { return prefetch ? la->drain() : la->done_min(); }
   void park_odometry(int restart) {
-    if (restart >= 0) pre_t = -1;
+    ef.note(EarlyFrontEvent::chain_parked);
     la->park(restart);
   }
 
   ~Pipeline() {
     la.reset();
+    if (ef.pending) (void)hipStreamSynchronize(reg.stream());
     for (auto& c : chains) {
       for (auto& e : c->ev_tail) if (e) (void)hipEventDestroy(e);
       for (auto& tm : c->tm) tm.destroy();
@@ -255,6 +259,7 @@
     fx.clear();
   }
   void restart_input_(uint32_t n_slots, bool ring) {
+    ef.note(EarlyFrontEvent::upload);
     streaming = ring;
     staged_hi = 0;
     last_step = -1;
@@ -289,6 +294,7 @@
     LX_REQUIRE(t < RING || last_step.load() + (long)RING >= (long)t, std::string(entry) + "(t) needs step(t - 8) to have run: only eight steps can be in flight");
   }
   void publish_staged_(uint32_t t) {
+    ef.note(EarlyFrontEvent::stage_step, (int)(t % RING) == front_slot.load(std::memory_order_acquire));
     LA(t) = 0;
     staged_hi.store(t + 1, std::memory_order_release);
   }
@@ -550,36 +556,6 @@
       N.to_end = odom.to_end_params(l, true);
     }
   }
-  int pre_t = -1;
-  void prestage_gather(int tn, int last_staged, hipStream_t s_) {
-    static const bool off = !(diag_env("LOAMX_PRESTAGE") && atoi(diag_env("LOAMX_PRESTAGE")) != 0);
-    if (off || !prefetch || pre_t == tn || tn > last_staged || tn < 1) return;
-    const uint32_t ns = n_streams_;
-    if (la->done_min() < tn) return;
-    FeatureExtractor& F = FX((uint32_t)tn);
-    std::vector<const float4*> fsrc;
-    std::vector<uint32_t> nfr;
-    std::vector<ToEndParams> tep;
-    for (uint32_t s = 0; s < ns; s++) {
-      const OdomPub& N = ores[tn % OR][s];
-      if (N.rc != LOAMX_OK) continue;
-      fsrc.push_back(F.d_cloud() + F.point_base(s));
-      nfr.push_back(F.point_base(s + 1) - F.point_base(s));
-      tep.push_back(N.to_end);
-    }
-    const uint32_t nw = (uint32_t)fsrc.size();
-    if (!nw) return;
-    const int par = (int)(run_count & 1);
-    hostlink.wait(par);
-    if (d2h_pending[par]) { LX_HIP(hipStreamWaitEvent(s_, ev_d2h[par], 0)); d2h_pending[par] = false; }
-    float4* dst = reg.stage_full_next(nw, nfr.data());
-    if (!dst) return;
-    std::vector<uint32_t> foff(nw + 1, 0);
-    for (uint32_t k = 0; k < nw; k++) foff[k + 1] = foff[k] + nfr[k];
-    chains[0]->ob->to_end_gather(dst, foff.data(), fsrc.data(), tep.data(), nw, s_);
-    pre_t = tn;
-  }
-
   bool trace = getenv("LOAMX_PIPE_TRACE") != nullptr;
   std::chrono::steady_clock::time_point tr0, tr_exit = std::chrono::steady_clock::now();
   double tr_us() const { return std::chrono::duration<double, std::micro>(std::chrono::steady_clock::now() - tr0).count(); }
@@ -598,7 +574,16 @@
     uint32_t nw = 0;
     float f_ms = 0.f;
     double gap_us = 0, tr[5] = {0, 0, 0, 0, 0};
+    std::vector<uint32_t> foff;
+    int front = 0;
+    double tr_front[2] = {0, 0};
   };
+  EarlyFrontState ef;
+  Step fS;
+  std::vector<PipeStreamState> fst;
+  std::atomic<int> front_slot{-1};
+  std::unique_ptr<std::atomic<char>[]> in_front;
+  const bool no_early_front = getenv("LOAMX_NO_EARLY_FRONT") != nullptr;
   void launch_features_upto(int k) {
     while (f_hi < k) { ++f_hi; if (!LA((uint32_t)f_hi)) launch_features((uint32_t)f_hi); }
   }
@@ -638,9 +623,7 @@
     launch_features_upto(S.w.feat_late);
     la->allow(S.w.odom_late);
   }
-  void gather_inputs_(Step& S) {
-    S.tr[0] = tr_us();
-    if (timing) tmM[S.t & 1].start(S.s_);
+  void gather_inputs_(Step& S, std::vector<PipeStreamState>& st) {
     const uint32_t ns = n_streams_;
     FeatureExtractor& F = FX(S.t);
     S.cl.resize(ns); S.sl.resize(ns); S.fsrc.resize(ns);
@@ -661,41 +644,52 @@
       S.who.push_back(s);
     }
     S.nw = (uint32_t)S.who.size();
+    S.foff.assign(S.nw + 1, 0);
+    for (uint32_t k = 0; k < S.nw; k++) S.foff[k + 1] = S.foff[k] + S.nfr[k];
   }
   void stage_full_res_(Step& S) {
+    if (!S.nw) return;
+    float4* full_dst = reg.stage_full(S.nw, S.nfr.data());
+    chains[0]->ob->to_end_gather(full_dst, S.foff.data(), S.fsrc.data(), S.to_end.data(), S.nw, S.s_);
+  }
+  bool full_buffer_free_(Step& S, bool block) {
+    const int par = (int)(run_count & 1);
+    if (block) {
+      const double tw0 = trace ? tr_us() : 0.0;
+      hostlink.wait(par);
+      if (trace) S.tr[4] = tr_us() - tw0;
+      if (d2h_pending[par]) { LX_HIP(hipStreamWaitEvent(S.s_, ev_d2h[par], 0)); d2h_pending[par] = false; }
+      return true;
+    }
+    if (!hostlink.landed(par)) return false;
+    if (d2h_pending[par]) {
+      const hipError_t q = hipEventQuery(ev_d2h[par]);
+      if (q == hipErrorNotReady) return false;
+      LX_HIP(q);
+      d2h_pending[par] = false;
+    }
+    return true;
+  }
+  void count_run_(Step& S) {
     if (!S.nw) { last_full_off.clear(); last_who.clear(); return; }
-    const uint32_t nw = S.nw;
-    std::vector<uint32_t> foff(nw + 1, 0);
-    for (uint32_t k = 0; k < nw; k++) foff[k + 1] = foff[k] + S.nfr[k];
-    const bool adopted = pre_t == S.ti && reg.adopt_full_next(nw, S.nfr.data());
-    pre_t = -1;
-    if (!adopted) {
-      if (reg.double_buffer_full) {
-        const int par = (int)(run_count & 1);
-        const double tw0 = trace ? tr_us() : 0.0;
-        hostlink.wait(par);
-        if (trace) S.tr[4] = tr_us() - tw0;
-        if (d2h_pending[par]) { LX_HIP(hipStreamWaitEvent(S.s_, ev_d2h[par], 0)); d2h_pending[par] = false; }
-      }
-      float4* full_dst = reg.stage_full(nw, S.nfr.data());
-      chains[0]->ob->to_end_gather(full_dst, foff.data(), S.fsrc.data(), S.to_end.data(), nw, S.s_);
-    }
-    last_full_off = foff;
+    last_full_off = S.foff;
     last_who = S.who;
     run_count++;
+  }
+  void upload_registration_(Step& S) {
+    reg.upload_device(S.nw, S.cl.data(), S.ncl.data(), S.sl.data(), S.nsl.data(), nullptr, nullptr, S.guess.data());
   }
   void enqueue_registration_(Step& S) {
     if (!S.nw) return;
     const uint32_t nw = S.nw;
     const RawSlot& R = rawslot[S.t % RING];
-    reg.upload_device(nw, S.cl.data(), S.ncl.data(), S.sl.data(), S.nsl.data(), nullptr, nullptr, S.guess.data());
     bool blend = false;
     static const bool no_blend = diag_env("LOAMX_NO_MAP_IMU_BLEND") != nullptr;
     if (!no_blend && streaming && R.raw && !R.scan_time.empty())
       for (uint32_t k = 0; k < nw; k++) blend = blend || R.map_imu_upto[S.who[k]] > 0;
     reg.defer_full = blend;
-    reg.on_first_wait = [&]() { release_late_(S); prestage_gather(S.ti + 1, S.last_staged, S.s_); };
-    reg.run_async();
+    reg.on_first_wait = [&]() { release_late_(S); };
+    reg.run_async(false, S.front == 1);
     reg.on_first_wait = nullptr;
     if (blend) {
       std::vector<float> p6(6 * (size_t)nw);
@@ -713,7 +707,6 @@
   }
   void release_behind_registration_(Step& S) {
     release_late_(S);
-    if (S.nw) prestage_gather(S.ti + 1, S.last_staged, S.s_);
     if (timing) tmM[S.t & 1].stop(S.s_);
     S.tr[1] = tr_us();
   }
@@ -739,6 +732,61 @@
     S.tr[2] = tr_us();
     return ret;
   }
+  void send_front_(Step& S) {
+    const int tn = S.ti + 1;
+    const uint64_t epoch = ef.epoch.load(std::memory_order_acquire);
+    EarlyFrontAsk a;
+    a.lookahead_on = prefetch;
+    a.switched_off = no_early_front;
+    a.next_step = tn;
+    a.last_staged = (int)n_staged() - 1;
+    a.odom_done_min = la->done_min();
+    a.buffer_free = true;
+    a.n_registered = 1;
+    if (early_front_goes_out(a)) {
+      fS = Step();
+      fS.t = (uint32_t)tn; fS.ti = tn; fS.s_ = S.s_;
+      fst = st;
+      for (uint32_t s = 0; s < n_streams_; s++) fst[s].cur = ores[tn % OR][s];
+      gather_inputs_(fS, fst);
+      a.n_registered = fS.nw;
+      a.buffer_free = full_buffer_free_(fS, false);
+    }
+    if (!ef.ask(a)) return;
+    if (trace) S.tr_front[0] = tr_us();
+    for (auto& c : chains) LX_HIP(hipStreamWaitEvent(S.s_, c->ev_tail[tn % OR], 0));
+    (void)tmM[tn & 1].resolve();
+    tmM[tn & 1].start(S.s_);
+    reg.hold_results();
+    try {
+      stage_full_res_(fS);
+      upload_registration_(fS);
+      reg.run_front();
+    } catch (...) {
+      reg.drop_front();
+      throw;
+    }
+    for (uint32_t k = 0; k < fS.nw; k++) in_front[fS.who[k]].store(1, std::memory_order_release);
+    front_slot.store(streaming ? tn % (int)RING : -1, std::memory_order_release);
+    ef.sent(tn, epoch);
+    if (trace) S.tr_front[1] = tr_us();
+  }
+  bool take_front_(Step& S) {
+    if (!ef.pending) return false;
+    const bool adopt = ef.take(S.ti);
+    front_slot.store(-1, std::memory_order_release);
+    for (uint32_t s = 0; s < n_streams_; s++) in_front[s].store(0, std::memory_order_release);
+    S.front = adopt ? 1 : 2;
+    if (!adopt) {
+      reg.drop_front();
+      return false;
+    }
+    S.who = std::move(fS.who); S.cl = std::move(fS.cl); S.sl = std::move(fS.sl); S.fsrc = std::move(fS.fsrc);
+    S.ncl = std::move(fS.ncl); S.nsl = std::move(fS.nsl); S.nfr = std::move(fS.nfr); S.guess = std::move(fS.guess);
+    S.to_end = std::move(fS.to_end); S.foff = std::move(fS.foff); S.nw = fS.nw;
+    st = fst;
+    return true;
+  }
   void finish_step_(Step& S) {
     const uint32_t t = S.t;
     S.tr[3] = tr_us();
@@ -751,6 +799,7 @@
         fprintf(stderr, " O[%u-%u): %.0f %.0f %.0f %.0f done %d pass %.0f us |", c.s0, c.s1, c.tr[0], c.tr[1], c.tr[2], c.tr[3], la->done(g), (double)c.last_us.load());
       }
       fprintf(stderr, " f_hi %d o_limit %d staged %u", f_hi, la->limit(), n_staged());
+      fprintf(stderr, " | front %s  next-front %.0f %.0f", S.front == 1 ? "adopted" : S.front == 2 ? "discarded" : "none", S.tr_front[0], S.tr_front[1]);
       fprintf(stderr, "\n");
     }
     if (timing) {
@@ -780,13 +829,27 @@
     S.s_ = reg.stream();
     S.last_staged = (int)n_staged() - 1;
     S.w = lookahead_window(S.ti, depth(), S.last_staged, prefetch);
-    join_odometry_(S);
-    release_lookahead_(S);
-    gather_inputs_(S);
-    stage_full_res_(S);
+    if (take_front_(S)) {
+      LX_REQUIRE(!la->jumped(S.ti) && S.ti <= la->done_min(), "internal: an adopted front without its odometry");
+      LA(t) = 0;
+      S.f_ms = feat_ms[t % OR];
+      release_lookahead_(S);
+      S.tr[0] = tr_us();
+    } else {
+      join_odometry_(S);
+      release_lookahead_(S);
+      S.tr[0] = tr_us();
+      if (timing) tmM[S.t & 1].start(S.s_);
+      gather_inputs_(S, st);
+      if (S.nw && reg.double_buffer_full) full_buffer_free_(S, true);
+      stage_full_res_(S);
+      if (S.nw) upload_registration_(S);
+    }
+    count_run_(S);
     enqueue_registration_(S);
     release_behind_registration_(S);
     const int ret = collect_(S);
+    send_front_(S);
     finish_step_(S);
     return ret;
   }
@@ -859,6 +922,7 @@
                              const float* aft) {
   return guard([&]() {
     LX_REQUIRE(h && stream < h->p.n_streams_, "invalid stream");
+    h->p.ef.note(EarlyFrontEvent::set_state);
     h->p.park_odometry(-1);
     if (transform) h->p.OB(stream).stream_state(h->p.LS(stream)).transform.set(transform);
     if (transform_sum) h->p.OB(stream).stream_state(h->p.LS(stream)).transform_sum.set(transform_sum);
@@ -893,6 +957,7 @@
 int loamx_pipeline_update_imu(loamx_pipeline* h, uint32_t stream, double stamp_sec, float roll, float pitch, float yaw, const float acc_xyz[3]) {
   return guard([&]() {
     LX_REQUIRE(h && acc_xyz && stream < h->p.n_streams_, "invalid argument");
+    h->p.ef.note(EarlyFrontEvent::update_imu, true, h->p.in_front[stream].load(std::memory_order_acquire) != 0);
     h->p.imu[stream].update(stamp_sec, roll, pitch, yaw, acc_xyz);
     h->p.map_imu_push(stream, stamp_sec, roll, pitch);
     return LOAMX_OK;
@@ -909,6 +974,13 @@
     LX_REQUIRE(h && counts, "NULL argument");
     counts[0] = h->p.downloads_direct;
     counts[1] = h->p.downloads_hip;
+    return LOAMX_OK;
+  });
+}
+int loamx_pipeline_early_front_counts(loamx_pipeline* h, uint64_t counts[4]) {
+  return guard([&]() {
+    LX_REQUIRE(h && counts, "NULL argument");
+    for (int k = 0; k < 4; k++) counts[k] = h->p.ef.counts[k];
     return LOAMX_OK;
   });
 }
@@ -956,6 +1028,7 @@
 int loamx_pipeline_set_lookahead(loamx_pipeline* h, int on) {
   return guard([&]() {
     LX_REQUIRE(h, "NULL handle");
+    h->p.ef.note(EarlyFrontEvent::set_lookahead);
     if (!on && h->p.prefetch) h->p.park_odometry(-1);
     h->p.prefetch = on != 0;
     return LOAMX_OK;
diff --git a/loam_velodyne_amd/csrc/registration.hip b/loam_velodyne_amd/csrc/registration.hip
--- a/loam_velodyne_amd/csrc/registration.hip
+++ b/loam_velodyne_amd/csrc/registration.hip
@@ -554,10 +554,12 @@
   h_poses_.reserve(max_sweeps);
   ev_.resize(2 + 2 * 64);
   for (auto& e : ev_) LX_HIP(hipEventCreate(&e));
+  LX_HIP(hipEventCreate(&ev_front_));
 }
 
 Registrar::~Registrar() {
   for (auto& e : ev_) (void)hipEventDestroy(e);
+  if (ev_front_) (void)hipEventDestroy(ev_front_);
   if (ev_build_) (void)hipEventDestroy(ev_build_);
   if (ev_swap_) (void)hipEventDestroy(ev_swap_);
   if (ev_look_) (void)hipEventDestroy(ev_look_);
@@ -729,37 +731,16 @@
 
 float4* Registrar::stage_full(uint32_t n_sweeps, const uint32_t* n_full) {
   LX_REQUIRE(n_sweeps >= 1 && n_sweeps <= max_sweeps_, "n_sweeps out of range for this handle");
-  full_next_staged_ = false;
   prefix_offsets(h_full_off_, n_sweeps, [&](uint32_t s) { return n_full[s]; });
   n_full_ = h_full_off_[n_sweeps];
   if (double_buffer_full) {
     std::swap(full_.p, full_alt_.p);
     std::swap(full_.cap, full_alt_.cap);
+    if (held_.on) held_.swapped = !held_.swapped;
   }
   full_.reserve((size_t)n_full_ + 1);
   full_staged_ = true;
   return full_.p;
-}
-
-float4* Registrar::stage_full_next(uint32_t n_sweeps, const uint32_t* n_full) {
-  LX_REQUIRE(double_buffer_full, "internal: pre-staging needs the second full-resolution buffer");
-  LX_REQUIRE(n_sweeps >= 1 && n_sweeps <= max_sweeps_, "n_sweeps out of range for this handle");
-  prefix_offsets(next_full_off_, n_sweeps, [&](uint32_t s) { return n_full[s]; });
-  if ((size_t)next_full_off_[n_sweeps] + 1 > full_alt_.cap) return nullptr;
-  full_next_staged_ = true;
-  return full_alt_.p;
-}
-bool Registrar::adopt_full_next(uint32_t n_sweeps, const uint32_t* n_full) {
-  if (!full_next_staged_ || next_full_off_.size() != n_sweeps + 1) { full_next_staged_ = false; return false; }
-  for (uint32_t s = 0; s < n_sweeps; s++)
-    if (next_full_off_[s + 1] - next_full_off_[s] != n_full[s]) { full_next_staged_ = false; return false; }
-  full_next_staged_ = false;
-  h_full_off_ = next_full_off_;
-  n_full_ = h_full_off_[n_sweeps];
-  std::swap(full_.p, full_alt_.p);
-  std::swap(full_.cap, full_alt_.cap);
-  full_staged_ = true;
-  return true;
 }
 
 void Registrar::upload_device(uint32_t n_sweeps, const float4* const* corner_last, const uint32_t* n_corner,
@@ -937,16 +918,63 @@
 }
 #endif
 
-void Registrar::begin_attempt_(bool legacy) {
-  if (timing_) LX_HIP(hipEventRecord(ev_[0], st_));
-  n_res_launch_ = 0;
+void Registrar::begin_attempt_(bool legacy, bool early) {
+  if (early) LX_HIP(hipEventRecord(ev_front_, st_));
+  else if (timing_) LX_HIP(hipEventRecord(ev_[0], st_));
+  if (!early) n_res_launch_ = 0;
   if (early_exit) memset(h_stats_.p, 0, sizeof(SweepStats) * n_sweeps_);
   run_ = Run{};
   run_.vb_unchecked = !legacy && n_in_ > 0;
 }
 
-void Registrar::run_async(bool force_general) {
+void Registrar::hold_results() {
+  LX_REQUIRE(!held_.on, "internal: results are held already");
+  held_ = Held{};
+  held_.n_sweeps = n_sweeps_;
+  held_.full_off = h_full_off_;
+  held_.full = full_.p;
+  if (n_sweeps_) {
+    fetch_results();
+    held_.stats.assign(h_stats_.p, h_stats_.p + n_sweeps_);
+    held_.poses.assign(h_poses_.p, h_poses_.p + n_sweeps_);
+  }
+  held_.on = true;
+}
+
+void Registrar::run_front() {
+  LX_REQUIRE(held_.on && n_sweeps_ > 0, "internal: run_front() needs hold_results() and upload_device()");
+  TraceRange trace_range("loamx:registration:front");
+  LX_HIP(hipSetDevice(device_));
+  front_legacy_ = vb_disabled_ || !VoxBucket::fits(n_in_, 2 * n_sweeps_);
+  begin_attempt_(front_legacy_, true);
+  enqueue_front(front_legacy_);
+  front_out_ = true;
+  LX_HIP(hipGetLastError());
+}
+
+void Registrar::drop_front() {
+  if (!held_.on) return;
+  if (held_.swapped) {
+    std::swap(full_.p, full_alt_.p);
+    std::swap(full_.cap, full_alt_.cap);
+  }
+  n_sweeps_ = held_.n_sweeps;
+  h_full_off_ = held_.full_off;
+  n_full_ = h_full_off_.empty() ? 0u : h_full_off_.back();
+  if (n_sweeps_) {
+    memcpy(h_stats_.p, held_.stats.data(), sizeof(SweepStats) * n_sweeps_);
+    memcpy(h_poses_.p, held_.poses.data(), sizeof(Pose) * n_sweeps_);
+  }
+  run_ = Run{};
+  run_.mirrors_written = run_.results_final = true;
+  full_staged_ = front_out_ = false;
+  held_ = Held{};
+}
+
+void Registrar::run_async(bool force_general, bool adopt_front) {
   LX_REQUIRE(n_sweeps_ > 0, "run() before upload()");
+  LX_REQUIRE(!adopt_front || (front_out_ && held_.on && !force_general), "internal: no front to continue");
+  LX_REQUIRE(adopt_front || !held_.on, "internal: a front is out: continue it or drop it");
   TraceRange trace_range("loamx:registration");
   static const bool trace = getenv("LOAMX_REG_TRACE") != nullptr;
   RunTrace tr{trace, trace ? host_us() : 0.0};
@@ -955,8 +983,16 @@
   RegOutcome o;
   for (int attempt = 0; attempt < 2; attempt++) {
     const bool legacy = attempt == 1 || !can_bucket;
-    begin_attempt_(legacy);
-    enqueue_front(legacy);
+    if (adopt_front && attempt == 0) {
+      LX_REQUIRE(legacy == front_legacy_, "internal: the front took another voxel path");
+      std::swap(ev_[0], ev_front_);
+      n_res_launch_ = 0;
+      front_out_ = false;
+      held_ = Held{};
+    } else {
+      begin_attempt_(legacy);
+      enqueue_front(legacy);
+    }
     if (trace) tr.front = host_us();
     o = RegOutcome{};
     if (submap_sufficient() && n_in_ > 0) {
@@ -1127,21 +1163,25 @@
 }
 
 void Registrar::download_stats(SweepStats* out) {
+  if (held_.on) { if (held_.n_sweeps) memcpy(out, held_.stats.data(), sizeof(SweepStats) * held_.n_sweeps); return; }
   fetch_results();
   memcpy(out, h_stats_.p, sizeof(SweepStats) * n_sweeps_);
 }
 
 void Registrar::download(float* poses6, int* stats4) {
-  LX_REQUIRE(n_sweeps_ > 0, "download() before run()");
-  fetch_results();
-  for (uint32_t s = 0; s < n_sweeps_; s++) {
+  const uint32_t ns = held_.on ? held_.n_sweeps : n_sweeps_;
+  LX_REQUIRE(ns > 0, "download() before run()");
+  if (!held_.on) fetch_results();
+  const Pose* hp = held_.on ? held_.poses.data() : h_poses_.p;
+  const SweepStats* hs = held_.on ? held_.stats.data() : h_stats_.p;
+  for (uint32_t s = 0; s < ns; s++) {
     if (poses6) {
-      const Pose& T = h_poses_.p[s];
+      const Pose& T = hp[s];
       float* o = poses6 + 6 * s;
       o[0] = T.rx; o[1] = T.ry; o[2] = T.rz; o[3] = T.tx; o[4] = T.ty; o[5] = T.tz;
     }
     if (stats4) {
-      const SweepStats& st = h_stats_.p[s];
+      const SweepStats& st = hs[s];
       int* o = stats4 + 4 * s;
       o[0] = st.iterations; o[1] = st.sel; o[2] = st.corner_q; o[3] = st.surf_q;
     }
@@ -1163,6 +1203,15 @@
 }
 
 int Registrar::download_full_res(uint32_t sweep, loamx_cloud* out) {
+  if (held_.on) {
+    LX_REQUIRE(sweep < held_.n_sweeps, "sweep index out of range");
+    check_cloud(out, false);
+    const uint32_t a = held_.full_off[sweep], b = held_.full_off[sweep + 1];
+    h_full_dl_.reserve((size_t)(b - a) + 1);
+    if (b > a) LX_HIP(hipMemcpyAsync(h_full_dl_.p, held_.full + a, sizeof(float4) * (b - a), hipMemcpyDeviceToHost, st_));
+    wait_stream(st_);
+    return unpack_cloud(h_full_dl_.p, b - a, out);
+  }
   LX_REQUIRE(sweep < n_sweeps_, "sweep index out of range");
   check_cloud(out, false);
   fetch_results();
@@ -1215,7 +1264,7 @@
     ms[1] += t;
   }
   counts[0] = n_res_launch_;
-  std::vector<SweepStats> st(n_sweeps_);
+  std::vector<SweepStats> st(held_.on ? held_.n_sweeps : n_sweeps_);
   download_stats(st.data());
   for (auto& s : st) {
     counts[1] += (uint64_t)s.iterations * (uint64_t)(s.corner_q + s.surf_q);
diff --git a/loam_velodyne_amd/csrc/registration.hpp b/loam_velodyne_amd/csrc/registration.hpp
--- a/loam_velodyne_amd/csrc/registration.hpp
+++ b/loam_velodyne_amd/csrc/registration.hpp
@@ -54,9 +54,11 @@
   void upload_device(uint32_t n_sweeps, const float4* const* corner_last, const uint32_t* n_corner, const float4* const* surf_last,
                      const uint32_t* n_surf, const float4* const* full_res, const uint32_t* n_full, const float* guess6);
   float4* stage_full(uint32_t n_sweeps, const uint32_t* n_full);
-  float4* stage_full_next(uint32_t n_sweeps, const uint32_t* n_full);
-  bool adopt_full_next(uint32_t n_sweeps, const uint32_t* n_full);
-  void run_async(bool force_general = false);
+  void run_async(bool force_general = false, bool adopt_front = false);
+  void hold_results();
+  void run_front();
+  void drop_front();
+  bool holding() const { return held_.on; }
   void sync();
   void download(float* poses6, int* stats4);
   void download_stats(SweepStats* out);
@@ -68,7 +70,7 @@
   const float4* d_ds_points() const { return ds_pts_.p; }
   const uint32_t* d_ds_offsets() const { return ds_off_.p; }
   const Pose* d_poses() const { return poses_.p; }
-  const float4* d_full_res() const { return full_.p; }
+  const float4* d_full_res() const { return held_.on ? held_.full : full_.p; }
   uint32_t full_offset(uint32_t s) const { return h_full_off_[s]; }
 
   void knn_probe(int which, const float* xyz, uint32_t n, uint32_t* idx5, float* d2_5);
@@ -93,8 +95,7 @@
   DevBuf<float4> in_, stack_, ds_pts_, full_, full_alt_;
   DevBuf<uint32_t> ds_off_;
   DevBuf<float> guess_;
-  bool full_staged_ = false, full_next_staged_ = false;
-  std::vector<uint32_t> next_full_off_;
+  bool full_staged_ = false;
   hipEvent_t ev_look_ = nullptr;
   PinBuf<float4> h_full_dl_;
   struct Run {
@@ -104,6 +105,15 @@
     int full_dl_sweep = -1;
     void* full_dl_direct = nullptr;
   } run_;
+  struct Held {
+    bool on = false, swapped = false;
+    uint32_t n_sweeps = 0;
+    std::vector<uint32_t> full_off;
+    const float4* full = nullptr;
+    std::vector<SweepStats> stats;
+    std::vector<Pose> poses;
+  } held_;
+  bool front_out_ = false, front_legacy_ = false;
   VoxelPipeline vox_;
   VoxBucket vb_;
   bool vb_disabled_ = false;
@@ -115,7 +125,7 @@
   struct RunTrace;
   template <class Count> void plan_inputs_(uint32_t n_sweeps, bool staged, Count&& count);
   size_t write_param_block_(const float* guess6, const float4* const* corner_src, const float4* const* surf_src, const float4* const* full_src);
-  void begin_attempt_(bool legacy);
+  void begin_attempt_(bool legacy, bool early = false);
   RegOutcome run_iterations(RunTrace& tr);
   bool bucket_stage_gave_up_();
   void dump_gn_profile_();
@@ -145,6 +155,7 @@
   uint32_t nblk_ = 0;
 
   std::vector<hipEvent_t> ev_;
+  hipEvent_t ev_front_ = nullptr;
   int n_res_launch_ = 0;
   PinBuf<SweepStats> h_stats_;
   PinBuf<Pose> h_poses_;
diff --git a/loam_velodyne_amd/loamx.py b/loam_velodyne_amd/loamx.py
--- a/loam_velodyne_amd/loamx.py
+++ b/loam_velodyne_amd/loamx.py
@@ -875,6 +875,11 @@
     def step(self, t: int):
         return _check(lib().loamx_pipeline_step(self.h, t))
 
+    def early_front_counts(self):
+        c = (C.c_uint64 * 4)()
+        _check(lib().loamx_pipeline_early_front_counts(self.h, c))
+        return dict(zip(("enqueued", "adopted", "discarded", "not_attempted"), (int(v) for v in c)))
+
     def get(self, stream: int):
         tr, ts, aft = (np.zeros(6, np.float32) for _ in range(3))
         st = (C.c_int * 8)()
```

New measurement: 15880. 2.4% lower.
